# ypicchi-arm/vectorscan

Measured on AMD Instinct MI355X. Metric: GB/s scanned (hsbench block mode), FDR 5k literals, higher is better.
Workload: dtype u8; 1 GPU; cfg4: FDR 5000 literals len 4-8 (2% nocase), one 4 GiB corpus as 4 blocks striped over 1 GPU(s), engine id 0; global_bytes=4294967296, parallelism=stripe1

## Files before the change

include/vectorscan_amd.h:

```cpp
#ifndef VECTORSCAN_AMD_H
#define VECTORSCAN_AMD_H

#include <stddef.h>
#include <stdint.h>

#if defined(__x86_64__) || defined(__i386__)
#include <emmintrin.h>
typedef __m128i vsa_m128_t;
#else
typedef struct { uint8_t b[16]; } __attribute__((aligned(16))) vsa_m128_t;
#endif

#ifdef __cplusplus
extern "C" {
#endif


struct HWLM;
struct FDR;
struct noodTable;
struct hs_scratch;
union AccelAux;

typedef int hwlm_error_t;
// ... 85 lines not shown
#define VSA_E_OVERFLOW (-5)

typedef struct vsa_ctx vsa_ctx_t;
typedef struct vsa_db vsa_db_t;

typedef struct {
    uint64_t key;
    uint32_t id;
    uint32_t pad;
} vsa_match_t;

int vsa_device_count(void);
int vsa_ctx_create(int device, vsa_ctx_t **ctx);
int vsa_ctx_destroy(vsa_ctx_t *ctx);
int vsa_ctx_create_shared(vsa_ctx_t *base, vsa_ctx_t **ctx);
void *vsa_ctx_stream(vsa_ctx_t *ctx);
int vsa_ctx_set_reserved_cus(vsa_ctx_t *ctx, int n);

int vsa_db_load(vsa_ctx_t *ctx, const void *hwlm, size_t size, vsa_db_t **db);
int vsa_db_free(vsa_db_t *db);
int vsa_db_engine(const vsa_db_t *db);

int vsa_malloc(vsa_ctx_t *ctx, size_t bytes, void **dptr);
int vsa_free(vsa_ctx_t *ctx, void *dptr);
int vsa_memcpy_h2d(vsa_ctx_t *ctx, void *dst, const void *src, size_t bytes);
int vsa_memcpy_d2h(vsa_ctx_t *ctx, void *dst, const void *src, size_t bytes);
int vsa_sync(vsa_ctx_t *ctx);

#define VSA_MAX_BLOCKS (1u << 20)

#define VSA_SCAN_UNSORTED 1u
#define VSA_SCAN_ASYNC 2u
int vsa_scan_blocks(vsa_ctx_t *ctx, const vsa_db_t *db, const uint8_t *d_data,
                    const uint64_t *offsets, const uint64_t *lens,
                    const uint64_t *starts, uint32_t nblocks, uint32_t flags,
                    uint64_t *n_matches);
int vsa_scan_blocks_ex(vsa_ctx_t *ctx, const vsa_db_t *db, const uint8_t *d_data,
                       const uint64_t *offsets, const uint64_t *lens,
                       const uint64_t *starts, const uint64_t *report_lo,
                       uint32_t nblocks, uint32_t flags, uint64_t *n_matches);
int vsa_scan_blocks_stream(vsa_ctx_t *ctx, const vsa_db_t *db, const uint8_t *d_data,
                           const uint64_t *offsets, const uint64_t *lens,
                           const uint64_t *starts, const uint64_t *hlens, uint32_t nblocks,
                           uint32_t flags, uint64_t *n_matches);
typedef struct vsa_plan vsa_plan_t;
int vsa_plan_describe(const uint8_t *d_data, const uint64_t *offsets, const uint64_t *lens,
                      const uint64_t *starts, const uint64_t *hlens, const uint64_t *report_lo,
                      uint32_t nblocks, uint32_t num_cus, uint32_t ns, uint32_t *words,
                      uint64_t cap, uint64_t *nsegs, uint32_t *grid,
                      const float *wg_weights);
int vsa_plan_blocks(const uint8_t *d_data, const uint64_t *offsets, const uint64_t *lens,
                    const uint64_t *starts, const uint64_t *hlens, const uint64_t *report_lo,
                    uint32_t nblocks, void *out);

int vsa_plan_dyn(const uint8_t *d_data, const uint64_t *offsets, const uint64_t *lens,
                 const uint64_t *starts, const uint64_t *hlens, const uint64_t *report_lo,
                 uint32_t nblocks, uint32_t num_cus, uint32_t ns, uint32_t *out);
int vsa_feedback_simulate(const double *rate, uint32_t grid, uint32_t launches, double jitter,
                          float *w_out);
int vsa_plan_create(vsa_ctx_t *ctx, const uint8_t *d_data, const uint64_t *offsets,
                    const uint64_t *lens, const uint64_t *starts, const uint64_t *hlens,
                    const uint64_t *report_lo, uint32_t nblocks, vsa_plan_t **plan);
int vsa_plan_free(vsa_plan_t *plan);
uint32_t vsa_plan_rebuilds(const vsa_plan_t *plan);
int vsa_scan_plan(vsa_ctx_t *ctx, const vsa_db_t *db, const vsa_plan_t *plan, uint32_t flags,
                  uint64_t *n_matches);
int vsa_scan_wait(vsa_ctx_t *ctx, uint64_t *n_matches);
int vsa_scan_pack(vsa_ctx_t *ctx, void *d_dst, uint64_t cap);
int vsa_scan_plan_pack(vsa_ctx_t *ctx, const vsa_db_t *db, const vsa_plan_t *plan, void *d_dst,
                       uint64_t cap);
int vsa_scan_results(vsa_ctx_t *ctx, const uint64_t **d_keys,
                     const uint32_t **d_ids);
int vsa_scan_copy(vsa_ctx_t *ctx, vsa_match_t *out, uint64_t cap,
                  uint64_t *n_copied);
int vsa_scan_copy_device(vsa_ctx_t *ctx, uint64_t *d_keys, uint32_t *d_ids, uint64_t cap,
                         uint64_t *n_copied);
uint64_t vsa_scan_candidates(vsa_ctx_t *ctx);
int vsa_scan_debug_counters(vsa_ctx_t *ctx, uint64_t out[16]);
double vsa_scan_kernel_ms(vsa_ctx_t *ctx);
int vsa_ctx_set_timing(vsa_ctx_t *ctx, uint32_t every);
uint64_t vsa_scan_launches(vsa_ctx_t *ctx);
int vsa_scan_last_fused(vsa_ctx_t *ctx);
int vsa_scan_last_dyn(vsa_ctx_t *ctx);
int vsa_ctx_set_dyn_shares(vsa_ctx_t *ctx, int on, uint64_t min_bytes);
int vsa_ctx_set_fused_finish(vsa_ctx_t *ctx, int on);
int vsa_read_ceiling(vsa_ctx_t *ctx, const uint8_t *d_data, uint64_t len, uint32_t runs,
                     double *best_ms, uint64_t *bytes);

int vsa_class_scan(vsa_ctx_t *ctx, const uint8_t cls[32], const uint8_t *cls2,
                   const uint8_t *d_data, uint64_t len, uint64_t *d_bitmap,
                   uint64_t *first, uint64_t *last, uint64_t *count,
                   uint32_t flags);
int vsa_class_scan_masks(vsa_ctx_t *ctx, int kind, const uint8_t a[16], const uint8_t b[16],
                         const uint8_t *d_data, uint64_t len, uint64_t *d_bitmap,
                         uint64_t *first, uint64_t *last, uint64_t *count);


typedef struct {
    const uint8_t *s;
    uint32_t len;
    uint32_t id;
    uint8_t nocase;
    uint8_t noruns;
    uint8_t msk_len;
    uint8_t pad;
    uint64_t groups;
    const uint8_t *msk;
    const uint8_t *cmp;
} vsa_literal_t;

typedef struct {
    int32_t engine_hint;
    uint8_t allow_noodle;
    uint8_t allow_teddy;
    uint8_t allow_fat_teddy;
    uint8_t allow_flood;
} vsa_build_opts_t;

void vsa_build_opts_default(vsa_build_opts_t *o);
int vsa_hwlm_build(const vsa_literal_t *lits, size_t n,
                   const vsa_build_opts_t *opts, void **blob, size_t *size);
void vsa_blob_free(void *blob);
int vsa_hwlm_set_accel(void *blob, const union AccelAux *accel0,
                       const union AccelAux *accel1, uint64_t accel1_groups);
int vsa_shufti_build_masks(const uint8_t cls[32], uint8_t lo[16], uint8_t hi[16]);
void vsa_truffle_build_masks(const uint8_t cls[32], uint8_t m1[16], uint8_t m2[16]);

int64_t vsa_shufti_find(const uint8_t lo[16], const uint8_t hi[16],
                        const uint8_t *buf, size_t len, int reverse);
int64_t vsa_truffle_find(const uint8_t m1[16], const uint8_t m2[16],
                         const uint8_t *buf, size_t len, int reverse);
int64_t vsa_shufti_double_find(const uint8_t lo1[16], const uint8_t hi1[16],
                               const uint8_t lo2[16], const uint8_t hi2[16],
                               const uint8_t *buf, size_t len);
void vsa_set_accel_vector_size(uint32_t vsize);

void vsa_set_wave_log(void *d_log);
int vsa_shufti_build_double_masks(const uint8_t onechar[32], const uint8_t *pairs,
                                  size_t npairs, uint8_t lo1[16], uint8_t hi1[16],
                                  uint8_t lo2[16], uint8_t hi2[16]);
int64_t vsa_verm_find(int mode, uint8_t c1, uint8_t c2, uint8_t m1, uint8_t m2,
                      int nocase, const uint8_t *buf, size_t len);

int vsa_derive_first_stage(const void *hwlm, size_t size, uint64_t *table, uint32_t cap,
                           uint32_t *key_bits, uint32_t *field_bits);
int vsa_derive_fdr4_table(const void *hwlm, size_t size, uint32_t bits, uint32_t *table,
                          uint32_t cap);

int vsa_derive_fdr4_pass(const void *hwlm, size_t size, int par, uint32_t *table, uint32_t cap,
                         double *text_rate);

int vsa_db_split(const vsa_db_t *db);

void vsa_set_scratch_layout(long fdr_conf_off, long fdr_conf_offset_off);
void vsa_get_scratch_layout(long *fdr_conf_off, long *fdr_conf_offset_off);

void vsa_set_scratch_core_info(long buf_off, long hbuf_off, long hlen_off);
void vsa_get_scratch_core_info(long *buf_off, long *hbuf_off, long *hlen_off);

int vsa_last_error(void);

const char *vsa_version(void);

#ifdef __cplusplus
}
#endif
// ... 3 lines not shown
```

vectorscan_amd/__init__.py:

```python
import ctypes
import os

import numpy as np

__all__ = [
    "HWLM_SUCCESS", "HWLM_TERMINATED", "HWLM_ERROR_UNKNOWN",
    "HWLM_ALL_GROUPS", "HWLM_CONTINUE_MATCHING", "HWLM_TERMINATE_MATCHING",
    "HwlmLiteral", "hwlm_build", "hwlm_exec", "fdr_exec", "nood_exec",
    "engine_blob", "shufti_exec", "rshufti_exec", "truffle_exec",
    "rtruffle_exec", "vermicelli_exec", "nvermicelli_exec",
    "rvermicelli_exec", "rnvermicelli_exec", "vermicelli_double_exec",
    "vermicelli_double_masked_exec", "shufti_build_masks",
    "truffle_build_masks", "Context", "Database", "lib", "LIB_PATH",
]

HWLM_SUCCESS = 0
HWLM_TERMINATED = 1
HWLM_ERROR_UNKNOWN = 2
HWLM_ALL_GROUPS = (1 << 64) - 1
HWLM_CONTINUE_MATCHING = HWLM_ALL_GROUPS
HWLM_TERMINATE_MATCHING = 0

ENGINE_NOOD = 16
HWLM_HEADER = 192
# ... 41 lines not shown
_sig("vsa_hwlm_set_accel", ctypes.c_int, ctypes.c_void_p, ctypes.c_void_p,
     ctypes.c_void_p, ctypes.c_uint64)
_sig("hwlmExec", ctypes.c_int, ctypes.c_void_p, ctypes.c_void_p, ctypes.c_size_t,
     ctypes.c_size_t, HWLMCallback, ctypes.c_void_p, ctypes.c_uint64)
_sig("fdrExec", ctypes.c_int, ctypes.c_void_p, ctypes.c_void_p, ctypes.c_size_t,
     ctypes.c_size_t, HWLMCallback, ctypes.c_void_p, ctypes.c_uint64)
_sig("noodExec", ctypes.c_int, ctypes.c_void_p, ctypes.c_void_p, ctypes.c_size_t,
     ctypes.c_size_t, HWLMCallback, ctypes.c_void_p)
_sig("hwlmExecStreaming", ctypes.c_int, ctypes.c_void_p, ctypes.c_size_t, ctypes.c_size_t,
     HWLMCallback, ctypes.c_void_p, ctypes.c_uint64)
_sig("fdrExecStreaming", ctypes.c_int, ctypes.c_void_p, ctypes.c_void_p, ctypes.c_size_t,
     ctypes.c_void_p, ctypes.c_size_t, ctypes.c_size_t, HWLMCallback, ctypes.c_void_p,
     ctypes.c_uint64)
_sig("noodExecStreaming", ctypes.c_int, ctypes.c_void_p, ctypes.c_void_p, ctypes.c_size_t,
     ctypes.c_void_p, ctypes.c_size_t, HWLMCallback, ctypes.c_void_p)
_sig("vsa_get_scratch_core_info", None, ctypes.POINTER(ctypes.c_long),
     ctypes.POINTER(ctypes.c_long), ctypes.POINTER(ctypes.c_long))
_sig("vsa_shufti_find", ctypes.c_int64, ctypes.c_void_p, ctypes.c_void_p,
     ctypes.c_void_p, ctypes.c_size_t, ctypes.c_int)
_sig("vsa_shufti_double_find", ctypes.c_int64, ctypes.c_void_p, ctypes.c_void_p,
     ctypes.c_void_p, ctypes.c_void_p, ctypes.c_void_p, ctypes.c_size_t)
_sig("vsa_set_accel_vector_size", None, ctypes.c_uint32)
_sig("vsa_shufti_build_double_masks", ctypes.c_int, ctypes.c_void_p, ctypes.c_void_p,
     ctypes.c_size_t, ctypes.c_void_p, ctypes.c_void_p, ctypes.c_void_p, ctypes.c_void_p)
_sig("vsa_truffle_find", ctypes.c_int64, ctypes.c_void_p, ctypes.c_void_p,
     ctypes.c_void_p, ctypes.c_size_t, ctypes.c_int)
_sig("vsa_verm_find", ctypes.c_int64, ctypes.c_int, ctypes.c_uint8, ctypes.c_uint8,
     ctypes.c_uint8, ctypes.c_uint8, ctypes.c_int, ctypes.c_void_p, ctypes.c_size_t)
_sig("vsa_shufti_build_masks", ctypes.c_int, ctypes.c_void_p, ctypes.c_void_p,
     ctypes.c_void_p)
_sig("vsa_truffle_build_masks", None, ctypes.c_void_p, ctypes.c_void_p,
     ctypes.c_void_p)
_sig("vsa_device_count", ctypes.c_int)
_sig("vsa_ctx_create", ctypes.c_int, ctypes.c_int, ctypes.POINTER(ctypes.c_void_p))
_sig("vsa_ctx_destroy", ctypes.c_int, ctypes.c_void_p)
_sig("vsa_ctx_create_shared", ctypes.c_int, ctypes.c_void_p, ctypes.POINTER(ctypes.c_void_p))
_sig("vsa_ctx_stream", ctypes.c_void_p, ctypes.c_void_p)
_sig("vsa_db_load", ctypes.c_int, ctypes.c_void_p, ctypes.c_void_p, ctypes.c_size_t,
     ctypes.POINTER(ctypes.c_void_p))
_sig("vsa_db_free", ctypes.c_int, ctypes.c_void_p)
_sig("vsa_db_engine", ctypes.c_int, ctypes.c_void_p)
_sig("vsa_malloc", ctypes.c_int, ctypes.c_void_p, ctypes.c_size_t,
     ctypes.POINTER(ctypes.c_void_p))
_sig("vsa_free", ctypes.c_int, ctypes.c_void_p, ctypes.c_void_p)
_sig("vsa_memcpy_h2d", ctypes.c_int, ctypes.c_void_p, ctypes.c_void_p,
     ctypes.c_void_p, ctypes.c_size_t)
_sig("vsa_memcpy_d2h", ctypes.c_int, ctypes.c_void_p, ctypes.c_void_p,
     ctypes.c_void_p, ctypes.c_size_t)
_sig("vsa_sync", ctypes.c_int, ctypes.c_void_p)
_sig("vsa_scan_blocks", ctypes.c_int, ctypes.c_void_p, ctypes.c_void_p,
     ctypes.c_void_p, _u64p, _u64p, ctypes.c_void_p, ctypes.c_uint32,
     ctypes.c_uint32, _u64p)
_sig("vsa_scan_blocks_ex", ctypes.c_int, ctypes.c_void_p, ctypes.c_void_p,
     ctypes.c_void_p, _u64p, _u64p, ctypes.c_void_p, ctypes.c_void_p, ctypes.c_uint32,
     ctypes.c_uint32, _u64p)
_sig("vsa_scan_blocks_stream", ctypes.c_int, ctypes.c_void_p, ctypes.c_void_p,
     ctypes.c_void_p, _u64p, _u64p, ctypes.c_void_p, _u64p, ctypes.c_uint32,
     ctypes.c_uint32, _u64p)
_sig("vsa_plan_create", ctypes.c_int, ctypes.c_void_p, ctypes.c_void_p, ctypes.c_void_p,
     ctypes.c_void_p, ctypes.c_void_p, ctypes.c_void_p, ctypes.c_void_p, ctypes.c_uint32,
     ctypes.POINTER(ctypes.c_void_p))
_sig("vsa_plan_free", ctypes.c_int, ctypes.c_void_p)
_sig("vsa_plan_rebuilds", ctypes.c_uint32, ctypes.c_void_p)
_sig("vsa_scan_plan", ctypes.c_int, ctypes.c_void_p, ctypes.c_void_p, ctypes.c_void_p,
     ctypes.c_uint32, _u64p)
_sig("vsa_scan_wait", ctypes.c_int, ctypes.c_void_p, _u64p)
_sig("vsa_scan_pack", ctypes.c_int, ctypes.c_void_p, ctypes.c_void_p, ctypes.c_uint64)
_sig("vsa_scan_plan_pack", ctypes.c_int, ctypes.c_void_p, ctypes.c_void_p, ctypes.c_void_p,
     ctypes.c_void_p, ctypes.c_uint64)
_sig("vsa_scan_results", ctypes.c_int, ctypes.c_void_p,
     ctypes.POINTER(ctypes.c_void_p), ctypes.POINTER(ctypes.c_void_p))
_sig("vsa_scan_copy", ctypes.c_int, ctypes.c_void_p, ctypes.c_void_p,
     ctypes.c_uint64, _u64p)
_sig("vsa_scan_copy_device", ctypes.c_int, ctypes.c_void_p, ctypes.c_void_p, ctypes.c_void_p,
     ctypes.c_uint64, _u64p)
_sig("vsa_scan_candidates", ctypes.c_uint64, ctypes.c_void_p)
_sig("vsa_scan_debug_counters", ctypes.c_int, ctypes.c_void_p, ctypes.c_void_p)
_sig("vsa_derive_first_stage", ctypes.c_int, ctypes.c_void_p, ctypes.c_size_t, ctypes.c_void_p,
     ctypes.c_uint32, ctypes.POINTER(ctypes.c_uint32), ctypes.POINTER(ctypes.c_uint32))
_sig("vsa_scan_kernel_ms", ctypes.c_double, ctypes.c_void_p)
_sig("vsa_scan_launches", ctypes.c_uint64, ctypes.c_void_p)
_sig("vsa_scan_last_fused", ctypes.c_int, ctypes.c_void_p)
_sig("vsa_scan_last_dyn", ctypes.c_int, ctypes.c_void_p)
_sig("vsa_ctx_set_dyn_shares", ctypes.c_int, ctypes.c_void_p, ctypes.c_int, ctypes.c_uint64)
_sig("vsa_ctx_set_fused_finish", ctypes.c_int, ctypes.c_void_p, ctypes.c_int)
_sig("vsa_ctx_set_timing", ctypes.c_int, ctypes.c_void_p, ctypes.c_uint32)
_sig("vsa_ctx_set_reserved_cus", ctypes.c_int, ctypes.c_void_p, ctypes.c_int)
_sig("vsa_read_ceiling", ctypes.c_int, ctypes.c_void_p, ctypes.c_void_p, ctypes.c_uint64,
     ctypes.c_uint32, ctypes.POINTER(ctypes.c_double), _u64p)
_sig("vsa_class_scan", ctypes.c_int, ctypes.c_void_p, ctypes.c_void_p,
     ctypes.c_void_p, ctypes.c_void_p, ctypes.c_uint64, ctypes.c_void_p, _u64p,
     _u64p, _u64p, ctypes.c_uint32)
_sig("vsa_class_scan_masks", ctypes.c_int, ctypes.c_void_p, ctypes.c_int, ctypes.c_void_p,
     ctypes.c_void_p, ctypes.c_void_p, ctypes.c_uint64, ctypes.c_void_p, _u64p, _u64p, _u64p)
_sig("vsa_version", ctypes.c_char_p)
_sig("vsa_set_scratch_layout", None, ctypes.c_long, ctypes.c_long)
_sig("vsa_get_scratch_layout", None, ctypes.POINTER(ctypes.c_long), ctypes.POINTER(ctypes.c_long))
_sig("vsa_last_error", ctypes.c_int)


class HwlmLiteral:

    def __init__(self, s, nocase=False, id=0, noruns=False,
                 groups=HWLM_ALL_GROUPS, msk=b"", cmp=b""):
        if isinstance(s, str):
            s = s.encode("latin-1")
        self.s = bytes(s)
        self.nocase = bool(nocase)
        self.id = int(id)
        self.noruns = bool(noruns)
        self.groups = int(groups)
        self.msk = bytes(msk)
        self.cmp = bytes(cmp)

    def __repr__(self):
        return "HwlmLiteral(%r, nocase=%s, id=%d)" % (self.s, self.nocase, self.id)


class Blob:

    def __init__(self, ptr, size, owned=True):
        self.ptr = ptr
        self.size = size
        self.owned = owned

    def tobytes(self):
        return ctypes.string_at(self.ptr, self.size)

    @property
    def type(self):
        return ctypes.string_at(self.ptr, 1)[0]

    @property
    def is_noodle(self):
        return self.type == ENGINE_NOOD

    @property
    def engine_id(self):
        if self.is_noodle:
            return None
        return int(np.frombuffer(ctypes.string_at(self.ptr + HWLM_HEADER, 4), np.uint32)[0])

    def set_accel(self, accel0=None, accel1=None, accel1_groups=0):
        a0 = ctypes.create_string_buffer(bytes(accel0), 80) if accel0 else None
        a1 = ctypes.create_string_buffer(bytes(accel1), 80) if accel1 else None
        _check(lib.vsa_hwlm_set_accel(self.ptr, a0, a1, accel1_groups))

    def __del__(self):
        if getattr(self, "ptr", None) and getattr(self, "owned", True) and lib is not None:
            lib.vsa_blob_free(self.ptr)
        self.ptr = None


class BuildError(RuntimeError):
    pass


def _check(rc):
    if rc != 0:
        raise BuildError("vectorscan_amd call failed with %d" % rc)


def hwlm_build(lits, engine_hint=-1, allow_noodle=True, allow_teddy=True,
               allow_fat_teddy=True, allow_flood=True):
    arr = (_Literal * len(lits))()
    keep = []
# ... 404 lines not shown
        ln = np.ascontiguousarray(lens, np.uint64)
        hl = np.ascontiguousarray(hlens, np.uint64)
        st = None if starts is None else np.ascontiguousarray(starts, np.uint64)
        n = ctypes.c_uint64()
        flags = (0 if sort else 1) | (2 if asynchronous else 0)
        rc = lib.vsa_scan_blocks_stream(
            self.ptr, db.ptr, d_data, off.ctypes.data_as(_u64p), ln.ctypes.data_as(_u64p),
            None if st is None else st.ctypes.data, hl.ctypes.data_as(_u64p), len(off), flags,
            ctypes.byref(n))
        if rc != 0:
            raise RuntimeError("vsa_scan_blocks_stream failed (%d)" % rc)
        return n.value

    def plan(self, d_data, offsets, lens, starts=None, hlens=None, report_lo=None):
        arrs = [None if a is None else np.ascontiguousarray(a, np.uint64)
                for a in (offsets, lens, starts, hlens, report_lo)]
        h = ctypes.c_void_p()
        rc = lib.vsa_plan_create(self.ptr, d_data, *[None if a is None else a.ctypes.data
                                                      for a in arrs], len(arrs[0]),
                                 ctypes.byref(h))
        if rc != 0:
            raise RuntimeError("vsa_plan_create failed (%d)" % rc)
        return Plan(self, h.value)

    def scan_plan(self, db, plan, sort=True, asynchronous=False):
        n = ctypes.c_uint64()
        flags = (0 if sort else 1) | (2 if asynchronous else 0)
        rc = lib.vsa_scan_plan(self.ptr, db.ptr, plan.ptr, flags, ctypes.byref(n))
        if rc != 0:
            raise RuntimeError("vsa_scan_plan failed (%d)" % rc)
        return n.value

    def scan_wait(self):
        n = ctypes.c_uint64()
        _check(lib.vsa_scan_wait(self.ptr, ctypes.byref(n)))
        return n.value

    def scan_pack(self, d_dst, cap):
        _check(lib.vsa_scan_pack(self.ptr, d_dst, cap))

    def scan_plan_pack(self, db, plan, d_dst, cap):
        _check(lib.vsa_scan_plan_pack(self.ptr, db.ptr, plan.ptr, d_dst, cap))

    def results(self, n):
        out = np.zeros(n, dtype=[("key", np.uint64), ("id", np.uint32), ("pad", np.uint32)])
        got = ctypes.c_uint64()
        _check(lib.vsa_scan_copy(self.ptr, out.ctypes.data, n, ctypes.byref(got)))
        return out[: got.value]

    def results_to_device(self, d_keys, d_ids, cap):
        got = ctypes.c_uint64()
        _check(lib.vsa_scan_copy_device(self.ptr, d_keys, d_ids, cap, ctypes.byref(got)))
        return got.value

    def candidates(self):
        return lib.vsa_scan_candidates(self.ptr)

    def debug_counters(self):
        out = (ctypes.c_uint64 * 16)()
        _check(lib.vsa_scan_debug_counters(self.ptr, out))
        return list(out)

    def kernel_ms(self):
        return lib.vsa_scan_kernel_ms(self.ptr)

    def reserve_cus(self, n):
        _check(lib.vsa_ctx_set_reserved_cus(self.ptr, n))

    def launches(self):
        return lib.vsa_scan_launches(self.ptr)

    def timing(self, every=1):
        _check(lib.vsa_ctx_set_timing(self.ptr, every))

    def fused_finish(self, on=True):
        _check(lib.vsa_ctx_set_fused_finish(self.ptr, 1 if on else 0))

    def last_fused(self):
        return lib.vsa_scan_last_fused(self.ptr) == 1

    def last_dyn(self):
        return lib.vsa_scan_last_dyn(self.ptr) == 1

    def dyn_shares(self, on=True, min_mib=2048):
        _check(lib.vsa_ctx_set_dyn_shares(self.ptr, 1 if on else 0, int(min_mib) << 20))

    def read_ceiling(self, d_data, length, runs=5):
        ms = ctypes.c_double()
        n = ctypes.c_uint64()
        _check(lib.vsa_read_ceiling(self.ptr, d_data, length, runs, ctypes.byref(ms),
                                    ctypes.byref(n)))
        return n.value / (ms.value * 1e-3) / 1e9, ms.value, n.value

    def class_scan(self, cls, d_data, length, d_bitmap=None, cls2=None):
        cls = np.ascontiguousarray(cls, np.uint8)
        c2 = None if cls2 is None else np.ascontiguousarray(cls2, np.uint8)
        f, l, c = ctypes.c_uint64(), ctypes.c_uint64(), ctypes.c_uint64()
        _check(lib.vsa_class_scan(self.ptr, cls.ctypes.data,
                                  None if c2 is None else c2.ctypes.data, d_data,
                                  length, d_bitmap, ctypes.byref(f), ctypes.byref(l),
                                  ctypes.byref(c), 0))
        return f.value, l.value, c.value

    def class_scan_masks(self, kind, a, b, d_data, length, d_bitmap=None):
        ma = ctypes.create_string_buffer(bytes(a), 16)
        mb = ctypes.create_string_buffer(bytes(b), 16)
        f, l, c = ctypes.c_uint64(), ctypes.c_uint64(), ctypes.c_uint64()
        _check(lib.vsa_class_scan_masks(self.ptr, 0 if kind == "shufti" else 1, ma, mb, d_data,
                                        length, d_bitmap, ctypes.byref(f), ctypes.byref(l),
                                        ctypes.byref(c)))
        return f.value, l.value, c.value

    def close(self):
        if self.ptr:
            lib.vsa_ctx_destroy(self.ptr)
            self.ptr = None

    def __del__(self):
        try:
            self.close()
        except Exception:
            pass


class Plan:

    def __init__(self, ctx, ptr):
        self.ctx = ctx
        self.ptr = ptr

    def rebuilds(self):
        return lib.vsa_plan_rebuilds(self.ptr)

    def close(self):
        if self.ptr:
            lib.vsa_plan_free(self.ptr)
            self.ptr = None

    def __del__(self):
        try:
            self.close()
        except Exception:
            pass


class Database:

    def __init__(self, ctx, blob):
        self.ctx = ctx
        self.blob = blob
        self.ptr = ctypes.c_void_p()
        rc = lib.vsa_db_load(ctx.ptr, blob.ptr, blob.size, ctypes.byref(self.ptr))
        if rc != 0:
            raise RuntimeError("vsa_db_load failed (%d)" % rc)

    @property
    def engine(self):
        return lib.vsa_db_engine(self.ptr)

    @property
    def split(self):
        return lib.vsa_db_split(self.ptr) == 1

    def close(self):
        if self.ptr:
            lib.vsa_db_free(self.ptr)
# ... 6 lines not shown
```

vectorscan_amd/csrc/kernels.h:

```cpp
#ifndef VSA_KERNELS_H
#define VSA_KERNELS_H

#include <stdint.h>

struct VsaBlock {
    uint64_t base;
    uint64_t len;
    uint64_t start;
    uint64_t seg_first;
    int64_t zbase;
    int64_t org;
    int64_t rlo;
    uint64_t hlen;
    uint32_t hist;
    uint32_t flags;
};
#ifdef __cplusplus
static_assert(sizeof(VsaBlock) == 72, "VsaBlock layout (vsa_plan_blocks, tests/test_plan.py)");
#endif

#define VSA_BLK_STREAM 1u
#define VSA_BLK_RUN 2u
#define VSA_RUN_MAX 128u
#define VSA_RUN_MIN_LEN 1024u

#define VSA_KEY_END_SHIFT 24
#define VSA_KEY_BUCKET_SHIFT 20
#define VSA_KEY_LI_MASK 0xfffffu

#ifdef __HIPCC__
__host__ __device__
#endif
static inline uint32_t vsa_fdr4_key(uint32_t b2, uint32_t b1, uint32_t b0) {
    return (b1 & 0x7fu) | ((b2 & 1u) << 7) | ((b0 & 0x7fu) << 8);
}

enum VsaLitMode {
    VSA_MODE_TEDDY = 1,
    VSA_MODE_FAT = 2,
    VSA_MODE_NOOD = 3,
    VSA_MODE_FDR4 = 4,
};

#define VSA_SORT_BIN_BITS 14
#define VSA_SORT_BINS (1u << VSA_SORT_BIN_BITS)
#define VSA_LBINS 256u
#define VSA_SORT_BIN_MAX 64
#define VSA_CTR_BIN_OVERFLOW 12
#define VSA_FIN_MAX_GRID 1024u

struct VsaLitParams {
    const uint8_t *data;
    const VsaBlock *blocks;
    uint32_t nblocks;
    uint64_t nsegs;
    const uint32_t *seg_desc;
    const uint32_t *wg_seg;
    const uint32_t *wg_bins;
    uint32_t steal;
    const uint64_t *table;
    uint32_t table_entries;
    uint32_t dmask;
    uint32_t end_par;
    uint64_t state_lo, state_hi;
    const uint8_t *conf_base;
    uint32_t conf_off[16];
    const uint32_t *slotmap;
    uint32_t slot_words;
    uint32_t slot_off[16];
    uint8_t slot_bits[16];
    uint64_t nood_msk, nood_cmp;
    uint32_t nood_len, nood_id;
    uint64_t pf_mult;
    uint32_t qcap;
    uint32_t nconf;
    uint32_t dbg;
    uint64_t *out_keys;
    uint32_t *out_ids;
    uint64_t out_cap;
    uint32_t *bin_counts;
    uint32_t bin_shift;
    uint64_t *bin_keys;
    uint32_t *bin_ids;
    unsigned long long *wg_time;
    unsigned long long *wave_log;
    unsigned long long *counters;
    const uint32_t *fin_wg;
    uint64_t *fin_keys;
    uint32_t *fin_ids;
    unsigned long long *fin_agg;
    uint32_t fin_epoch;
    unsigned long long *fin_pub;
    unsigned long long fin_seq;
    uint64_t *fin_pk;
    uint64_t fin_pk_cap;
    const unsigned long long *dyn_prev;
    const uint32_t *dyn_wprev;
    uint32_t *dyn_wout;
    uint32_t dyn_kib;
    uint32_t dyn_margin;
};


struct VsaClassParams {
    const uint8_t *data;
    uint64_t len;
    uint32_t cls[8];
    uint32_t cls2[8];
    int pair;
    uint64_t *bitmap;
    unsigned long long *first;
    unsigned long long *last;
    unsigned long long *count;
    uint32_t slots;
};

struct VsaPairParams {
    const uint8_t *data;
    uint64_t len;
    uint8_t n1[256], n2[256];
    uint32_t vsize;
    uint32_t mis;
    unsigned long long *first;
};

// ... 2 lines not shown
```

vectorscan_amd/csrc/kernels.hip:

```cpp
#include <hip/hip_runtime.h>
#include <stdint.h>

#include "kernels.h"

#define WAVE 64
#define LIT_WAVES 16
#ifdef VSA_DIAG
#define VSA_DIAG_ON 1
#else
#define VSA_DIAG_ON 0
#endif
#define VSA_DBG(flags, bits) (VSA_DIAG_ON && ((flags) & (bits)))
#define LIT_THREADS (LIT_WAVES * WAVE)
#define QCAP 256

typedef uint32_t u32;
typedef uint64_t u64;
typedef uint8_t u8;

__device__ __forceinline__ u32 lane_id() { return __lane_id(); }

__device__ __forceinline__ u32 readlane_u32(u32 v, int src) {
    return (u32)__builtin_amdgcn_readlane((int)v, src);
}
__device__ __forceinline__ u32 readfirstlane_u32(u32 v) {
    return (u32)__builtin_amdgcn_readfirstlane((int)v);
}

__device__ __forceinline__ u32 shfl_u32(u32 v, int src) {
    return (u32)__shfl((int)v, src, WAVE);
}
__device__ __forceinline__ u32 shfl_up_u32(u32 v, unsigned d) {
    return (u32)__shfl_up((int)v, d, WAVE);
}
__device__ __forceinline__ u32 lane_up1(u32 v) {
    return (u32)__builtin_amdgcn_update_dpp(0, (int)v, 0x138, 0xf, 0xf, true);
}
__device__ __forceinline__ u32 lane_down1(u32 v) {
    return (u32)__builtin_amdgcn_update_dpp(0, (int)v, 0x130, 0xf, 0xf, true);
}
__device__ __forceinline__ u32 lane_up1_or_old(u32 old, u32 v) {
    return (u32)__builtin_amdgcn_update_dpp((int)old, (int)v, 0x138, 0xf, 0xf, false);
}
__device__ __forceinline__ u32 lane_ror1(u32 v) {
    return (u32)__builtin_amdgcn_update_dpp(0, (int)v, 0x13c, 0xf, 0xf, true);
}
template <int L>
__device__ __forceinline__ u32 writelane_u32(u32 v, u32 s) {
    asm("v_writelane_b32 %0, %1, %2" : "+v"(v) : "s"(readfirstlane_u32(s)), "n"(L));
    return v;
}
typedef const __attribute__((address_space(3))) u64 lds_u64_t;
typedef const __attribute__((address_space(3))) u8 lds_u8_t;
__device__ __forceinline__ u64 lds_ld64(u32 addr) { return *(lds_u64_t *)(uintptr_t)addr; }

#define TEDDY_TAB_LDS 0x10000u

__device__ __forceinline__ u32 or3(u32 a, u32 b, u32 c) {
    u32 r;
    asm("v_or3_b32 %0, %1, %2, %3" : "=v"(r) : "v"(a), "v"(b), "v"(c));
    return r;
}
__device__ __forceinline__ u32 shfl_xor_u32(u32 v, int m) {
    return (u32)__shfl_xor((int)v, m, WAVE);
}
__device__ __forceinline__ u32 shfl_down_u32(u32 v, unsigned d) {
    return (u32)__shfl_down((int)v, d, WAVE);
}
template <int M>
__device__ __forceinline__ u32 lane_xor(u32 v) {
    static_assert(M == 1 || M == 2 || M == 4 || M == 8 || M == 16 || M == 32, "lane_xor");
    if constexpr (M == 1) {
        return (u32)__builtin_amdgcn_update_dpp(0, (int)v, 0xB1, 0xf, 0xf, false);
    } else if constexpr (M == 2) {
        return (u32)__builtin_amdgcn_update_dpp(0, (int)v, 0x4E, 0xf, 0xf, false);
    } else if constexpr (M == 4) {
        const int h = __builtin_amdgcn_update_dpp(0, (int)v, 0x141, 0xf, 0xf, false);
        return (u32)__builtin_amdgcn_update_dpp(0, h, 0x1B, 0xf, 0xf, false);
    } else if constexpr (M == 8) {
        const int h = __builtin_amdgcn_update_dpp(0, (int)v, 0x140, 0xf, 0xf, false);
        return (u32)__builtin_amdgcn_update_dpp(0, h, 0x141, 0xf, 0xf, false);
    } else if constexpr (M == 16) {
        return (u32)__builtin_amdgcn_ds_swizzle((int)v, 0x401F);
    } else {
        return shfl_xor_u32(v, 32);
    }
}

struct Bins4 {
    u64 k[4];
    u32 id[4], jb[4];
    bool ok[4];
    u32 S, npass, r;
};
__device__ __forceinline__ void bins4_load(Bins4 &B, const uint64_t *skeys, const uint32_t *sids,
// ... 109 lines not shown
    }
    *total = shfl_u32(x, WAVE - 1);
    return x - v;
}

__device__ __forceinline__ u8 load_byte_masked(const u8 *A, int64_t aoff, int64_t lo, int64_t hi,
                                               bool want, const u8 *safe) {
    const bool ok = want && aoff >= lo && aoff < hi;
    typedef const __attribute__((address_space(1))) u8 gu8;
    const u8 v = *(gu8 *)(ok ? A + aoff : safe);
    return ok ? v : (u8)0;
}

__device__ __forceinline__ VsaBlock load_block(const VsaBlock *blocks, u32 i) {
    static_assert(sizeof(VsaBlock) == 9 * sizeof(u64), "VsaBlock: 9 words");
    typedef const __attribute__((address_space(4))) u64 cu64;
    cu64 *p = (cu64 *)(blocks + i);
    u64 w[9];
#pragma unroll
    for (int k = 0; k < 9; k++) w[k] = p[k];
    VsaBlock b;
    __builtin_memcpy(&b, w, sizeof(b));
    return b;
}


template <int MODE>
struct LitTraits;

template <>
struct LitTraits<VSA_MODE_TEDDY> {
    static constexpr int LB = 8;
    static constexpr int NL = 4;
    static constexpr int CW = 4;
    static constexpr int EW = 3;
    typedef u32 S_t;
};
template <>
struct LitTraits<VSA_MODE_NOOD> {
    static constexpr int LB = 8;
    static constexpr int NL = 1;
    static constexpr int CW = 1;
    static constexpr int EW = 2;
    typedef u32 S_t;
};
template <>
struct LitTraits<VSA_MODE_FAT> {
    static constexpr int LB = 16;
    static constexpr int NL = 4;
    static constexpr int CW = 8;
    static constexpr int EW = 4;
    typedef u64 S_t;
};
template <>
struct LitTraits<VSA_MODE_FDR4> {
    static constexpr int LB = 8;
    static constexpr int NL = 4;
    static constexpr int CW = 4;
    static constexpr int EW = 3;
    typedef u32 S_t;
};

struct PfRec {
    u64 andmsk;
    u32 slot_off;
    u32 shift;
};

struct ConfLds {
    u64 andmsk[16];
    u64 mult[16];
    u32 nbits[16];
    u32 off[16];
    PfRec pf[16];
    u32 lb_lo, lb_n;
    u32 lbins[VSA_LBINS];
    u32 nrec;
    u64 f_lo;
    u32 f_shift;
    u32 f_bad;
    u32 f_cand;
};

__device__ __forceinline__ u32 rec_bin(const VsaLitParams &P, const ConfLds &cl, u64 end) {
    if (P.fin_keys) {
        const u64 d = (end - cl.f_lo) >> cl.f_shift;
        return d < VSA_LBINS ? (u32)d : 0xffffffffu;
    }
    return (u32)(end >> P.bin_shift);
}
__device__ __forceinline__ size_t bin_row(const VsaLitParams &P, u32 bin) {
    return P.fin_keys ? (size_t)blockIdx.x * VSA_LBINS + bin : (size_t)bin;
}

__device__ __forceinline__ u32 bin_slot_take(const VsaLitParams &P, const ConfLds &cl, u32 bin) {
    const u32 k = bin - cl.lb_lo;
    if (k < cl.lb_n)
        return __hip_atomic_fetch_add(const_cast<u32 *>(&cl.lbins[k]), 1u, __ATOMIC_RELAXED,
                                      __HIP_MEMORY_SCOPE_WORKGROUP);
    if (P.fin_keys) {
        __hip_atomic_store(const_cast<u32 *>(&cl.f_bad), 1u, __ATOMIC_RELAXED,
                           __HIP_MEMORY_SCOPE_WORKGROUP);
        return VSA_SORT_BIN_MAX;
    }
    return __hip_atomic_fetch_add(&P.bin_counts[bin], 1u, __ATOMIC_RELAXED,
                                  __HIP_MEMORY_SCOPE_AGENT);
}

__device__ __forceinline__ void flag_crowd(const VsaLitParams &P) {
    __hip_atomic_store(&P.counters[VSA_CTR_BIN_OVERFLOW], 1ULL, __ATOMIC_RELAXED,
                       __HIP_MEMORY_SCOPE_AGENT);
}

struct QEnt {
    u64 meta;
    u64 key;
};

#define ENT_BLK_SHIFT 40
#define ENT_LAP_SHIFT 60
#define ENT_P0_MASK ((1ULL << ENT_BLK_SHIFT) - 1)
struct LitShared {
    const void *tab;
    u32 tab_lds;
    u32 tsel;
    uint4 *ring;
    const u32 *tail;
    u32 *head;
    u32 lg;
    u32 dbg;
    const u32 *slots;
    unsigned long long *diag;
};

__device__ __forceinline__ u32 lds_ld32(const u32 *p) {
    return __hip_atomic_load(p, __ATOMIC_RELAXED, __HIP_MEMORY_SCOPE_WORKGROUP);
}
__device__ __forceinline__ void lds_st32(u32 *p, u32 v) {
    __hip_atomic_store(p, v, __ATOMIC_RELAXED, __HIP_MEMORY_SCOPE_WORKGROUP);
}

__device__ __forceinline__ u32 conf_hash(u64 key, u64 andmsk, u64 mult, u32 nbits) {
    return (u32)(((key & andmsk) * mult) >> (64 - nbits));
}

template <int CONF_U>
__device__ __forceinline__ void confirm_multi(const VsaLitParams &P, const ConfLds &cl,
                                              const QEnt (&q)[CONF_U], const bool (&valid)[CONF_U],
                                              u32 mis) {
    u32 fc[CONF_U], li[CONF_U];
    u32 st[CONF_U], b[CONF_U];
    u64 base[CONF_U], blen[CONF_U];
    int64_t hlen[CONF_U], e[CONF_U];
#pragma unroll
    for (int i = 0; i < CONF_U; i++) {
        b[i] = (u32)(q[i].meta & 15);
        const u32 blk = (u32)((q[i].meta >> 4) & 0xfffff);
        fc[i] = cl.off[b[i]];
        st[i] = 0;
        base[i] = 0;
        blen[i] = ~0ULL;
        hlen[i] = 0;
        if (valid[i]) {
            const u32 c = conf_hash(q[i].key, cl.andmsk[b[i]], cl.mult[b[i]], cl.nbits[b[i]]);
            st[i] = *((const u32 *)(P.conf_base + fc[i] + 32) + c);
            base[i] = P.blocks[blk].base;
            blen[i] = P.blocks[blk].len;
            hlen[i] = (int64_t)P.blocks[blk].hlen;
        }
    }
    bool live[CONF_U];
#pragma unroll
    for (int i = 0; i < CONF_U; i++) {
        live[i] = st[i] != 0;
        li[i] = fc[i] + st[i];
        e[i] = (int64_t)((q[i].meta >> 24) - mis - base[i]);
        if (e[i] >= (int64_t)blen[i]) {
            const VsaBlock &nb = P.blocks[((q[i].meta >> 4) & 0xfffff) + 1];
            base[i] += blen[i];
            e[i] -= (int64_t)blen[i];
            hlen[i] = (int64_t)nb.hlen;
        }
    }
    for (;;) {
        bool any = false;
#pragma unroll
        for (int i = 0; i < CONF_U; i++) any |= live[i];
        if (!__any(any)) break;
        uint4 w0[CONF_U], w1[CONF_U];
#pragma unroll
        for (int i = 0; i < CONF_U; i++) {
            if (live[i]) {
                w0[i] = *(const uint4 *)(P.conf_base + li[i]);
                w1[i] = *(const uint4 *)(P.conf_base + li[i] + 16);
            }
        }
        bool mt[CONF_U];
        u64 pm[CONF_U];
        u32 tot = 0;
#pragma unroll
        for (int i = 0; i < CONF_U; i++) {
            mt[i] = false;
            if (live[i]) {
                const u64 v = ((u64)w0[i].y << 32) | w0[i].x;
                const u64 msk = ((u64)w0[i].w << 32) | w0[i].z;
                const u32 size = w1[i].w & 0xff;
                mt[i] = (q[i].key & msk) == v && e[i] + 1 + hlen[i] >= (int64_t)size;
            }
            pm[i] = __ballot(mt[i]);
            tot += (u32)__popcll(pm[i]);
        }
        if (tot) {
            const bool bins = P.bin_keys != nullptr;
            unsigned long long s0 = 0;
            if (lane_id() == 0) {
                if (bins)
                    __hip_atomic_fetch_add(const_cast<u32 *>(&cl.nrec), tot, __ATOMIC_RELAXED,
                                           __HIP_MEMORY_SCOPE_WORKGROUP);
                else
                    s0 = atomicAdd(&P.counters[0], (unsigned long long)tot);
            }
            const u64 sb = ((u64)readlane_u32((u32)(s0 >> 32), 0) << 32) | readlane_u32((u32)s0, 0);
            u32 bslot[CONF_U], bbin[CONF_U];
#pragma unroll
            for (int i = 0; i < CONF_U; i++)
                if (bins && mt[i]) {
                    bbin[i] = rec_bin(P, cl, base[i] + (u64)e[i]);
                    bslot[i] = bin_slot_take(P, cl, bbin[i]);
                }
#pragma unroll
            for (int i = 0; i < CONF_U; i++) {
                if (!mt[i]) continue;
                const u64 end = base[i] + (u64)e[i];
                const u64 lidx = (u64)((li[i] - fc[i]) >> 3) & VSA_KEY_LI_MASK;
                u32 before = 0;
#pragma unroll
                for (int k = 0; k < i; k++) before += (u32)__popcll(pm[k]);
                const u64 q = bins ? (u64)bin_row(P, bbin[i]) * VSA_SORT_BIN_MAX + bslot[i]
                                   : sb + before + __builtin_amdgcn_mbcnt_hi(
                                         (u32)(pm[i] >> 32), __builtin_amdgcn_mbcnt_lo((u32)pm[i], 0));
                if (bins ? bslot[i] < VSA_SORT_BIN_MAX : q < P.out_cap) {
                    (bins ? P.bin_keys : P.out_keys)[q] = (end << VSA_KEY_END_SHIFT) |
                                                          ((u64)b[i] << VSA_KEY_BUCKET_SHIFT) | lidx;
                    (bins ? P.bin_ids : P.out_ids)[q] = w1[i].z;
                } else if (bins) {
                    flag_crowd(P);
                }
            }
        }
#pragma unroll
        for (int i = 0; i < CONF_U; i++) {
            if (!live[i]) continue;
            li[i] += 32;
            live[i] = ((w1[i].w >> 16) & 0xff) != 0;
        }
    }
}

template <int MODE>
__device__ __forceinline__ u64 lit_lookup(const void *tab, u32 key, u32 lane) {
    if constexpr (MODE == VSA_MODE_FDR4) {
        (void)lane;
        return ((const u32 *)tab)[key];
    } else if constexpr (MODE == VSA_MODE_TEDDY) {
        return ((const u32 *)tab)[(key << 6) | (lane & 31)];
    } else {
        return ((const u64 *)tab)[(key << 5) | (lane & 31)];
    }
}

struct IterState {
    u64 carry;
    u64 pbytes;
    u32 p3, p4;
    u32 ncand;
    u32 tail_cache;
    u32 head;
    u32 xs[4];
    u32 xn;
};

struct SegCtx {
    u32 blk;
    int64_t blo, bhi;
    int64_t vlo;
    int64_t start, len, zbase;
    int64_t rlo;
    int64_t qlo;
    int64_t run_nxt;
    bool stream;
};

template <int EW, typename ST>
__device__ __forceinline__ void ring_push(const LitShared &L, ST &st, bool push,
                                          const u32 (&w)[4 * EW]) {
    const u64 pm = __ballot(push);
    if (pm == 0) return;
    const u32 n = (u32)__popcll(pm);
    const u32 r = __builtin_amdgcn_mbcnt_hi((u32)(pm >> 32),
                                             __builtin_amdgcn_mbcnt_lo((u32)pm, 0));
    const u32 cap = 1u << L.lg;
    for (u32 b0 = 0; b0 < n; b0 += cap) {
        const u32 m = n - b0 < cap ? n - b0 : cap;
        const u32 pos = st.head;
        if (pos + m - st.tail_cache > cap) {
            for (;;) {
                st.tail_cache = readfirstlane_u32(lds_ld32(L.tail));
                if (pos + m - st.tail_cache <= cap) break;
                __builtin_amdgcn_s_sleep(2);
            }
        }
        if (push && r >= b0 && r < b0 + m) {
            const u32 slot = pos + r - b0;
            uint4 *q = L.ring + (size_t)(slot & (cap - 1)) * EW;
#pragma unroll
            for (int k = 0; k < EW; k++)
                if (k < 2 || !VSA_DBG(L.dbg, 256))
                    q[k] = make_uint4(w[4 * k], w[4 * k + 1], w[4 * k + 2], w[4 * k + 3]);
        }
        st.head = pos + m;
        asm volatile("" ::: "memory");
// ... 174 lines not shown
__device__ __forceinline__ u32 nib_to_bytes(u32 t) {
    return (((t & 0xfu) * 0x00204081u) & 0x01010101u) * 0xffu;
}
__device__ __forceinline__ u32 window4(const u32 (&s)[4], int o) {
    const int a = o >> 2;
    const u32 b = (u32)o & 3u;
    auto W = [&](int i) -> u32 {
        u32 v = 0;
#pragma unroll
        for (int k = 0; k < 4; k++) v = i == k ? s[k] : v;
        return v;
    };
    return __builtin_amdgcn_alignbyte(W(a + 1), W(a), b);
}

template <typename ST>
__device__ __forceinline__ void xp_flush(const VsaLitParams &P, const ConfLds &cl,
                                         const LitShared &L, ST &st) {
    const u32 n = st.xn;
    if (n == 0) return;
    const bool act = lane_id() < n;
    const u64 key = ((u64)st.xs[3] << 32) | st.xs[2];
    const u32 bb = st.xs[0] & 7u;
    const PfRec pf = cl.pf[bb];
    const bool chk = act && pf.slot_off != 0xffffffffu;
    const u32 h = (u32)(((key & pf.andmsk) * P.pf_mult) >> pf.shift);
    const u32 sw = chk ? lds_ld32(&L.slots[pf.slot_off + (h >> 5)]) : ~0u;
    const bool push = act && ((sw >> (h & 31)) & 1u);
    const u32 w[4] = {st.xs[0], st.xs[1], st.xs[2], st.xs[3]};
    ring_push<1>(L, st, push, w);
    st.xn = 0;
}

__device__ __forceinline__ void xp_push(const VsaLitParams &P, const ConfLds &cl,
                                        const LitShared &L, IterState &st, u32 (&c)[4],
                                        u64 meta, u32 pv2, u32 pv3, const u32 (&d)[4]) {
    const u32 D[6] = {pv2, pv3, d[0], d[1], d[2], d[3]};
    const u64 p0 = meta & ENT_P0_MASK;
    const u64 blk4 = (meta >> ENT_BLK_SHIFT) << 4;
    const u32 lane = lane_id();
    u64 lo = ((u64)c[1] << 32) | c[0];
    u64 hi = ((u64)c[3] << 32) | c[2];
    for (;;) {
        const bool have = (lo | hi) != 0;
        const u64 B = __ballot(have);
        if (B == 0) break;
        const u32 cnt = (u32)__popcll(B);
        if (st.xn + cnt > WAVE) xp_flush(P, cl, L, st);
        const bool inlo = lo != 0;
        const u64 cur = inlo ? lo : hi;
        const u32 b = (inlo ? 0u : 64u) + (u32)__builtin_ctzll(cur | (1ull << 63));
        const u64 nxt = cur & (cur - 1);
        lo = inlo ? nxt : lo;
        hi = inlo ? hi : nxt;
        const u32 jj = b >> 3, bb = b & 7;
        const u32 o = jj + 1, a = o >> 2, sh = o & 3u;
        u32 x0 = D[0], x1 = D[1], x2 = D[2];
#pragma unroll
        for (int k = 1; k < 5; k++) {
            const bool sel = a == (u32)k;
            x0 = sel ? D[k] : x0;
            x1 = sel ? D[k + 1] : x1;
            x2 = sel ? D[k + 2 < 6 ? k + 2 : 5] : x2;
        }
        const u32 key_lo = __builtin_amdgcn_alignbyte(x1, x0, sh);
        const u32 key_hi = __builtin_amdgcn_alignbyte(x2, x1, sh);
        const u64 qm = ((p0 + jj) << 24) | blk4 | bb;
        const u32 rk = __builtin_amdgcn_mbcnt_hi((u32)(B >> 32), __builtin_amdgcn_mbcnt_lo((u32)B, 0));
        const u32 dst = have ? st.xn + rk : (st.xn + cnt + (lane - rk)) & (WAVE - 1);
        const int da = (int)(dst << 2);
        const u32 r0 = (u32)__builtin_amdgcn_ds_permute(da, (int)(u32)qm);
        const u32 r1 = (u32)__builtin_amdgcn_ds_permute(da, (int)(u32)(qm >> 32));
        const u32 r2 = (u32)__builtin_amdgcn_ds_permute(da, (int)key_lo);
        const u32 r3 = (u32)__builtin_amdgcn_ds_permute(da, (int)key_hi);
        const bool mine = lane - st.xn < cnt;
        st.xs[0] = mine ? r0 : st.xs[0];
        st.xs[1] = mine ? r1 : st.xs[1];
        st.xs[2] = mine ? r2 : st.xs[2];
        st.xs[3] = mine ? r3 : st.xs[3];
        st.xn += cnt;
    }
}

template <int MODE, bool EDGE, bool XP, bool SPLIT>
__device__ __forceinline__ IterState lit_iter(const VsaLitParams &P, const ConfLds &cl,
                                              const LitShared &L, const SegCtx &S,
                                              u32 mis, int64_t ib, uint4 chunk,
                                              IterState in, u32 bucket_mask) {
    typedef LitTraits<MODE> T;
    typedef typename T::S_t S_t;
    const u32 lane = lane_id();
    const int64_t p0 = ib + 16 * (int64_t)lane;
    const int64_t q0 = p0 - S.blo;

    u32 d[4] = {chunk.x, chunk.y, chunk.z, chunk.w};
    u32 look_m = 0xffffu;
    if (EDGE) {
        const int r_len = rel32(S.len, q0);
        const u32 bm = range_mask(rel32(S.vlo - S.blo, q0), r_len);
#pragma unroll
        for (int w = 0; w < 4; w++) d[w] &= nib_to_bytes(bm >> (4 * w));
        look_m = range_mask(rel32(MODE == VSA_MODE_FDR4 ? S.zbase : S.qlo, q0), r_len);
    }

    constexpr bool F4 = MODE == VSA_MODE_FDR4;
    constexpr bool PSTATE = F4 && !EDGE;
    u32 pv3;
    IterState out;
    if constexpr (PSTATE) {
        pv3 = lane_up1_or_old(in.p3, d[3]);
        out.p3 = lane_ror1(d[3]);
    } else {
        pv3 = writelane_u32<0>(lane_up1(d[3]), (u32)(in.pbytes >> 32));
    }
    u32 c[T::CW];
    out.ncand = in.ncand;
    out.tail_cache = in.tail_cache;
    out.head = in.head;
#pragma unroll
    for (int k = 0; k < 4; k++) out.xs[k] = in.xs[k];
    out.xn = in.xn;
    if constexpr (PSTATE) {
        out.pbytes = (in.pbytes & 0xffffffff00000000ULL) | readlane_u32(d[2], WAVE - 1);
        out.carry = in.carry;
    } else {
        out.pbytes = ((u64)readlane_u32(d[3], WAVE - 1) << 32) | readlane_u32(d[2], WAVE - 1);
    }
    if constexpr (F4) {
        u32 U[5];
        fdr4_conf<EDGE>(L, {d[0], d[1], d[2], d[3]}, pv3, look_m, U);
        auto split_mask = [&]() {
            if constexpr (SPLIT) {
                const u32 fl = P.end_par == 1 ? 0u : 0x01010101u;
#pragma unroll
                for (int w = 0; w < 4; w++) {
                    const u32 t = (d[w] ^ fl) & 0x01010101u;
                    U[w] |= (t << 8) - t;
                }
            }
        };
        if constexpr (EDGE) {
            const u32 s_in = writelane_u32<0>(lane_up1(U[4]), (u32)in.carry);
            out.carry = readlane_u32(U[4], WAVE - 1);
            U[0] |= s_in;
            split_mask();
        } else {
            U[0] |= lane_up1_or_old(in.p4, U[4]);
            out.p4 = lane_ror1(U[4]);
            split_mask();
            const u32 nbm = ~bucket_mask;
            if (!wave_any(((U[0] & U[1] & U[2] & U[3]) | nbm) != 0xffffffffu)) return out;
        }
#pragma unroll
        for (int w = 0; w < 4; w++) c[w] = U[w];
    } else {
    S_t x[16];
#pragma unroll
    for (int j = 0; j < 16; j++) {
        const u32 sel = 0x0c020000u | ((4u + (j & 3)) << 8);
        const u32 a = __builtin_amdgcn_perm(d[j >> 2], L.tsel, sel);
        if constexpr (MODE == VSA_MODE_TEDDY) x[j] = lds_ld32a(a);
        else x[j] = lds_ld64(a);
        if (EDGE) {
            if (!((look_m >> j) & 1u)) x[j] = 0;
        }
    }
    u64 s_out;
    conf_accumulate<MODE>(x, c, s_out);
    const u32 s_in_lo = writelane_u32<0>(lane_up1((u32)s_out), (u32)in.carry);
    const u32 s_in_hi = sizeof(S_t) == 8
                            ? writelane_u32<0>(lane_up1((u32)(s_out >> 32)), (u32)(in.carry >> 32))
                            : 0u;
    const u64 s_in = ((u64)s_in_hi << 32) | s_in_lo;
    out.carry = ((u64)readlane_u32((u32)(s_out >> 32), WAVE - 1) << 32) |
                readlane_u32((u32)s_out, WAVE - 1);
    c[0] |= (u32)s_in;
    if constexpr (sizeof(S_t) == 8) c[1] |= (u32)(s_in >> 32);
    }
    if (EDGE) {
        if constexpr (MODE == VSA_MODE_FDR4) if (!S.stream) {
            const int64_t r0 = q0 - S.start;
            if (r0 > -16 && r0 < 16) {
                const u32 sv[4] = {(u32)P.state_lo, (u32)(P.state_lo >> 32), (u32)P.state_hi,
                                   (u32)(P.state_hi >> 32)};
#pragma unroll
                for (int w = 0; w < 4; w++) c[w] |= window4(sv, (int)r0 + 4 * w);
            }
        }
        const u32 out_m = ~range_mask(rel32(S.rlo, q0), rel32(S.len, q0)) & 0xffffu;
        if constexpr (T::LB == 8) {
#pragma unroll
            for (int w = 0; w < 4; w++) c[w] |= nib_to_bytes(out_m >> (4 * w));
        } else {
#pragma unroll
            for (int w = 0; w < 8; w++) {
                const u32 t = out_m >> (2 * w);
                c[w] |= ((t & 1u) ? 0xffffu : 0u) | ((t & 2u) ? 0xffff0000u : 0u);
            }
        }
    }

    u32 all = c[0];
#pragma unroll
    for (int i = 1; i < T::CW; i++) all &= c[i];
    if (!wave_any((all | ~bucket_mask) != 0xffffffffu)) return out;
#ifdef VSA_DIAG
    const bool tdiag = (P.dbg & 32768) != 0;
#else
    constexpr bool tdiag = false;
#endif
    const u64 t_c0 = tdiag ? __builtin_amdgcn_s_memtime() : 0;
    u32 any = 0;
#pragma unroll
    for (int i = 0; i < T::CW; i++) {
        c[i] = ~c[i] & bucket_mask;
        any |= c[i];
    }
    if (VSA_DBG(P.dbg, 32)) {
        u32 pc = 0;
#pragma unroll
        for (int i = 0; i < T::CW; i++) pc += __popc(c[i]);
#pragma unroll
        for (int dd = 32; dd >= 1; dd >>= 1) pc += shfl_xor_u32(pc, dd);
        out.ncand += readfirstlane_u32(pc);
    }
    if (VSA_DBG(P.dbg, 8)) return out;

    u32 pv2 = lane_up1(d[2]);
    if (lane == 0) pv2 = (u32)in.pbytes;
    const u32 lblk = S.blk + (p0 >= S.run_nxt ? 1u : 0u);
    const u64 meta = (u64)p0 | ((u64)lblk << ENT_BLK_SHIFT);
    if constexpr (XP) {
        xp_push(P, cl, L, out, c, meta, pv2, pv3, d);
        return out;
    }
    u32 w[4 * T::EW];
#pragma unroll
    for (int i = 0; i < 4 * T::EW; i++) w[i] = 0;
    w[0] = (u32)meta;
    w[1] = (u32)(meta >> 32);
#pragma unroll
    for (int i = 0; i < T::CW; i++) w[2 + i] = c[i];
    w[2 + T::CW] = pv2;
    w[3 + T::CW] = pv3;
#pragma unroll
    for (int i = 0; i < 4; i++) w[4 + T::CW + i] = d[i];
    const u64 t_c1 = tdiag ? __builtin_amdgcn_s_memtime() : 0;
    ring_push<T::EW>(L, out, any != 0, w);
    if (tdiag && lane == 0) {
        const u64 t_c2 = __builtin_amdgcn_s_memtime();
        atomicAdd(&L.diag[0], (unsigned long long)(t_c1 - t_c0));
        atomicAdd(&L.diag[1], (unsigned long long)(t_c2 - t_c1));
        atomicAdd(&L.diag[2], 1ull);
    }
    return out;
}

template <bool EDGE>
__device__ __forceinline__ IterState nood_iter(const VsaLitParams &P, const LitShared &L,
                                               const SegCtx &S, int64_t ib, uint4 chunk,
                                               IterState in) {
    const u32 lane = lane_id();
    const int64_t p0 = ib + 16 * (int64_t)lane;
    const int64_t q0 = p0 - S.blo;
    u32 d[4] = {chunk.x, chunk.y, chunk.z, chunk.w};
    if (EDGE) {
        const u32 bm = range_mask(rel32(S.vlo - S.blo, q0), rel32(S.len, q0));
#pragma unroll
        for (int w = 0; w < 4; w++) d[w] &= nib_to_bytes(bm >> (4 * w));
    }
    u32 pv2 = lane_up1(d[2]), pv3 = lane_up1(d[3]);
    if (lane == 0) {
        pv2 = (u32)in.pbytes;
        pv3 = (u32)(in.pbytes >> 32);
    }
    IterState out = in;
    out.pbytes = ((u64)readlane_u32(d[3], WAVE - 1) << 32) | readlane_u32(d[2], WAVE - 1);
    if (!EDGE) {
        auto rep8 = [](u64 v, int byte) { return ((u32)(v >> (8 * byte)) & 0xffu) * 0x01010101u; };
        const u32 M2 = rep8(P.nood_msk, 7), C2 = rep8(P.nood_cmp, 7);
        const u32 M1 = rep8(P.nood_msk, 6), C1 = rep8(P.nood_cmp, 6);
        const u32 M0 = rep8(P.nood_msk, 5), C0 = rep8(P.nood_cmp, 5);
        u32 z = 0;
#pragma unroll
        for (int k = 0; k < 4; k++) {
            const u32 lo = k ? d[k - 1] : pv3;
            const u32 p1 = __builtin_amdgcn_alignbyte(d[k], lo, 3);
            const u32 p2 = __builtin_amdgcn_alignbyte(d[k], lo, 2);
            const u32 t = or3((d[k] & M2) ^ C2, (p1 & M1) ^ C1, (p2 & M0) ^ C0);
            z |= (t - 0x01010101u) & ~t;
        }
        if (!wave_any((z & 0x80808080u) != 0)) return out;
    }
    const u32 w[6] = {pv2, pv3, d[0], d[1], d[2], d[3]};
    const u32 mlo = (u32)P.nood_msk, mhi = (u32)(P.nood_msk >> 32);
    const u32 clo = (u32)P.nood_cmp, chi = (u32)(P.nood_cmp >> 32);
    u32 hits = 0;
#pragma unroll
    for (int j = 0; j < 16; j++) {
        const int bo = j + 1;
        u32 lo, hi;
        if (bo & 3) {
            lo = __builtin_amdgcn_alignbyte(w[(bo >> 2) + 1], w[bo >> 2], bo & 3);
            hi = __builtin_amdgcn_alignbyte(w[(bo >> 2) + 2], w[(bo >> 2) + 1], bo & 3);
        } else {
            lo = w[bo >> 2];
            hi = w[(bo >> 2) + 1];
        }
        if (((lo & mlo) == clo) & ((hi & mhi) == chi)) hits |= 1u << j;
    }
    if (EDGE) {
        const int64_t elo = S.start + (int64_t)P.nood_len - 1 + S.qlo;
        hits &= range_mask(rel32(elo > S.rlo ? elo : S.rlo, q0), rel32(S.len, q0));
    }
    if (!wave_any(hits != 0)) return out;
    const u64 meta = (u64)p0 | ((u64)S.blk << ENT_BLK_SHIFT);
    const u32 ent[8] = {(u32)meta, (u32)(meta >> 32), 0, 0, hits, 0, 0, 0};
    ring_push<2>(L, out, hits != 0, ent);
    return out;
}

template <int MODE, bool EDGE, bool XP, bool SPLIT>
__device__ __forceinline__ IterState scan_iter(const VsaLitParams &P, const ConfLds &cl,
                                               const LitShared &L, const SegCtx &S,
                                               u32 mis, int64_t ib, uint4 chunk,
                                               IterState in, u32 bucket_mask) {
    if constexpr (MODE == VSA_MODE_NOOD) {
        return nood_iter<EDGE>(P, L, S, ib, chunk, in);
    } else {
        return lit_iter<MODE, EDGE, XP, SPLIT>(P, cl, L, S, mis, ib, chunk, in,
                                                   bucket_mask);
    }
}

__device__ __forceinline__ uint4 load_chunk(const u8 *A, int64_t p0, int64_t bhi) {
    uint4 v = make_uint4(0, 0, 0, 0);
    typedef u32 v4u __attribute__((ext_vector_type(4)));
    if (p0 < bhi) {
        v4u t = __builtin_nontemporal_load((const v4u *)(A + p0));
        v = make_uint4(t.x, t.y, t.z, t.w);
    }
    return v;
}

__device__ __forceinline__ uint4 load_chunk_nc(const u8 *A, int64_t p0) {
    typedef u32 v4u __attribute__((ext_vector_type(4)));
    v4u t = __builtin_nontemporal_load((const v4u *)(A + p0));
    return make_uint4(t.x, t.y, t.z, t.w);
}

__device__ __forceinline__ const u8 *uniform_ptr(const u8 *p) {
    const u64 a = (u64)p;
    return (const u8 *)(((u64)readfirstlane_u32((u32)(a >> 32)) << 32) |
                        readfirstlane_u32((u32)a));
}
__device__ __forceinline__ uint4 load_wave_kib(const u8 *base, u32 off) {
    typedef u32 v4u __attribute__((ext_vector_type(4)));
    typedef const __attribute__((address_space(1))) v4u gv4u;
    gv4u *p = (gv4u *)(base + (off + 16 * lane_id()));
    v4u t = __builtin_nontemporal_load(p);
    return make_uint4(t.x, t.y, t.z, t.w);
}

#define LIT_DEPTH 4
#define VMCNT0 0x0f70

#define MAX_CONF_WAVES 4
#ifndef CONF_IDLE_SLEEP
#define CONF_IDLE_SLEEP 8
#endif
#define EXP_U 1
#define PQ_ENTRIES(CU) ((CU) == 4 ? 512 : 256)
template <int MODE, int CONF_U, bool XP>
__device__ __forceinline__ void confirm_wave(const VsaLitParams &P, const ConfLds &cl,
                                             const uint4 *rings, u32 lg, u32 *tails,
                                             const u32 *heads, const u32 *q_done, u32 mis,
                                             const u32 *slots, QEnt *pq, u32 cw, u32 nc,
                                             u64 *pcl, u64 (&dg)[3]) {
    typedef LitTraits<MODE> T;
    constexpr int EW = XP ? 1 : T::EW;
    constexpr int CW = T::CW;
    constexpr u32 PQ_CAP = PQ_ENTRIES(CONF_U);
    static_assert(PQ_CAP >= CONF_U * 64 + EXP_U * 64 - 1, "confirm queue too small");
    const u32 lane = lane_id();
    const u32 cap = 1u << lg;
    const u32 nscan = LIT_WAVES - nc;
    const u32 nr = (nscan - cw + nc - 1) / nc;
    const u32 sl0 = nr <= 4 ? 16u : nr <= 8 ? 8u : 4u;
    const u32 sl = sl0 < cap ? sl0 : cap;
    const u32 ri = lane / sl;
    const u32 rr = cw + nc * ri, rk = lane - ri * sl;
    const bool ring_lane = ri < nr;
    u32 tail = 0;
    u32 filled = 0;
    u32 consumed = 0;
    u32 pq_head = 0, pq_tail = 0;
    const bool prof = VSA_DBG(P.dbg, 64);
    u64 tmark = prof ? __builtin_amdgcn_s_memtime() : 0;
    auto pcount = [&](int i, u64 v) {
        if (prof && lane == 0) pcl[i] += v;
    };
    auto phase = [&](int i) {
        if (prof) {
            const u64 now = __builtin_amdgcn_s_memtime();
            pcount(i, now - tmark);
            tmark = now;
        }
    };
#ifdef VSA_DIAG
    const bool dlog = (P.dbg & 8192) != 0;
#else
    constexpr bool dlog = false;
#endif
    bool seen_done = false;
    auto confirm_batch = [&](u32 k) {
        if (dlog) {
            dg[1] = __builtin_amdgcn_s_memrealtime();
            if (seen_done) dg[2]++;
        }
        phase(1);
        asm volatile("" ::: "memory");
        QEnt q[CONF_U];
        bool valid[CONF_U];
#pragma unroll
        for (int i = 0; i < CONF_U; i++) {
            const u32 j = lane + (u32)WAVE * i;
            valid[i] = j < k;
            q[i] = valid[i] ? pq[(pq_tail + j) & (PQ_CAP - 1)] : QEnt{0, 0};
        }
        confirm_multi<CONF_U>(P, cl, q, valid, mis);
        asm volatile("" ::: "memory");
        pq_tail += k;
        consumed += k;
        pcount(7, 1);
        phase(2);
    };
    for (;;) {
        const bool all_done = lds_ld32(q_done) == nscan;
        asm volatile("" ::: "memory");
        if (dlog && all_done && !seen_done) {
            seen_done = true;
            dg[0] = __builtin_amdgcn_s_memrealtime();
        }
        const u32 avail = ring_lane ? lds_ld32(&heads[rr]) - tail : 0u;
        const bool valid = rk < avail;
        u32 e[4 * EW];
#pragma unroll
        for (int i = 0; i < 4 * EW; i++) e[i] = 0;
        filled = (u32)__popcll(__ballot(valid));
        if (filled) {
            if (valid) {
                const uint4 *q = rings + ((size_t)rr * cap + ((tail + rk) & (cap - 1))) * EW;
#pragma unroll
                for (int k = 0; k < EW; k++) {
                    const uint4 v = q[k];
                    e[4 * k] = v.x;
                    e[4 * k + 1] = v.y;
                    e[4 * k + 2] = v.z;
                    e[4 * k + 3] = v.w;
                }
            }
            asm volatile("" ::: "memory");
            const u32 run = avail < sl ? avail : sl;
            tail += run;
            if (rk == 0 && ring_lane && run) lds_st32(&tails[rr], tail);
        }
        pcount(4, 1);
        pcount(5, filled);
        phase(0);
        if (filled == 0) {
            if (pq_head != pq_tail) {
                confirm_batch(pq_head - pq_tail);
                continue;
            }
            if (all_done) break;
            __builtin_amdgcn_s_setprio(0);
            __builtin_amdgcn_s_sleep(CONF_IDLE_SLEEP);
            phase(3);
            continue;
        }
        if (VSA_DBG(P.dbg, 128)) continue;
        if constexpr (XP) {
            const u64 pm = __ballot(valid);
            if (valid) {
                const u32 r = __builtin_amdgcn_mbcnt_hi((u32)(pm >> 32),
                                                        __builtin_amdgcn_mbcnt_lo((u32)pm, 0));
                QEnt *q = &pq[(pq_head + r) & (PQ_CAP - 1)];
                q->meta = ((u64)e[1] << 32) | e[0];
                q->key = ((u64)e[3] << 32) | e[2];
            }
            pq_head += filled;
            if (pq_head - pq_tail >= (u32)WAVE * CONF_U) {
                if (filled >= 16 && !VSA_DBG(P.dbg, 1024)) __builtin_amdgcn_s_setprio(2);
                else __builtin_amdgcn_s_setprio(0);
                confirm_batch(WAVE * CONF_U);
            }
            continue;
        }
        if constexpr (MODE != VSA_MODE_NOOD)
        {
            if (filled >= 16 && !VSA_DBG(P.dbg, 1024)) __builtin_amdgcn_s_setprio(2);
            else __builtin_amdgcn_s_setprio(0);
        }
        const u64 meta0 = ((u64)e[1] << 32) | e[0];
        const u64 p0 = meta0 & ENT_P0_MASK;
        const u32 blk = (u32)(meta0 >> ENT_BLK_SHIFT);
        if constexpr (MODE == VSA_MODE_NOOD) {
            u32 hits = e[4];
            if (hits && P.bin_keys) {
                __hip_atomic_fetch_add(const_cast<u32 *>(&cl.nrec), (u32)__popc(hits),
                                       __ATOMIC_RELAXED, __HIP_MEMORY_SCOPE_WORKGROUP);
                consumed += (u32)__popc(hits);
                for (; hits; hits &= hits - 1) {
                    const u32 j = __ffs(hits) - 1;
                    const u64 end = p0 + j - mis;
                    const u32 bin = rec_bin(P, cl, end);
                    const u32 s = bin_slot_take(P, cl, bin);
                    if (s < VSA_SORT_BIN_MAX) {
                        const size_t q = bin_row(P, bin) * VSA_SORT_BIN_MAX + s;
                        P.bin_keys[q] = end << VSA_KEY_END_SHIFT;
                        P.bin_ids[q] = P.nood_id;
                    } else {
                        flag_crowd(P);
                    }
                }
            } else if (hits) {
                const u32 n = (u32)__popc(hits);
                unsigned long long slot = atomicAdd(&P.counters[0], (unsigned long long)n);
                consumed += n;
                for (; hits; hits &= hits - 1, slot++) {
                    const u32 j = __ffs(hits) - 1;
                    if (slot < P.out_cap) {
                        P.out_keys[slot] = (p0 + j - mis) << VSA_KEY_END_SHIFT;
                        P.out_ids[slot] = P.nood_id;
                    }
                }
            }
            continue;
        } else {
            u32 c[CW];
#pragma unroll
            for (int i = 0; i < CW; i++) c[i] = e[2 + i];
            const u64 W0 = ((u64)e[3 + CW] << 32) | e[2 + CW];
            const u64 W1 = ((u64)e[5 + CW] << 32) | e[4 + CW];
            const u64 W2 = ((u64)e[7 + CW] << 32) | e[6 + CW];
            for (;;) {
                bool have[EXP_U];
                u32 jj[EXP_U], bb[EXP_U];
#pragma unroll
                for (int u = 0; u < EXP_U; u++) {
                    u32 word = 0, bits = c[0];
#pragma unroll
                    for (int k = 1; k < CW; k++) {
                        const bool take = bits == 0;
                        bits = take ? c[k] : bits;
                        word = take ? (u32)k : word;
                    }
                    have[u] = bits != 0;
                    const u32 bit = __ffs(bits) - 1;
#pragma unroll
                    for (int k = 0; k < CW; k++)
                        if (have[u] && word == (u32)k) c[k] &= c[k] - 1;
                    if constexpr (T::LB == 8) {
                        jj[u] = 4 * word + (bit >> 3);
                        bb[u] = bit & 7;
                    } else {
                        jj[u] = 2 * word + (bit >> 4);
                        bb[u] = bit & 15;
                    }
                }
                if (!__any(have[0])) break;
                pcount(6, 1);
                u64 key[EXP_U];
                PfRec pf[EXP_U];
#pragma unroll
                for (int u = 0; u < EXP_U; u++) {
                    const u32 o = jj[u] + 1;
                    u64 k8;
                    if (o < 8) k8 = (W0 >> (8 * o)) | (W1 << (64 - 8 * o));
                    else if (o == 8) k8 = W1;
                    else if (o < 16) k8 = (W1 >> (8 * (o - 8))) | (W2 << (64 - 8 * (o - 8)));
                    else k8 = W2;
                    key[u] = k8;
                    pf[u] = cl.pf[bb[u] & 15];
                }
                u32 sw[EXP_U], sh[EXP_U];
                bool chk[EXP_U];
#pragma unroll
                for (int u = 0; u < EXP_U; u++) {
                    chk[u] = have[u] && pf[u].slot_off != 0xffffffffu;
                    const u32 h = (u32)(((key[u] & pf[u].andmsk) * P.pf_mult) >> pf[u].shift);
                    sh[u] = h & 31;
                    sw[u] = chk[u] ? lds_ld32(&slots[pf[u].slot_off + (h >> 5)]) : ~0u;
                }
                bool push[EXP_U];
#pragma unroll
                for (int u = 0; u < EXP_U; u++) {
                    push[u] = have[u] && ((sw[u] >> sh[u]) & 1u);
                    if (VSA_DBG(P.dbg, 16)) push[u] = false;
                }
#pragma unroll
                for (int u = 0; u < EXP_U; u++) {
                    const u64 pm = __ballot(push[u]);
                    if (push[u]) {
                        const u32 r = __builtin_amdgcn_mbcnt_hi(
                            (u32)(pm >> 32), __builtin_amdgcn_mbcnt_lo((u32)pm, 0));
                        QEnt *q = &pq[(pq_head + r) & (PQ_CAP - 1)];
                        q->meta = ((p0 + jj[u]) << 24) | ((u64)blk << 4) | bb[u];
                        q->key = key[u];
                    }
                    pq_head += (u32)__popcll(pm);
                }
                if (pq_head - pq_tail >= (u32)WAVE * CONF_U) confirm_batch(WAVE * CONF_U);
            }
            phase(1);
        }
    }
    if (P.counters && lane == 0 && consumed && !VSA_DBG(P.dbg, 32)) {
        atomicAdd(&P.counters[2], (unsigned long long)consumed);
        if (P.fin_keys)
            __hip_atomic_fetch_add(const_cast<u32 *>(&cl.f_cand), consumed, __ATOMIC_RELAXED,
                                   __HIP_MEMORY_SCOPE_WORKGROUP);
    }
    if (prof && lane == 0) {
        phase(1);
        for (int i = 0; i < 8; i++) atomicAdd(&P.counters[4 + i], (unsigned long long)pcl[i]);
    }
}

template <int UNR, typename TV, typename F>
__device__ __forceinline__ void stage_lds(TV *dst, u32 n, u32 tid, F &&src) {
    u32 base = 0;
    for (; base + UNR * LIT_THREADS <= n; base += UNR * LIT_THREADS) {
        TV v[UNR];
#pragma unroll
        for (int k = 0; k < UNR; k++) v[k] = src(base + (u32)k * LIT_THREADS + tid);
#pragma unroll
        for (int k = 0; k < UNR; k++) dst[base + (u32)k * LIT_THREADS + tid] = v[k];
    }
    for (u32 i = base + tid; i < n; i += LIT_THREADS) dst[i] = src(i);
}

__device__ __forceinline__ void fused_finish(const VsaLitParams &P, const ConfLds &cl, u32 *sc);

struct DynB {
    u32 s_lo, s_hi;
    u32 lk, hk;
};

__device__ __forceinline__ u32 wave_sum_u32(u32 v) {
#pragma unroll
    for (int m = 32; m >= 1; m >>= 1) v += shfl_xor_u32(v, m);
    return readfirstlane_u32(v);
}

__device__ __forceinline__ u32 dyn_window_base(u32 n, u32 near) {
    u32 base = near > 32 ? near - 32 : 0;
    if (base + 64 > n) base = n > 64 ? n - 64 : 0;
    return base;
}

__device__ __forceinline__ u32 dyn_count(const VsaLitParams &P, u32 lane, u32 base, u32 v, u32 L,
                                         bool strict) {
    const u32 n = (u32)P.nsegs;
    const u32 *pos = P.seg_desc + 3;
    auto pred = [&](u32 s, u32 end) -> bool {
        if (s >= end) return false;
        const u32 x = pos[4 * (size_t)s];
        return strict ? x < L : x <= L;
    };
    {
        const bool in = base + lane < n && (strict ? v < L : v <= L);
        const u32 c = (u32)__popcll(__ballot(in));
        if ((c > 0 || base == 0) && (c < 64 || base + 64 >= n)) return base + c;
    }
    u32 lo = 0, hi = n;
    while (hi - lo > 64) {
        const u32 step = (hi - lo + 63) / 64;
        const u32 c = (u32)__popcll(__ballot(pred(lo + lane * step, hi)));
        if (c == 0) return lo;
        const u32 nhi = min(hi, lo + c * step);
        lo = lo + (c - 1) * step + 1;
        hi = nhi;
    }
    return lo + (u32)__popcll(__ballot(pred(lo + lane, hi)));
}

struct DynPre {
    unsigned long long en[4], ex[4];
    u32 wp;
    u32 base_lo, base_hi, v_lo, v_hi;
};

__device__ __forceinline__ void dyn_load(const VsaLitParams &P, u32 lane, DynPre &d) {
    const u32 G = gridDim.x, b = blockIdx.x;
    const u32 n = (u32)P.nsegs;
    const unsigned long long T = P.dyn_kib;
    const u32 *pos = P.seg_desc + 3;
    d.base_lo = dyn_window_base(n, (u32)((unsigned long long)n * (T * b / G) / T));
    d.base_hi = dyn_window_base(n, (u32)((unsigned long long)n * (T * (b + 1) / G) / T));
    d.v_lo = d.base_lo + lane < n ? pos[4 * (size_t)(d.base_lo + lane)] : 0xffffffffu;
    d.v_hi = d.base_hi + lane < n ? pos[4 * (size_t)(d.base_hi + lane)] : 0xffffffffu;
    constexpr unsigned long long M60 = (1ull << 60) - 1;
    d.wp = 65536;
    if (!P.dyn_prev) return;
    if (lane < 8 && P.dyn_wprev) d.wp = P.dyn_wprev[lane];
#pragma unroll
    for (int j = 0; j < 4; j++) {
        const u32 k = lane + 64 * j;
        d.en[j] = ~0ull;
        d.ex[j] = M60;
        if (k < G) {
            d.ex[j] = P.dyn_prev[k];
            d.en[j] = P.dyn_prev[G + k];
        }
    }
}

__device__ __forceinline__ void dyn_bounds(const VsaLitParams &P, u32 lane, const DynPre &dp,
                                           DynB &o) {
    const u32 G = gridDim.x, b = blockIdx.x;
    constexpr u32 ONE = 65536;
    constexpr unsigned long long M60 = (1ull << 60) - 1;
    u32 wq[8];
#pragma unroll
// ... 24 lines not shown
            const u32 x = (u32)(ex[j] >> 60) & 7u;
            const unsigned long long e = ex[j] & M60;
            bad = bad || (k < G && e <= t0);
            const unsigned long long dt = e > t0 ? e - t0 : 0ull;
            const u32 d = dt < 0xffffffull ? (u32)dt : 0xffffffu;
            xk[j] = x;
#pragma unroll
            for (int xx = 0; xx < 8; xx++)
                if (k < G && x == (u32)xx) {
                    s[xx] += d;
                    c[xx] += 1;
                }
        }
        if (!__ballot(bad)) {
            float tx[8], tm = 0.f, np = 0.f;
#pragma unroll
            for (int x = 0; x < 8; x++) {
                s[x] = wave_sum_u32(s[x]);
                c[x] = wave_sum_u32(c[x]);
                tx[x] = c[x] ? (float)s[x] / (float)c[x] : 0.f;
                if (c[x]) {
                    tm += tx[x];
                    np += 1.f;
                }
            }
            tm /= np;
            float tw[8], tsum = 0.f;
#pragma unroll
            for (int x = 0; x < 8; x++) {
                const float w0 = (float)readlane_u32(wp, x) * (1.f / 65536.f);
                tw[x] = c[x] ? w0 * tm / fmaxf(tx[x], 1.f) : 0.f;
                tsum += tw[x];
            }
            const float mean = tsum / np;
#pragma unroll
            for (int x = 0; x < 8; x++)
                if (c[x]) wq[x] = (u32)(fminf(1.1f, fmaxf(0.9f, tw[x] / mean)) * 65536.f + 0.5f);
        } else {
#pragma unroll
            for (int j = 0; j < 4; j++) xk[j] = 0;
        }
    }
    if (b == 0 && lane < 8 && P.dyn_wout) {
        u32 w = wq[0];
#pragma unroll
        for (int x = 1; x < 8; x++) w = lane == (u32)x ? wq[x] : w;
        P.dyn_wout[lane] = w;
    }
    u32 pre = 0, mine = 0, tot = 0;
#pragma unroll
    for (int j = 0; j < 4; j++) {
        const u32 k = lane + 64 * j;
        u32 w = wq[0];
#pragma unroll
        for (int x = 1; x < 8; x++) w = xk[j] == (u32)x ? wq[x] : w;
        if (k < G) {
            tot += w;
            if (k < b) pre += w;
            if (k == b) mine = w;
        }
    }
    pre = wave_sum_u32(pre);
    mine = wave_sum_u32(mine);
    tot = wave_sum_u32(tot);
    const unsigned long long T = P.dyn_kib, M = P.dyn_margin;
    auto bound = [&](u32 i, u32 S) -> u32 {
        if (i == 0) return 0u;
        if (i >= G) return (u32)T;
        const unsigned long long nom = T * i / G;
        unsigned long long L = T * S / tot;
        const unsigned long long lo = nom > M ? nom - M : 0ull, hi = min(nom + M, T);
        L = L < lo ? lo : L > hi ? hi : L;
        return (u32)L;
    };
    o.lk = bound(b, pre);
    o.hk = bound(b + 1, pre + mine);
    o.s_lo = o.s_hi = 0;
    if (o.lk < o.hk) {
        o.s_lo = dyn_count(P, lane, dp.base_lo, dp.v_lo, o.lk, false) - 1;
        o.s_hi = dyn_count(P, lane, dp.base_hi, dp.v_hi, o.hk, true);
    }
}

template <int MODE, bool XP, bool SPLIT>
__global__ void __launch_bounds__(LIT_THREADS)
vsa_lit_scan(VsaLitParams P) {
    typedef LitTraits<MODE> T;
    constexpr int REW = XP ? 1 : T::EW;
    typedef typename T::S_t S_t;
    extern __shared__ __align__(16) u8 smem[];
    __shared__ ConfLds cl;
    __shared__ u32 q_tails[16], q_heads[16], q_done, wg_ctr, conf_fin;
    __shared__ u32 dyn_s[4];
    __shared__ unsigned long long rng[16];
    __shared__ u64 prof_lds[8 * MAX_CONF_WAVES];
    __shared__ unsigned long long diag_lds[3];
    const u32 tid = threadIdx.x;
    const u32 lane = lane_id();
    const u32 wave = readfirstlane_u32(tid / WAVE);
    const unsigned long long t_entry = __builtin_amdgcn_s_memrealtime();
    DynPre dpre;
    if (P.dyn_kib && wave == 0) dyn_load(P, lane, dpre);

    const u32 mis = (u32)((uintptr_t)P.data & 15);
    const u8 *A = P.data - mis;

    u32 tab_bytes = 0;
    const void *tab;
    if constexpr (MODE == VSA_MODE_FDR4) {
        tab_bytes = P.table_entries * 4;
        const uint4 *src = (const uint4 *)P.table;
        stage_lds<8>((uint4 *)smem, tab_bytes / 16, tid, [&](u32 i) { return src[i]; });
        tab = smem;
    } else if constexpr (MODE == VSA_MODE_NOOD) {
        tab = nullptr;
    } else {
        u8 *tb = smem + (TEDDY_TAB_LDS - (u32)(uintptr_t)(lds_u8_t *)smem);
        if constexpr (MODE == VSA_MODE_TEDDY) {
            u32 *t32 = (u32 *)tb;
            for (u32 b0 = 0; b0 < 256 * 32; b0 += 8 * LIT_THREADS) {
                u32 v[8];
#pragma unroll
                for (int k = 0; k < 8; k++) v[k] = (u32)P.table[(b0 + k * LIT_THREADS + tid) >> 5];
#pragma unroll
                for (int k = 0; k < 8; k++) {
                    const u32 i = b0 + k * LIT_THREADS + tid;
                    t32[((i >> 5) << 6) | (i & 31)] = v[k];
                }
            }
        } else {
            stage_lds<8>((u64 *)tb, 256 * 32, tid, [&](u32 i) { return P.table[i >> 5]; });
        }
        tab = tb;
    }
    const u32 NC = P.nconf;
    const u32 NS = LIT_WAVES - NC;
    uint4 *rings = (uint4 *)(smem + ((tab_bytes + 15) & ~15u));
    u32 *slots = (u32 *)(rings + (size_t)NS * P.qcap * REW);
    QEnt *pqx = (QEnt *)(slots + ((P.slot_words + 3) & ~3u));
    stage_lds<4>(slots, P.slot_words, tid, [&](u32 i) { return P.slotmap[i]; });
    if (tid < 16) {
        const u32 off = P.conf_off[tid];
        cl.off[tid] = off;
        PfRec pf;
        pf.slot_off = P.slot_off[tid];
        if (off) {
            const u8 *fc = P.conf_base + off;
            cl.andmsk[tid] = pf.andmsk = *(const u64 *)fc;
            cl.mult[tid] = *(const u64 *)(fc + 8);
            cl.nbits[tid] = *(const u32 *)(fc + 16);
            pf.shift = 64 - (P.slot_bits[tid] ? P.slot_bits[tid] : cl.nbits[tid]);
            if (cl.mult[tid] != P.pf_mult) pf.slot_off = 0xffffffffu;
        } else {
            cl.andmsk[tid] = pf.andmsk = 0;
            cl.mult[tid] = 0;
            cl.nbits[tid] = 1;
            pf.shift = 63;
            pf.slot_off = 0xffffffffu;
        }
        cl.pf[tid] = pf;
    }
    {
        u32 lo = 0, n = 0;
        if (P.fin_keys) {
            const uint32_t *f = P.fin_wg + 4 * (size_t)blockIdx.x;
            n = f[3];
            if (tid == 0) {
                cl.f_lo = ((u64)f[1] << 32) | f[0];
                cl.f_shift = f[2];
                cl.f_bad = 0;
                cl.f_cand = 0;
            }
            for (u32 i = tid; i < n; i += LIT_THREADS) cl.lbins[i] = 0;
        } else if (P.bin_keys && P.wg_bins) {
            lo = P.wg_bins[2 * blockIdx.x];
            n = P.wg_bins[2 * blockIdx.x + 1] - lo;
            for (u32 i = tid; i < n; i += LIT_THREADS) cl.lbins[i] = P.bin_counts[lo + i];
        }
        if (tid == 0) {
            cl.lb_lo = lo;
            cl.lb_n = n;
            cl.nrec = 0;
            conf_fin = 0;
        }
    }
    if (tid < 16) {
        q_tails[tid] = 0;
        q_heads[tid] = 0;
        rng[tid] = 0;
    }
    if (tid == 0) {
        q_done = 0;
        wg_ctr = 0;
        if (P.wg_time)
            __hip_atomic_store(&P.wg_time[gridDim.x + blockIdx.x], t_entry, __ATOMIC_RELAXED,
                               __HIP_MEMORY_SCOPE_AGENT);
    }
    if (tid < 8 * MAX_CONF_WAVES) prof_lds[tid] = 0;
    if (tid < 3) diag_lds[tid] = 0;
    if (P.dyn_kib && wave == 0) {
        DynB d;
        dyn_bounds(P, lane, dpre, d);
        if (lane == 0) {
            dyn_s[0] = d.s_lo;
            dyn_s[1] = d.s_hi;
            dyn_s[2] = d.lk;
            dyn_s[3] = d.hk;
        }
    }
    __syncthreads();

    if (wave >= NS) {
        const u32 cw = wave - NS;
        u64 dg[3] = {0, 0, 0};
        if (NC == 1)
            confirm_wave<MODE, 4, XP>(P, cl, rings, 31 - __clz(P.qcap), q_tails, q_heads, &q_done,
                                  mis, slots, pqx, 0, 1, prof_lds, dg);
        else
            confirm_wave<MODE, 2, XP>(P, cl, rings, 31 - __clz(P.qcap), q_tails, q_heads, &q_done,
                                  mis, slots, pqx + (size_t)cw * PQ_ENTRIES(2), cw, NC,
                                  prof_lds + 8 * cw, dg);
        {
            u32 prev = 0;
            if (lane == 0)
                prev = __hip_atomic_fetch_add(&conf_fin, 1u, __ATOMIC_ACQ_REL,
                                              __HIP_MEMORY_SCOPE_WORKGROUP);
            if (readfirstlane_u32(prev) + 1 == NC) {
                const u32 lo = cl.lb_lo, n = P.fin_keys ? 0u : cl.lb_n;
                for (u32 i = lane; i < n; i += WAVE) P.bin_counts[lo + i] = cl.lbins[i];
                if (lane == 0 && cl.nrec)
                    atomicAdd(&P.counters[0], (unsigned long long)cl.nrec);
            }
        }
        if ((P.dbg & 8192) && P.wave_log && lane < 8) {
            const unsigned long long t_end = __builtin_amdgcn_s_memrealtime();
            P.wave_log[((size_t)blockIdx.x * LIT_WAVES + wave) * 8 + lane] =
                lane == 0 ? t_entry : lane == 1 ? t_end : lane == 2 ? 1ull
                : lane == 3 ? dg[0] : lane == 4 ? dg[1] : lane == 5 ? dg[2] : 0ull;
        }
        goto finish;
    }
    {

    u32 bucket_mask = 0;
    if (!(P.dbg & 2)) {
        u32 present = 0;
        for (int b = 0; b < 16; b++) {
            if (P.conf_off[b]) present |= 1u << b;
        }
        if (T::LB == 8) {
            u32 m8 = present & 0xff;
            bucket_mask = m8 | (m8 << 8) | (m8 << 16) | (m8 << 24);
        } else {
            bucket_mask = (present & 0xffff) | (present << 16);
        }
    }
    LitShared L;
    L.tab = tab;
    L.tab_lds = (u32)(uintptr_t)(lds_u8_t *)smem;
    L.tsel = TEDDY_TAB_LDS | ((lane & 31) << (MODE == VSA_MODE_TEDDY ? 2 : 3));
    L.ring = rings + (size_t)wave * P.qcap * REW;
    L.slots = slots;
    L.tail = &q_tails[wave];
    L.head = &q_heads[wave];
    L.lg = 31 - __clz(P.qcap);
    L.dbg = P.dbg;
    L.diag = diag_lds;

    const unsigned long long t_start = __builtin_amdgcn_s_memrealtime();
    u32 n_seg = 0, n_iter = 0;
    if ((P.dbg & 2048) && lane == 0)
        atomicMax(&P.counters[8], ~t_start);
    u32 ncand_total = 0;
    u32 ring_tail_cache = 0, ring_head = 0;
    u32 xp_s[4] = {0, 0, 0, 0}, xp_n = 0;

    auto take = [&]() -> u32 {
        u32 t = 0;
        if (lane == 0)
            t = __hip_atomic_fetch_add(&wg_ctr, 1u, __ATOMIC_RELAXED, __HIP_MEMORY_SCOPE_WORKGROUP);
        return t;
    };
    auto resolve = [&](u32 t0) -> u32 {
        const u32 t = readlane_u32(t0, 0);
        const u32 wg_lo = readfirstlane_u32(P.dyn_kib ? dyn_s[0] : P.wg_seg[blockIdx.x]);
        const u32 wg_hi = readfirstlane_u32(P.dyn_kib ? dyn_s[1] : P.wg_seg[blockIdx.x + 1]);
        return wg_lo + t < wg_hi ? wg_lo + t : (u32)P.nsegs;
    };
    const bool steal_on = P.steal != 0;
    auto steal = [&](u32 &sg, u32 &gs, u32 &ge) -> bool {
        for (int tries = 0; tries < 64; tries++) {
            unsigned long long w = 0;
            if (lane < NS) w = rng[lane];
            const u32 c = (u32)w & 0xfffffu, e = (u32)(w >> 20) & 0xfffffu;
            const u32 wt = lane < 4 ? 4u : lane < 8 ? 5u : lane < 12 ? 6u : 9u;
            u32 best = e > c ? (e - c) * wt : 0u;
            const u32 mine = best;
#pragma unroll
            for (int dd = 32; dd >= 1; dd >>= 1) {
                const u32 o = shfl_xor_u32(best, dd);
                best = o > best ? o : best;
            }
            best = readfirstlane_u32(best);
            if (best < 4u * P.steal) return false;
            const u64 mk = __ballot(mine == best);
            const u32 v = (u32)__ffsll((long long)mk) - 1;
            const unsigned long long wv =
                ((unsigned long long)readlane_u32((u32)(w >> 32), (int)v) << 32) |
                readlane_u32((u32)w, (int)v);
            const u32 vc = (u32)wv & 0xfffffu, ve = (u32)(wv >> 20) & 0xfffffu;
            const u32 wv_ = v < 4 ? 4u : v < 8 ? 5u : v < 12 ? 6u : 9u;
            const u32 wt_ = wave < 4 ? 4u : wave < 8 ? 5u : wave < 12 ? 6u : 9u;
            u32 mid = ve - ((ve - vc) * wv_ + (wv_ + wt_) / 2) / (wv_ + wt_);
            mid = mid < ve ? mid : ve - 1;
            const unsigned long long nw = (wv & ~(0xfffffULL << 20)) | ((unsigned long long)mid << 20);
            unsigned long long old = wv;
            if (lane == 0)
                __hip_atomic_compare_exchange_strong(&rng[v], &old, nw, __ATOMIC_RELAXED,
                                                     __ATOMIC_RELAXED, __HIP_MEMORY_SCOPE_WORKGROUP);
            old = ((unsigned long long)readlane_u32((u32)(old >> 32), 0) << 32) |
                  readlane_u32((u32)old, 0);
            if (old == wv) {
                sg = (u32)(wv >> 40);
                gs = mid;
                ge = ve;
                return true;
            }
        }
        return false;
    };
    u32 seg = resolve(take());
    u32 st_gs = 0, st_ge = 0;
    bool from_list = true;
    for (;;) {
        bool stolen = false;
        if (seg >= P.nsegs) {
            from_list = false;
            if (steal_on && steal(seg, st_gs, st_ge)) stolen = true;
            else break;
        }
        u32 t_next = 0;
        bool have_next = false;
        bool lastb = true;
        auto prefetch_ticket = [&]() {
            if (!have_next && lastb) {
                t_next = take();
                have_next = true;
            }
        };
        typedef const __attribute__((address_space(4))) u32 cu32;
        const u32 segu = readfirstlane_u32(seg);
        const u32 sbv = ((cu32 *)P.seg_desc)[4 * (size_t)segu];
        u32 d_off = ((cu32 *)P.seg_desc)[4 * (size_t)segu + 1];
        u32 d_len = ((cu32 *)P.seg_desc)[4 * (size_t)segu + 2];
        if (P.dyn_kib) {
            const u32 d_pos = ((cu32 *)P.seg_desc)[4 * (size_t)segu + 3];
            const u32 lk = readfirstlane_u32(dyn_s[2]), hk = readfirstlane_u32(dyn_s[3]);
            const u32 a = d_pos > lk ? d_pos : lk;
            const u32 e = d_pos + d_len < hk ? d_pos + d_len : hk;
            d_off += a - d_pos;
            d_len = e > a ? e - a : 0u;
        }
        const u32 gcount = sbv >> 24;
        const u32 first = sbv & 0xffffffu;
        bool run = false;
        if constexpr (MODE != VSA_MODE_NOOD)
            run = gcount > 1 &&
                  (((cu32 *)P.blocks)[(size_t)first * (sizeof(VsaBlock) / 4) +
                                      offsetof(VsaBlock, flags) / 4] & VSA_BLK_RUN);
        u32 rend0 = 0xffffffffu, rend1 = 0xffffffffu;
        const u32 nblk = run ? 1u : (gcount ? gcount : 1u);
        for (u32 gi = 0; gi < nblk; gi++) {
        lastb = gi + 1 == nblk;
        const u32 blk = first + gi;
        const VsaBlock B = load_block(P.blocks, blk);
        SegCtx S;
        S.blk = blk;
        S.blo = (int64_t)B.base + mis;
        S.bhi = S.blo + (int64_t)B.len;
        S.run_nxt = INT64_MAX;
        u32 rb = 0;
        if (run) {
            if (lane < gcount) {
                const VsaBlock &bl = P.blocks[first + lane];
                rend0 = (u32)(bl.base + bl.len - B.base);
            }
            if (lane + 64 < gcount) {
                const VsaBlock &bl = P.blocks[first + 64 + lane];
                rend1 = (u32)(bl.base + bl.len - B.base);
            }
            S.bhi = S.blo + (int64_t)(gcount > 64 ? readlane_u32(rend1, gcount - 65)
                                                  : readlane_u32(rend0, gcount - 1));
            S.run_nxt = S.blo + (int64_t)readlane_u32(rend0, 0);
        }
        int32_t rn32 = run ? (int32_t)readlane_u32(rend0, 0) : INT32_MAX;
        auto run_adv = [&](int64_t ib) {
            if ((int32_t)(ib - S.blo) + 1024 >= rn32) {
                rb++;
                S.blk++;
                const bool last = rb + 1 >= gcount;
                const u32 nx = rb < 64 ? readlane_u32(rend0, rb) : readlane_u32(rend1, rb - 64);
                S.run_nxt = last ? INT64_MAX : S.blo + (int64_t)nx;
                rn32 = last ? INT32_MAX : (int32_t)nx;
            }
        };
        S.vlo = S.blo - (int64_t)B.hist;
        S.stream = (B.flags & VSA_BLK_STREAM) != 0;
        S.qlo = 0;
        if (S.stream) {
            const int64_t back = (MODE == VSA_MODE_NOOD) ? (int64_t)P.nood_len - 1
                                                         : (int64_t)(T::NL - 1);
            if (MODE != VSA_MODE_NOOD || B.start == 0)
                S.qlo = -min((int64_t)B.hlen, back);
        }
        S.start = (int64_t)B.start;
        S.len = S.bhi - S.blo;
        S.zbase = B.zbase;
        S.rlo = B.rlo > S.start ? B.rlo : S.start;
        const int64_t s_lo = (gcount || run) ? B.org : B.org + ((int64_t)d_off << 10);
        const int64_t s_hi =
            (!gcount && s_lo + ((int64_t)d_len << 10) < S.bhi) ? s_lo + ((int64_t)d_len << 10) : S.bhi;
        const u32 niters = (u32)((s_hi - s_lo + 1023) >> 10);
        const int64_t zlo = MODE == VSA_MODE_FDR4 ? B.zbase : S.qlo;

        const int64_t fast_lo = S.blo + S.rlo + 16;
        u32 f0 = 0, f1 = niters;
        if (s_lo < fast_lo) f0 = (u32)min((int64_t)niters, (fast_lo - s_lo + 1023) >> 10);
        {
            int64_t lim = S.bhi - s_lo - 1024;
            int64_t nf = lim <= 0 ? 0 : (lim + 1023) >> 10;
            if (nf < (int64_t)f1) f1 = (u32)nf;
        }
        if (f1 < f0) f1 = f0;
        const u32 nf = f1 - f0;
        const int64_t fb = s_lo + 1024 * (int64_t)f0;
        uint4 ring[LIT_DEPTH];
        const u32 ng = nf / LIT_DEPTH;
        const u32 gs = stolen ? st_gs : 0u;
        const u32 it0 = gs * LIT_DEPTH;
        const int64_t pro_lo = stolen ? fb + 1024 * (int64_t)it0 : s_lo;
        const bool pro1 = lane < (u32)(T::NL - 1);
        const int64_t pp = pro_lo - (T::NL - 1) + (int64_t)lane;
        const bool pro1_in = pro1 && pp - S.blo >= zlo && pp - S.blo < S.len;
        const u8 *safe = (const u8 *)P.blocks;
        const u8 pb0 = load_byte_masked(A, pp, S.vlo, S.bhi, pro1_in, safe);
        const bool F4P = MODE == VSA_MODE_FDR4;
        const u8 pm2 = F4P ? load_byte_masked(A, pp - 2, S.vlo, S.bhi, pro1_in, safe) : (u8)0;
        const u8 pm1 = F4P ? load_byte_masked(A, pp - 1, S.vlo, S.bhi, pro1_in, safe) : (u8)0;
        const u32 pbb = load_byte_masked(A, pro_lo - 8 + (int64_t)lane, S.vlo, S.bhi, lane < 8, safe);
        const bool early = (f0 == 0 || stolen) && nf > 0;
        const u8 *sb = uniform_ptr(A + fb);
        if (early) {
#pragma unroll
            for (int k = 0; k < LIT_DEPTH; k++)
                ring[k] = load_wave_kib(sb, it0 + (u32)k < nf ? 1024u * (it0 + k) : 1024u * it0);
        }
        if (!early) {
            ring[0] = make_uint4(0, 0, 0, 0);
            ring[1] = make_uint4(0, 0, 0, 0);
        }
        if (f0 > 0 && !stolen) {
            ring[0] = load_chunk(A, s_lo + 16 * (int64_t)lane, S.bhi);
        }
        const bool tail_pre = nf == 0 && f1 < niters && f1 > 0;
        if (tail_pre) {
            const int64_t ibt = s_lo + 1024 * (int64_t)f1;
            ring[1] = load_chunk(A, ibt + 16 * (int64_t)lane, S.bhi);
        }
        IterState is;
        is.ncand = ncand_total;
        is.tail_cache = ring_tail_cache;
        is.head = ring_head;
#pragma unroll
        for (int k = 0; k < 4; k++) is.xs[k] = xp_s[k];
        is.xn = xp_n;
        {
            S_t x = 0;
            if (pro1_in) {
                u32 key;
                if constexpr (MODE == VSA_MODE_FDR4) key = vsa_fdr4_key(pm2, pm1, pb0);
                else key = pb0;
                x = (S_t)lit_lookup<MODE>(tab, key, lane);
                x >>= T::LB * (pro_lo - pp);
            }
            u64 xv = (u64)x;
#pragma unroll
            for (int dd = 1; dd < 8; dd <<= 1) {
                const u32 lo = shfl_down_u32((u32)xv, dd);
                const u32 hi = shfl_down_u32((u32)(xv >> 32), dd);
                xv |= ((u64)hi << 32) | lo;
            }
            is.carry = ((u64)shfl_u32((u32)(xv >> 32), 0) << 32) | shfl_u32((u32)xv, 0);
            u64 pb = (u64)pbb << (8 * (lane & 7));
#pragma unroll
            for (int dd = 1; dd < 8; dd <<= 1) {
                const u32 lo = shfl_down_u32((u32)pb, dd);
                const u32 hi = shfl_down_u32((u32)(pb >> 32), dd);
                pb |= ((u64)hi << 32) | lo;
            }
            is.pbytes = ((u64)shfl_u32((u32)(pb >> 32), 0) << 32) | shfl_u32((u32)pb, 0);
        }
        for (u32 it = 0; it < (stolen ? 0u : f0); it++) {
            const int64_t ib = s_lo + 1024 * (int64_t)it;
            uint4 cur = ring[0];
            if (it > 0) cur = load_chunk(A, ib + 16 * (int64_t)lane, S.bhi);
            is = scan_iter<MODE, true, XP, SPLIT>(P, cl, L, S, mis, ib, cur, is, bucket_mask);
            run_adv(ib);
        }
        bool tail_mine = true;
        u32 swept = 0;
        if (nf > 0) {
            if constexpr (MODE == VSA_MODE_FDR4) {
                is.p3 = (u32)(is.pbytes >> 32);
                is.p4 = (u32)is.carry;
            }
            __builtin_amdgcn_s_waitcnt(VMCNT0);
            if (!early) {
#pragma unroll
                for (int k = 0; k < LIT_DEPTH; k++)
                    ring[k] = load_wave_kib(sb, (u32)k < nf ? 1024u * k : 0u);
            }
            u32 g_end = stolen ? st_ge : ng;
            const bool stealable = steal_on && gcount == 0 && !run && g_end > gs + 1;
            if (stealable && lane == 0)
                rng[wave] = ((unsigned long long)seg << 40) | ((unsigned long long)g_end << 20) | (gs + 1);
            for (u32 g = gs; g < g_end; g++) {
                unsigned long long clm = 0;
                if (stealable && lane == 0)
                    clm = __hip_atomic_fetch_add(&rng[wave], 1ULL, __ATOMIC_RELAXED,
                                                 __HIP_MEMORY_SCOPE_WORKGROUP);
                if (g + 1 == g_end) prefetch_ticket();
#pragma unroll
                for (int k = 0; k < LIT_DEPTH; k++) {
                    const u32 it = g * LIT_DEPTH + k;
                    const int64_t ib = fb + 1024 * (int64_t)it;
                    is = scan_iter<MODE, false, XP, SPLIT>(P, cl, L, S, mis, ib, ring[k], is, bucket_mask);
                    run_adv(ib);
                    const u32 itn = (it + LIT_DEPTH < nf) ? it + LIT_DEPTH : it;
                    ring[k] = load_wave_kib(sb, 1024u * itn);
                }
                if (stealable) {
                    const u32 oe = (readlane_u32((u32)clm, 0) >> 20) |
                                   ((readlane_u32((u32)(clm >> 32), 0) & 0xffu) << 12);
                    if (g + 1 >= oe) {
                        g_end = g + 1;
                        prefetch_ticket();
                    }
                }
            }
            tail_mine = g_end == ng;
            const u32 rem = tail_mine ? nf - ng * LIT_DEPTH : 0u;
            swept = (g_end - gs) * LIT_DEPTH + rem;
#pragma unroll
            for (int k = 0; k < LIT_DEPTH - 1; k++) {
                if ((u32)k < rem) {
                    const u32 it = ng * LIT_DEPTH + k;
                    const int64_t ib = fb + 1024 * (int64_t)it;
                    is = scan_iter<MODE, false, XP, SPLIT>(P, cl, L, S, mis, ib, ring[k], is, bucket_mask);
                    run_adv(ib);
                }
            }
            if constexpr (MODE == VSA_MODE_FDR4) {
                is.pbytes = ((u64)readlane_u32(is.p3, 0) << 32) | (u32)is.pbytes;
                is.carry = readlane_u32(is.p4, 0);
            }
        }
        prefetch_ticket();
        for (u32 it = f1; tail_mine && it < niters; it++) {
            const int64_t ib = s_lo + 1024 * (int64_t)it;
            uint4 cur = ring[1];
            if (it > f1 || !tail_pre) cur = load_chunk(A, ib + 16 * (int64_t)lane, S.bhi);
            is = scan_iter<MODE, true, XP, SPLIT>(P, cl, L, S, mis, ib, cur, is, bucket_mask);
            run_adv(ib);
        }
        n_iter += (stolen ? 0u : f0) + swept + (tail_mine ? niters - f1 : 0u);
        ncand_total = is.ncand;
        ring_tail_cache = is.tail_cache;
        ring_head = is.head;
#pragma unroll
        for (int k = 0; k < 4; k++) xp_s[k] = is.xs[k];
        xp_n = is.xn;
        }
        n_seg++;
        seg = (stolen || !from_list) ? (u32)P.nsegs : resolve(t_next);
    }
    if constexpr (XP) {
        IterState fs;
        fs.tail_cache = ring_tail_cache;
        fs.head = ring_head;
#pragma unroll
        for (int k = 0; k < 4; k++) fs.xs[k] = xp_s[k];
        fs.xn = xp_n;
        xp_flush(P, cl, L, fs);
    }
    if ((P.dbg & 4096) && P.wave_log && lane < 8) {
        u32 xcc, hwid;
        asm volatile("s_getreg_b32 %0, hwreg(HW_REG_XCC_ID)" : "=s"(xcc));
        asm volatile("s_getreg_b32 %0, hwreg(HW_REG_HW_ID)" : "=s"(hwid));
        const unsigned long long t_end = __builtin_amdgcn_s_memrealtime();
        const unsigned long long v[8] = {t_start, t_end, n_seg, n_iter, blockIdx.x, wave,
                                         xcc, (P.dbg & 8192) ? t_entry : hwid};
        unsigned long long x = 0;
#pragma unroll
        for (int k = 0; k < 8; k++) x = (u32)k == lane ? v[k] : x;
        P.wave_log[((size_t)blockIdx.x * LIT_WAVES + wave) * 8 + lane] = x;
    }
    if ((P.dbg & 2048) && lane == 0) {
        const unsigned long long t = __builtin_amdgcn_s_memrealtime();
        atomicMax(&P.counters[9], ~t);
        atomicMax(&P.counters[10], t);
    }
    if (lane == 0) {
        const u32 prev = __hip_atomic_fetch_add(&q_done, 1u, __ATOMIC_RELAXED,
                                                __HIP_MEMORY_SCOPE_WORKGROUP);
        if (VSA_DIAG_ON && (P.dbg & 32768) && prev + 1 == NS) {
            for (int k = 0; k < 3; k++) atomicAdd(&P.counters[13 + k], diag_lds[k]);
        }
        if ((P.dbg & 2048) && prev + 1 == NS)
            atomicMax(&P.counters[11], ~(unsigned long long)__builtin_amdgcn_s_memrealtime());
        if (P.wg_time && prev + 1 == NS) {
            u32 xcc;
            asm volatile("s_getreg_b32 %0, hwreg(HW_REG_XCC_ID)" : "=s"(xcc));
            __hip_atomic_store(&P.wg_time[blockIdx.x],
                               ((unsigned long long)(xcc & 15u) << 60) |
                                   (__builtin_amdgcn_s_memrealtime() & ((1ULL << 60) - 1)),
                               __ATOMIC_RELAXED, __HIP_MEMORY_SCOPE_AGENT);
        }
    }
    if (P.counters && lane_id() == 0 && ncand_total) {
        atomicAdd(&P.counters[2], (unsigned long long)ncand_total);
        if (P.fin_keys)
            __hip_atomic_fetch_add(&cl.f_cand, ncand_total, __ATOMIC_RELAXED,
                                   __HIP_MEMORY_SCOPE_WORKGROUP);
    }
    }
finish:
    if constexpr (MODE != VSA_MODE_FAT)
        if (P.fin_keys) fused_finish(P, cl, (u32 *)smem);
}

template __global__ void vsa_lit_scan<VSA_MODE_FDR4, false, false>(VsaLitParams);
template __global__ void vsa_lit_scan<VSA_MODE_FDR4, true, false>(VsaLitParams);
template __global__ void vsa_lit_scan<VSA_MODE_FDR4, false, true>(VsaLitParams);
template __global__ void vsa_lit_scan<VSA_MODE_FDR4, true, true>(VsaLitParams);
template __global__ void vsa_lit_scan<VSA_MODE_TEDDY, false, false>(VsaLitParams);
template __global__ void vsa_lit_scan<VSA_MODE_FAT, false, false>(VsaLitParams);
template __global__ void vsa_lit_scan<VSA_MODE_NOOD, false, false>(VsaLitParams);



__device__ __forceinline__ void publish_body(unsigned long long *ctr, unsigned long long *h,
                                             unsigned long long seq, uint32_t nzero,
                                             const uint64_t *keys, const uint32_t *ids,
                                             uint32_t kmax) {
    const u32 t = threadIdx.x;
    unsigned long long v = 0;
    if (t < 16) v = ctr[t];
    if (kmax) {
        const uint64_t n = ctr[0];
        const uint32_t m = n < kmax ? (uint32_t)n : kmax;
        uint32_t *hid = (uint32_t *)(h + 17 + kmax);
        for (uint32_t i = t; i < m; i += 256) {
            h[17 + i] = keys[i];
            hid[i] = ids[i];
        }
    }
    __syncthreads();
    if (t < 16) {
        h[1 + t] = v;
        ctr[nzero + t] = v;
    }
    for (u32 i = t; i < nzero; i += 256) ctr[i] = 0;
    asm volatile("s_waitcnt vmcnt(0)" ::: "memory");
    __syncthreads();
    if (t == 0) {
        __threadfence_system();
        __hip_atomic_store(&h[0], seq, __ATOMIC_RELEASE, __HIP_MEMORY_SCOPE_SYSTEM);
    }
}

template <bool COH = false>
__device__ __forceinline__ void publish_wave(unsigned long long *ctr, unsigned long long *h,
                                             unsigned long long seq, uint32_t nzero,
                                             const unsigned long long *fb = nullptr,
                                             unsigned long long *hfb = nullptr, u32 nfb = 0,
                                             uint64_t *pk = nullptr, uint64_t out_cap = 0) {
    auto ld = [](const unsigned long long *p) -> unsigned long long {
        if constexpr (COH)
            return __hip_atomic_load(p, __ATOMIC_RELAXED, __HIP_MEMORY_SCOPE_AGENT);
        else
            return *p;
    };
    const u32 l = lane_id();
    const unsigned long long v = l < 16 ? ld(&ctr[l]) : 0ULL;
    if (pk && l == 0) {
        const unsigned long long ovf = ld(&ctr[VSA_CTR_BIN_OVERFLOW]);
        pk[0] = v | ((v > out_cap || ovf) ? (1ULL << 62) : 0ULL);
    }
    for (u32 i = l; i < nfb; i += WAVE) hfb[i] = ld(&fb[i]);
    asm volatile("s_waitcnt vmcnt(0)" ::: "memory");
    if (l < 16) {
        h[1 + l] = v;
        ctr[nzero + l] = v;
    }
    for (u32 i = l; i < nzero; i += WAVE) ctr[i] = 0;
    asm volatile("s_waitcnt vmcnt(0)" ::: "memory");
    if (l == 0) {
        __threadfence_system();
        __hip_atomic_store(&h[0], seq, __ATOMIC_RELEASE, __HIP_MEMORY_SCOPE_SYSTEM);
    }
}

__device__ __forceinline__ void publish_fused(const VsaLitParams &P, unsigned long long n,
                                              unsigned long long cand, bool crowded) {
    const u32 l = lane_id();
    unsigned long long v = 0;
    if (l == 0) v = n;
    else if (l == 2) v = cand;
    else if (l == VSA_CTR_BIN_OVERFLOW) v = crowded ? 1ULL : 0ULL;
    else if (P.dbg && l < 16)
        v = __hip_atomic_load(&P.counters[l], __ATOMIC_RELAXED, __HIP_MEMORY_SCOPE_AGENT);
    if (P.fin_pk && l == 0)
        P.fin_pk[0] = n | ((n > P.out_cap || crowded) ? (1ULL << 62) : 0ULL);
    asm volatile("s_waitcnt vmcnt(0)" ::: "memory");
    if (l < 16) {
        P.fin_pub[1 + l] = v;
        P.counters[144 + l] = v;
    }
    for (u32 i = l; i < 144; i += WAVE) P.counters[i] = 0;
    asm volatile("s_waitcnt vmcnt(0)" ::: "memory");
    if (l == 0)
        __hip_atomic_store(&P.fin_pub[0], P.fin_seq, __ATOMIC_RELEASE, __HIP_MEMORY_SCOPE_SYSTEM);
}

__device__ __forceinline__ void fused_finish(const VsaLitParams &P, const ConfLds &cl, u32 *sc) {
    __syncthreads();
    const u32 tid = threadIdx.x, wave = tid / WAVE, lane = lane_id();
    const u32 w = blockIdx.x, nb = cl.lb_n;
    u32 *loff = sc;
    u32 *misc = sc + VSA_LBINS;
    static_assert(VSA_LBINS == 4 * WAVE, "one wave scans the local bins, 4 per lane");
    if (wave == 0) {
        u32 c[4], t4 = 0;
        bool crowd = false;
#pragma unroll
        for (int k = 0; k < 4; k++) {
            const u32 i = 4 * lane + k;
            const u32 v = i < nb ? cl.lbins[i] : 0u;
            crowd |= v > VSA_SORT_BIN_MAX;
            c[k] = v < VSA_SORT_BIN_MAX ? v : VSA_SORT_BIN_MAX;
            t4 += c[k];
        }
        u32 tot;
        u32 e = wave_excl_scan(t4, &tot);
#pragma unroll
        for (int k = 0; k < 4; k++) {
            loff[4 * lane + k] = e;
            e += c[k];
        }
        const bool cr = wave_any(crowd) || cl.f_bad != 0;
        if (lane == 0) {
            const unsigned long long ep = (unsigned long long)P.fin_epoch << 32;
            __hip_atomic_store(&P.fin_agg[2 * w], ep | (cr ? (1ULL << 31) : 0ULL) | tot,
                               __ATOMIC_RELAXED, __HIP_MEMORY_SCOPE_AGENT);
            __hip_atomic_store(&P.fin_agg[2 * w + 1], ep | cl.f_cand, __ATOMIC_RELAXED,
                               __HIP_MEMORY_SCOPE_AGENT);
        }
        misc[1] = tot;
        misc[2] = cr;
    }
    const u32 lb = 16 * wave;
    const u32 nbw = nb > lb ? (nb - lb < 16 ? nb - lb : 16u) : 0u;
    u32 mmax = 0;
    for (u32 j = 0; j < nbw; j++) mmax = cl.lbins[lb + j] > mmax ? cl.lbins[lb + j] : mmax;
    const bool live = mmax != 0 && mmax <= VSA_SORT_BIN_MAX;
    u32 S = 2;
    while (S < mmax && S < WAVE) S <<= 1;
    const u32 per = WAVE / S;
    const u32 np = (nbw + per - 1) / per;
    const bool early = live && np <= 4;
    const size_t row0 = (size_t)w * VSA_LBINS + lb;
    Bins4 B0;
    if (early) {
        bins16_load(B0, P.bin_keys, P.bin_ids, row0, &cl.lbins[lb], nbw, S, 0, lane);
        bins4_sort(B0, lane);
    }
    auto put = [&](const Bins4 &B, u32 pass0, u32 base) {
        const u32 j_l = lane / S;
#pragma unroll
        for (u32 p = 0; p < 4; p++) {
            if (p >= B.npass) break;
            const u32 j = (pass0 + p) * per + j_l;
            if (j >= nbw || B.r >= cl.lbins[lb + j]) continue;
            const u64 o = (u64)base + loff[lb + j] + B.r;
            if (o < P.out_cap) {
                P.fin_keys[o] = B.k[p];
                P.fin_ids[o] = B.id[p];
            }
            if (P.fin_pk && o < P.fin_pk_cap) {
                P.fin_pk[1 + o] = B.k[p];
                ((uint32_t *)(P.fin_pk + 1 + P.fin_pk_cap))[o] = B.id[p];
            }
        }
    };
    if (wave == 0) {
        u32 base = 0, polls = 0, crowd_lo = 0;
        unsigned long long cand = 0;
        for (u32 v0 = 0; v0 < w; v0 += WAVE) {
            const u32 v = v0 + lane;
            if (v < w) {
                unsigned long long a = 0, b = 0;
                for (; polls < (1u << 20); polls++) {
                    a = __hip_atomic_load(&P.fin_agg[2 * v], __ATOMIC_RELAXED,
                                          __HIP_MEMORY_SCOPE_AGENT);
                    b = __hip_atomic_load(&P.fin_agg[2 * v + 1], __ATOMIC_RELAXED,
                                          __HIP_MEMORY_SCOPE_AGENT);
                    if ((u32)(a >> 32) == P.fin_epoch && (u32)(b >> 32) == P.fin_epoch) break;
                    __builtin_amdgcn_s_sleep(2);
                }
                base += (u32)a & 0x7fffffffu;
                crowd_lo |= (u32)(a >> 31) & 1u;
                cand += (u32)b;
            }
        }
        const bool timeout = wave_any(polls >= (1u << 20));
        if (timeout && lane == 0) flag_crowd(P);
#pragma unroll
        for (int dd = 32; dd >= 1; dd >>= 1) {
            base += shfl_xor_u32(base, dd);
            crowd_lo |= shfl_xor_u32(crowd_lo, dd);
            cand += ((unsigned long long)shfl_xor_u32((u32)(cand >> 32), dd) << 32) |
                    shfl_xor_u32((u32)cand, dd);
        }
        if (lane == 0) {
            misc[0] = base;
            misc[3] = crowd_lo | (timeout ? 1u : 0u);
            misc[4] = (u32)cand;
            misc[5] = (u32)(cand >> 32);
        }
    }
    __syncthreads();
    const u32 base = misc[0];
    if (early) {
        put(B0, 0, base);
    } else if (live) {
        for (u32 pass0 = 0; pass0 < np; pass0 += 4) {
            Bins4 B;
            bins16_load(B, P.bin_keys, P.bin_ids, row0, &cl.lbins[lb], nbw, S, pass0, lane);
            bins4_sort(B, lane);
            put(B, pass0, base);
        }
    }
    if (w + 1 == gridDim.x && wave == 0) {
        const unsigned long long n = (unsigned long long)base + misc[1];
        const bool crowded = misc[2] != 0 || misc[3] != 0;
        const unsigned long long cand =
            (((unsigned long long)misc[5] << 32) | misc[4]) + cl.f_cand;
        publish_fused(P, n, cand, crowded);
    }
}

__global__ void __launch_bounds__(256) vsa_publish(unsigned long long *ctr,
                                                   unsigned long long *h,
                                                   unsigned long long seq, uint32_t nzero,
                                                   const uint64_t *keys, const uint32_t *ids,
                                                   uint32_t kmax) {
    publish_body(ctr, h, seq, nzero, keys, ids, kmax);
}

#define FIN_BINS 64
__global__ void __launch_bounds__(1024) vsa_bin_finish(const uint32_t *counts, uint32_t *counts_next,
                                                     const uint64_t *skeys, const uint32_t *sids,
                                                     uint64_t *okeys,
                                                     uint32_t *oids,
                                                     uint64_t out_cap, unsigned long long *ctr,
                                                     unsigned long long *h,
                                                     unsigned long long seq,
                                                     const unsigned long long *fb,
                                                     unsigned long long *hfb, uint32_t nfb,
                                                     uint64_t *pk, uint64_t pk_cap) {
    __shared__ u32 red[16], cnt[FIN_BINS], off[FIN_BINS];
    static_assert(VSA_SORT_BINS / 4 <= 4 * 1024, "the prefix is 4 uint4 loads per thread");
    const u32 t = threadIdx.x, wv = t / WAVE, lane = lane_id();
    const u32 b0 = blockIdx.x * FIN_BINS;
    const u32 lb = wv * 4;
    const uint4 mc = *(const uint4 *)(counts + b0 + lb);
    const u32 c64 = counts[b0 + (t & (FIN_BINS - 1))];
    uint4 pv[4];
#pragma unroll
    for (u32 q = 0; q < 4; q++) {
        const u32 i = t + q * 1024;
        pv[q] = ((const uint4 *)counts)[i < b0 / 4 ? i : 0u];
    }
    u32 s = 0;
#pragma unroll
    for (u32 q = 0; q < 4; q++)
        if (t + q * 1024 < b0 / 4) s += pv[q].x + pv[q].y + pv[q].z + pv[q].w;
    const u32 m[4] = {mc.x, mc.y, mc.z, mc.w};
    u32 mmax = 0;
#pragma unroll
    for (int j = 0; j < 4; j++) mmax = m[j] > mmax ? m[j] : mmax;
    const bool sorting = mmax != 0 && mmax <= VSA_SORT_BIN_MAX;
    Bins4 B;
    bins4_load(B, skeys, sids, (size_t)(b0 + lb), m, sorting, lane);
#pragma unroll
    for (int dd = 32; dd >= 1; dd >>= 1) s += shfl_xor_u32(s, dd);
    if (lane == 0) red[wv] = s;
    if (t < FIN_BINS) {
        cnt[t] = c64;
        counts_next[b0 + t] = 0;
    }
    __syncthreads();
    if (wv == 0) {
        u32 base = 0;
#pragma unroll
        for (int kk = 0; kk < 16; kk++) base += red[kk];
        u32 tot;
        const u32 e = wave_excl_scan(cnt[lane], &tot);
        off[lane] = base + e;
    }
    __syncthreads();
    if (blockIdx.x == 0 && wv == 0) publish_wave(ctr, h, seq, 144u, fb, hfb, nfb, pk, out_cap);
    if (!sorting) return;
    bins4_sort(B, lane);
    const u32 o4[4] = {off[lb], off[lb + 1], off[lb + 2], off[lb + 3]};
    bins4_write(B, o4, okeys, oids, out_cap, pk, pk_cap);
}

__global__ void __launch_bounds__(256) vsa_pack(const unsigned long long *saved, uint64_t out_cap,
                                                const uint64_t *keys, const uint32_t *ids,
                                                uint64_t cap, uint64_t *dst) {
    const uint64_t n = saved[0];
    const bool bad = n > out_cap || saved[VSA_CTR_BIN_OVERFLOW] != 0;
    const uint64_t m = bad ? 0 : (n < cap ? n : cap);
    if (blockIdx.x == 0 && threadIdx.x == 0) dst[0] = n | (bad ? (1ULL << 62) : 0ULL);
    uint32_t *did = (uint32_t *)(dst + 1 + cap);
    for (uint64_t i = (uint64_t)blockIdx.x * 256 + threadIdx.x; i < m;
         i += (uint64_t)gridDim.x * 256) {
        dst[1 + i] = keys[i];
        did[i] = ids[i];
    }
}


// ... 185 lines not shown
            bits |= (r0 | (r1 << 2)) << (4 * k);
        }
        if (valid_bytes < 16) bits &= (1u << valid_bytes) - 1u;
        const u64 p0 = lo + 1024 * (u64)it + 16 * lane;
        if (P.bitmap) ((uint16_t *)P.bitmap)[p0 >> 4] = (uint16_t)bits;
        if (bits) {
            const u64 f = p0 + (u64)(__ffs(bits) - 1);
            const u64 l = p0 + (u64)(31 - __clz(bits)) + 1;
            first = f < first ? f : first;
            last = l > last ? l : last;
            cnt += __popc(bits);
        }
    };
    while (g < ngr) {
        u32 gnn = 0;
        if (lane == 0)
            gnn = __hip_atomic_fetch_add(&gctr, 1u, __ATOMIC_RELAXED, __HIP_MEMORY_SCOPE_WORKGROUP);
#pragma unroll
        for (int k = 0; k < CLS_DEPTH; k++) {
            const u32 it = g * CLS_DEPTH + k;
            const uint4 v = ring[k];
            const u32 itn = gn < ngr ? gn * CLS_DEPTH + k : it;
            if (nfull) ring[k] = load_wave_kib(sb, chunk_off(itn, it < nfull ? it : 0));
            if (it < nfull) {
                classify(it, v, 16);
            } else if (it < nit) {
                const u64 p0 = lo + 1024 * (u64)it + 16 * lane;
                u32 d[4] = {0, 0, 0, 0};
                u32 nv = 0;
                if (p0 < hi) {
                    nv = (u32)min((u64)16, hi - p0);
                    for (u32 b = 0; b < nv; b++) d[b >> 2] |= (u32)P.data[p0 + b] << (8 * (b & 3));
                }
                if (p0 < hi) classify(it, make_uint4(d[0], d[1], d[2], d[3]), nv);
            }
        }
        g = gn;
        gn = readfirstlane_u32(gnn);
    }
#pragma unroll
    for (int d = 32; d >= 1; d >>= 1) {
        u32 flo = shfl_down_u32((u32)first, d), fhi = shfl_down_u32((u32)(first >> 32), d);
        u64 of = ((u64)fhi << 32) | flo;
        if (of < first) first = of;
        u32 llo = shfl_down_u32((u32)last, d), lhi = shfl_down_u32((u32)(last >> 32), d);
        u64 ol = ((u64)lhi << 32) | llo;
        if (ol > last) last = ol;
        u32 clo = shfl_down_u32((u32)cnt, d), chi = shfl_down_u32((u32)(cnt >> 32), d);
        cnt += ((u64)chi << 32) | clo;
    }
    if (lane == 0) {
        const u32 sl = 16 * ((blockIdx.x * 16 + wave) % P.slots);
        if (first != ~0ULL) atomicMin(P.first + sl, first);
        if (last) atomicMax(P.last + sl, last);
        if (cnt) atomicAdd(P.count + sl, cnt);
    }
}

__global__ void __launch_bounds__(1024) vsa_read_probe(const uint8_t *A, u64 n, u32 *sink) {
    typedef u32 v4u __attribute__((ext_vector_type(4)));
    const u32 lane = threadIdx.x & 63;
    const u64 W = (u64)gridDim.x * 16;
    const u64 w = (u64)blockIdx.x * 16 + (threadIdx.x >> 6);
    constexpr u64 SEG = 64 << 10;
    constexpr u32 ITERS = SEG >> 10, DEPTH = 4;
    u32 acc = 0;
    for (u64 sg = w; sg * SEG < n; sg += W) {
        const uint8_t *base = A + sg * SEG + 16 * lane;
        v4u ring[DEPTH];
#pragma unroll
        for (u32 k = 0; k < DEPTH; k++) ring[k] = __builtin_nontemporal_load((const v4u *)(base + 1024 * k));
        for (u32 g = 0; g < ITERS / DEPTH; g++) {
#pragma unroll
            for (u32 k = 0; k < DEPTH; k++) {
                const v4u v = ring[k];
                acc ^= v.x + v.y * 3 + v.z * 5 + v.w * 7;
                const u32 it = g * DEPTH + k + DEPTH;
                ring[k] = __builtin_nontemporal_load((const v4u *)(base + 1024 * (it < ITERS ? it : 0)));
            }
        }
    }
    if (acc == 0x9e3779b9u) sink[threadIdx.x & 15] = acc;
}
```

vectorscan_amd/csrc/runtime.hip:

```cpp
#include <hipcub/hipcub.hpp>

#include "runtime_internal.h"

static uint32_t nconf_for_rate(double rate) {
    return rate > 0.05 ? 3u : rate > 5e-3 ? 2u : 1u;
}

static bool xp_for_rate(double rate) { return rate > 4e-4; }

namespace vsa_rt {


int ensure_out(vsa_ctx *c, uint64_t need) {
    Workspace &w = c->ws;
    if (need <= w.out_cap && w.d_tmp) return VSA_OK;
    uint64_t cap = std::max<uint64_t>(need + need / 4, 1u << 16);
    for (int i = 0; i < 2; i++) {
        if (w.d_keys[i]) (void)hipFree(w.d_keys[i]);
        if (w.d_ids[i]) (void)hipFree(w.d_ids[i]);
        w.d_keys[i] = nullptr;
        w.d_ids[i] = nullptr;
        VSA_CHECK(hipMalloc(&w.d_keys[i], cap * 8));
        VSA_CHECK(hipMalloc(&w.d_ids[i], cap * 4));
    }
    if (w.d_tmp) (void)hipFree(w.d_tmp);
    w.d_tmp = nullptr;
    size_t bytes = 0;
    hipcub::DoubleBuffer<uint64_t> kb(w.d_keys[0], w.d_keys[1]);
    hipcub::DoubleBuffer<uint32_t> vb(w.d_ids[0], w.d_ids[1]);
    VSA_CHECK(hipcub::DeviceRadixSort::SortPairs(nullptr, bytes, kb, vb, (int)std::min<uint64_t>(cap, 0x7fffffff), 0, 64, c->stream));
    VSA_CHECK(hipMalloc(&w.d_tmp, bytes));
    w.tmp_bytes = bytes;
    w.out_cap = cap;
    return VSA_OK;
}

int ensure_in(vsa_ctx *c, size_t need) {
    Workspace &w = c->ws;
    if (need <= w.in_cap) return VSA_OK;
    if (w.d_in) (void)hipFree(w.d_in);
    w.d_in = nullptr;
    size_t cap = std::max<size_t>(need + 64, 1u << 20);
    VSA_CHECK(hipMalloc(&w.d_in, cap));
    w.in_cap = cap;
    return VSA_OK;
}



int ensure_hin(vsa_ctx *c, size_t need) {
    Workspace &w = c->ws;
    if (need <= w.h_in_cap) return VSA_OK;
    if (w.h_in) (void)hipHostFree(w.h_in);
    w.h_in = nullptr;
    w.h_in_cap = 0;
    const size_t cap = std::max<size_t>(need, 64 << 10);
    VSA_CHECK(hipHostMalloc((void **)&w.h_in, cap, hipHostMallocDefault));
    w.h_in_cap = cap;
    return VSA_OK;
}

int ensure_tables(vsa_ctx *c, uint32_t nb, uint64_t nsegs, bool keep_blocks) {
    Workspace &w = c->ws;
    const size_t seg_off = ((size_t)nb * sizeof(VsaBlock) + TAB_ALIGN - 1) & ~(TAB_ALIGN - 1);
    const size_t need = seg_off + nsegs * sizeof(uint32_t);
    if (need > w.tab_cap) {
        VsaBlock *old = w.h_blocks;
        if (w.d_blocks) (void)hipFree(w.d_blocks);
        w.d_blocks = w.h_blocks = nullptr;
        w.tab_cap = 0;
        const size_t cap = std::max<size_t>(need + need / 4, 64 << 10);
        VSA_CHECK(hipMalloc(&w.d_blocks, cap));
        VSA_CHECK(hipHostMalloc((void **)&w.h_blocks, cap, hipHostMallocDefault));
        if (keep_blocks && old) memcpy(w.h_blocks, old, (size_t)nb * sizeof(VsaBlock));
        if (old) (void)hipHostFree(old);
        w.tab_cap = cap;
    }
    w.d_segblk = (uint32_t *)((uint8_t *)w.d_blocks + seg_off);
    w.h_segblk = (uint32_t *)((uint8_t *)w.h_blocks + seg_off);
    return VSA_OK;
}


int env_int(const char *name, int dflt) {
    const char *e = getenv(name);
    return e ? atoi(e) : dflt;
}

uint32_t steal_min() {
    static const uint32_t v = (uint32_t)std::max(0, env_int("VSA_STEAL", 4));
    return v;
}

int bits_for(uint64_t v) {
    int b = 0;
    while (v) {
        b++;
        v >>= 1;
    }
    return b;
}

template <int MODE, bool XP = false, bool SPLIT = false>
int launch_lit(vsa_ctx *c, const VsaLitParams &P, size_t lds) {
    auto fn = vsa_lit_scan<MODE, XP, SPLIT>;
    static std::atomic<int> lds_set[64];
    std::atomic<int> &ls = lds_set[c->device & 63];
    if (ls.load(std::memory_order_relaxed) < (int)lds) {
        VSA_CHECK(hipFuncSetAttribute((const void *)fn,
                                      hipFuncAttributeMaxDynamicSharedMemorySize, (int)lds));
        int cur = ls.load(std::memory_order_relaxed);
        while (cur < (int)lds && !ls.compare_exchange_weak(cur, (int)lds)) {
        }
    }
    const uint32_t grid = std::max<uint32_t>(1, c->launch.grid);
    static const bool print_launch = getenv("VSA_PRINT_LAUNCH") != nullptr;
    if (print_launch)
        fprintf(stderr,
                "vsa launch: mode %d xp %d grid %u nsegs %llu nblocks %u lds %zu qcap %u nconf %u "
                "end_par %u data %p blocks %p seg_desc %p out_cap %llu bins %p\n",
                MODE, (int)XP, grid, (unsigned long long)P.nsegs, P.nblocks, lds, P.qcap, P.nconf,
                P.end_par, (const void *)P.data, (const void *)P.blocks,
                (const void *)P.seg_desc, (unsigned long long)P.out_cap, (void *)P.bin_counts);
    hipEvent_t e0 = c->launch.ev_start;
    hipEvent_t e1 = P.end_par == 1 ? nullptr : c->launch.ev_stop;
    c->launch.ev_start = nullptr;
    if (e1) c->launch.ev_stop = nullptr;
    drop_stale_error();
    hipExtLaunchKernelGGL(fn, dim3(grid), dim3(LIT_THREADS), (uint32_t)lds, c->stream, e0, e1, 0u,
                          P);
    VSA_CHECK(hipGetLastError());
    return VSA_OK;
}

size_t plan_lds(size_t tab, uint32_t slot_words, size_t ent, uint32_t *qcap,
                size_t budget = LDS_BUDGET, uint32_t nconf = 1) {
    const size_t waves = LIT_WAVES - nconf;
    const size_t extra = nconf == 1 ? 512 * 16 : (size_t)nconf * 256 * 16;
    const size_t slots = ((size_t)slot_words * 4 + 15) & ~(size_t)15;
    tab = (tab + 15) & ~(size_t)15;
    size_t rest = budget > tab + slots + extra ? budget - tab - slots - extra : 0;
    uint32_t q = 4;
    while (q < 64 && waves * (size_t)(2 * q) * ent <= rest) q *= 2;
    *qcap = q;
    return tab + waves * (size_t)q * ent + slots + extra;
}

uint32_t launch_nconf(const vsa_db *db, size_t tab, size_t ent, size_t budget) {
    uint32_t nc = db->nconf.load(std::memory_order_relaxed);
    if (const char *e = getenv("VSA_NCONF")) nc = (uint32_t)std::min(4, std::max(1, atoi(e)));
    uint32_t q;
    while (nc > 1 && plan_lds(tab, db->slot_words, ent, &q, budget, nc) > budget) nc--;
    return nc;
}

bool use_xp(const vsa_db *db) {
    if (const char *e = getenv("VSA_XP")) return atoi(e) != 0;
    return db->xp.load(std::memory_order_relaxed);
}

bool use_bins(const vsa_ctx *c) {
    return !(c->launch.flags & VSA_SCAN_UNSORTED) && c->bin_skip == 0;
}

uint32_t bin_shift_for(int end_bits) {
    return end_bits > (int)VSA_SORT_BIN_BITS ? (uint32_t)end_bits - VSA_SORT_BIN_BITS : 0u;
}

uint64_t *bstage_keys(Workspace &w) { return (uint64_t *)w.d_bstage; }
uint32_t *bstage_ids(Workspace &w) {
    return (uint32_t *)(w.d_bstage + (size_t)VSA_SORT_BINS * VSA_SORT_BIN_MAX * sizeof(uint64_t));
}
uint32_t *bin_counts_of(vsa_ctx *c, uint32_t par) { return c->ws.d_bins + par * VSA_SORT_BINS; }

int queue_bin_sort(vsa_ctx *c) {
    Workspace &w = c->ws;
    const uint32_t par = c->bin_par;
    const bool fbd = c->fb.armed >= 0 && c->fb.dev;
    drop_stale_error();
    hipLaunchKernelGGL(vsa_bin_finish, dim3(VSA_SORT_BINS / 64), dim3(1024), 0, c->stream,
                       bin_counts_of(c, par), bin_counts_of(c, par ^ 1u), bstage_keys(w),
                       bstage_ids(w), w.d_keys[1], w.d_ids[1], (uint64_t)w.out_cap,
                       c->ws.d_counters, c->ws.d_pub, (unsigned long long)++c->pub_seq,
                       fbd ? c->fb.d_rec : nullptr, fbd ? c->fb.d : nullptr,
                       fbd ? 2 * c->fb.grid : 0u, (uint64_t *)c->launch.pack_dst,
                       c->launch.pack_cap);
    c->launch.pack_dst = nullptr;
    VSA_CHECK(hipGetLastError());
    c->bins_clean[par ^ 1u] = true;
    c->bin_par = par ^ 1u;
    return VSA_OK;
}

bool xcd_feedback_on() {
    static const bool v = env_int("VSA_XCD_FEEDBACK", 1) != 0;
    return v;
}

int fb_gain_us() {
    static const int v = env_int("VSA_FB_GAIN_US", 4);
    return v;
}

bool dyn_shares_on() {
    static const bool v = env_int("VSA_DYN_SHARES", 0) != 0;
    return v;
}

uint64_t dyn_min_bytes() {
    static const uint64_t v = (uint64_t)std::max(0, env_int("VSA_DYN_MIN_MIB", 2048)) << 20;
    return v;
}

static bool fb_trace() {
    static const bool v = env_int("VSA_FB_TRACE", 0) != 0;
// ... 176 lines not shown
        c->ctr_clean = true;
        return VSA_OK;
    }
    if (c->launch.fused) {
        c->launch.pack_dst = nullptr;
        c->launch.dev_sort = true;
        c->launch.published = true;
        c->ctr_clean = true;
        return VSA_OK;
    }
    c->launch.dev_sort = c->launch.bins;
    if (!c->launch.dev_sort) return VSA_OK;
    int r2 = queue_bin_sort(c);
    if (r2 != VSA_OK) return r2;
    c->launch.published = true;
    c->ctr_clean = true;
    return VSA_OK;
}

int launch_scan_kernel(vsa_ctx *c, const vsa_db *db, const uint8_t *d_data, uint32_t nb,
                       uint64_t nsegs) {
    Workspace &w = c->ws;
    VsaLitParams P;
    memset(&P, 0, sizeof(P));
    P.data = d_data;
    P.blocks = c->launch.d_blocks;
    P.seg_desc = c->launch.d_segblk;
    P.wg_seg = c->launch.d_segblk + 4 * nsegs;
    P.wg_bins = c->launch.d_segblk + 4 * nsegs + c->launch.grid + 1;
    P.nblocks = nb;
    P.steal = steal_min();
    P.nsegs = nsegs;
    P.out_keys = w.d_keys[0];
    P.out_ids = w.d_ids[0];
    P.out_cap = w.out_cap;
    P.bin_counts = c->launch.bins ? bin_counts_of(c, c->bin_par) : nullptr;
    P.bin_shift = bin_shift_for(c->launch.end_bits);
    P.bin_keys = c->launch.bins ? bstage_keys(w) : nullptr;
    P.bin_ids = c->launch.bins ? bstage_ids(w) : nullptr;
    P.counters = w.d_counters;
    P.wg_time = c->fb.armed >= 0 ? (c->fb.dev ? c->fb.d_rec : c->fb.d) : nullptr;
    if (c->launch.dyn) {
        DynState &D = *c->dyn;
        constexpr size_t REC = 512, WTS = 8;
        if (!D.d) {
            VSA_CHECK(hipMalloc(&D.d, (2 * REC + WTS) * sizeof(unsigned long long)));
            VSA_CHECK(hipMemsetAsync(D.d, 0, (2 * REC + WTS) * sizeof(unsigned long long),
                                     c->stream));
        }
        const uint64_t e = ++D.epoch;
        c->launch.dyn_epoch = e;
        const bool prev = D.grid == c->launch.grid && D.kind == db->mode;
        uint32_t *wts = (uint32_t *)(D.d + 2 * REC);
        P.wg_time = D.d + (e & 1) * REC;
        P.dyn_prev = prev ? D.d + ((e - 1) & 1) * REC : nullptr;
        P.dyn_wprev = prev ? wts + ((e - 1) & 1) * WTS : nullptr;
        P.dyn_wout = wts + (e & 1) * WTS;
        P.dyn_kib = c->launch.dyn_kib;
        P.dyn_margin = c->launch.dyn_margin;
        P.wg_bins = c->launch.d_segblk + 4 * nsegs + 7 * (size_t)c->launch.grid + 1;
        D.grid = c->launch.grid;
        D.kind = db->mode;
    }
    P.wave_log = g_wave_log;
    if (c->launch.fused) {
        const uint32_t G = c->launch.grid;
        P.bin_keys = (uint64_t *)w.d_fstage;
        P.bin_ids = (uint32_t *)(w.d_fstage + (size_t)w.fstage_grid * VSA_LBINS *
                                                  VSA_SORT_BIN_MAX * sizeof(uint64_t));
        P.bin_counts = nullptr;
        P.fin_wg = c->launch.d_segblk + 4 * nsegs + G + 1 + 2 * (size_t)G;
        P.fin_keys = w.d_keys[1];
        P.fin_ids = w.d_ids[1];
        P.fin_agg = w.d_fagg;
        P.fin_seq = ++c->pub_seq;
        P.fin_epoch = (uint32_t)(P.fin_seq % 0xfffffffeULL) + 1u;
        P.fin_pub = w.d_pub;
        P.fin_pk = (uint64_t *)c->launch.pack_dst;
        P.fin_pk_cap = c->launch.pack_cap;
    }
    {
        const char *e = getenv("VSA_DEBUG_FLAGS");
        P.dbg = e ? (uint32_t)atoi(e) : 0u;
    }
    if (db->type == HWLM_ENGINE_NOOD) {
        const uint32_t ml = db->nood.msk_len;
        P.nood_msk = db->nood.msk << (8 * (8 - ml));
        P.nood_cmp = db->nood.cmp << (8 * (8 - ml));
        P.nood_len = ml;
        P.nood_id = db->nood.id;
        for (int b = 0; b < 16; b++) P.slot_off[b] = 0xffffffffu;
        P.nconf = 1;
        size_t lds = plan_lds(0, 0, 32, &P.qcap);
        return launch_lit<VSA_MODE_NOOD>(c, P, lds);
    }
    const uint8_t *d_eng = db->d_blob + VSA_ROUNDUP_CL(sizeof(HWLM));
    P.table = db->d_table;
    P.table_entries = db->table_entries;
    P.dmask = db->dmask;
    P.state_lo = db->state_lo;
    P.state_hi = db->state_hi;
    const uint32_t conf_offset_in_eng = ((const uint32_t *)(db->hblob + VSA_ROUNDUP_CL(sizeof(HWLM))))[4];
    P.conf_base = d_eng + conf_offset_in_eng;
    memcpy(P.conf_off, db->conf_off, sizeof(P.conf_off));
    P.slotmap = db->d_slots;
    P.slot_words = db->slot_words;
    memcpy(P.slot_off, db->slot_off, sizeof(P.slot_off));
    memcpy(P.slot_bits, db->slot_bits, sizeof(P.slot_bits));
    P.pf_mult = db->pf_mult;
    if (db->mode == VSA_MODE_FDR4) {
        const size_t tb = (size_t)db->table_entries * 4;
        const bool xp = use_xp(db);
        const size_t ent = xp ? 16 : 48;
        P.nconf = launch_nconf(db, tb, ent, LDS_BUDGET);
        size_t lds = plan_lds(tb, db->slot_words, ent, &P.qcap, LDS_BUDGET, P.nconf);
        if (lds > LDS_BUDGET) return VSA_E_INVALID;
        if (!db->split)
            return xp ? launch_lit<VSA_MODE_FDR4, true>(c, P, lds)
                      : launch_lit<VSA_MODE_FDR4>(c, P, lds);
        auto go = [&](const VsaLitParams &Q) {
            return xp ? launch_lit<VSA_MODE_FDR4, true, true>(c, Q, lds)
                      : launch_lit<VSA_MODE_FDR4, false, true>(c, Q, lds);
        };
        P.end_par = 1;
        if (int r = go(P)) return r;
        P.end_par = 2;
        P.table = (const uint64_t *)db->d_table2;
        return go(P);
    }
    const size_t below = 0x10000 - (160 * 1024 - LDS_BUDGET);
    const size_t teddy_dyn = 128 * 1024;
    if (db->mode == VSA_MODE_TEDDY) {
        P.nconf = launch_nconf(db, 0, 48, below);
        if (plan_lds(0, db->slot_words, 48, &P.qcap, below, P.nconf) > below) return VSA_E_INVALID;
        return launch_lit<VSA_MODE_TEDDY>(c, P, teddy_dyn);
    }
    P.nconf = launch_nconf(db, 0, 64, below);
    if (plan_lds(0, db->slot_words, 64, &P.qcap, below, P.nconf) > below) return VSA_E_INVALID;
    return launch_lit<VSA_MODE_FAT>(c, P, teddy_dyn);
}

hipError_t wait_stream(vsa_ctx *c) {
    hipError_t e = hipEventRecord(c->ev_done, c->stream);
    if (e != hipSuccess) return e;
    const auto t0 = std::chrono::steady_clock::now();
    for (uint32_t i = 0;; i++) {
        e = hipEventQuery(c->ev_done);
        if (e != hipErrorNotReady) return e;
        (void)hipGetLastError();
        if ((i & 15) == 15) {
            const auto dt = std::chrono::steady_clock::now() - t0;
            if (dt > std::chrono::milliseconds(50)) return hipStreamSynchronize(c->stream);
            if (dt > std::chrono::microseconds(100)) sched_yield();
        }
    }
}

hipError_t wait_published(vsa_ctx *c, uint64_t seq) {
    volatile unsigned long long *h = c->ws.h_pub;
    const auto t0 = std::chrono::steady_clock::now();
    for (uint32_t i = 0;; i++) {
        if (h[0] == seq) break;
        if ((i & 15) == 15) {
            const auto dt = std::chrono::steady_clock::now() - t0;
            if (dt > std::chrono::milliseconds(50)) {
                hipError_t e = hipStreamSynchronize(c->stream);
// ... 717 lines not shown
    }
    c->pending = false;
    uint64_t n = 0;
    int r = complete_scan(c, &n);
    if (n_matches) *n_matches = n;
    return r;
}

int vsa_scan_results(vsa_ctx_t *c, const uint64_t **k, const uint32_t **ids) {
    if (!c) return VSA_E_INVALID;
    if (int r = finish_pending(c)) return r;
    VSA_CHECK(hipStreamSynchronize(c->stream));
    if (k) *k = c->ws.d_keys[c->cur];
    if (ids) *ids = c->ws.d_ids[c->cur];
    return VSA_OK;
}

int vsa_scan_pack(vsa_ctx_t *c, void *d_dst, uint64_t cap) {
    if (!c || !d_dst) return VSA_E_INVALID;
    VSA_CHECK(hipSetDevice(c->device));
    const uint32_t grid = (uint32_t)std::max<uint64_t>(1, std::min<uint64_t>((cap + 255) / 256, 256));
    if (c->pending && c->launch.published && c->launch.dev_sort) {
        drop_stale_error();
        hipLaunchKernelGGL(vsa_pack, dim3(grid), dim3(256), 0, c->stream,
                           (const unsigned long long *)c->ws.d_counters + 144,
                           (uint64_t)c->ws.out_cap, (const uint64_t *)c->ws.d_keys[1],
                           (const uint32_t *)c->ws.d_ids[1], cap, (uint64_t *)d_dst);
        VSA_CHECK(hipGetLastError());
        return VSA_OK;
    }
    if (int r = finish_pending(c)) return r;
    unsigned long long *save = c->ws.d_counters + 144;
    unsigned long long hv[16] = {c->last_n, 0};
    VSA_CHECK(hipMemcpyAsync(save, hv, sizeof(hv), hipMemcpyHostToDevice, c->stream));
    drop_stale_error();
    hipLaunchKernelGGL(vsa_pack, dim3(grid), dim3(256), 0, c->stream,
                       (const unsigned long long *)save, (uint64_t)c->ws.out_cap,
                       (const uint64_t *)c->ws.d_keys[c->cur], (const uint32_t *)c->ws.d_ids[c->cur],
                       cap, (uint64_t *)d_dst);
    VSA_CHECK(hipGetLastError());
    VSA_CHECK(hipStreamSynchronize(c->stream));
    return VSA_OK;
}

int vsa_scan_copy(vsa_ctx_t *c, vsa_match_t *out, uint64_t cap, uint64_t *n_copied) {
    if (!c) return VSA_E_INVALID;
    uint64_t n = std::min(cap, c->last_n);
    if (n) {
        std::vector<uint64_t> k(n);
        std::vector<uint32_t> id(n);
        VSA_CHECK(hipMemcpyAsync(k.data(), c->ws.d_keys[c->cur], n * 8, hipMemcpyDeviceToHost,
                                 c->stream));
        VSA_CHECK(hipMemcpyAsync(id.data(), c->ws.d_ids[c->cur], n * 4, hipMemcpyDeviceToHost,
                                 c->stream));
        VSA_CHECK(hipStreamSynchronize(c->stream));
        for (uint64_t i = 0; i < n; i++) {
            out[i].key = k[i];
            out[i].id = id[i];
            out[i].pad = 0;
        }
    }
    if (n_copied) *n_copied = n;
    return VSA_OK;
}

int vsa_scan_copy_device(vsa_ctx_t *c, uint64_t *d_keys, uint32_t *d_ids, uint64_t cap,
                         uint64_t *n_copied) {
    if (!c) return VSA_E_INVALID;
    const uint64_t n = std::min(cap, c->last_n);
    if (n) {
        if (d_keys)
            VSA_CHECK(hipMemcpyAsync(d_keys, c->ws.d_keys[c->cur], n * 8,
                                     hipMemcpyDeviceToDevice, c->stream));
        if (d_ids)
            VSA_CHECK(hipMemcpyAsync(d_ids, c->ws.d_ids[c->cur], n * 4,
                                     hipMemcpyDeviceToDevice, c->stream));
    }
    if (n_copied) *n_copied = n;
    return VSA_OK;
}

uint64_t vsa_scan_candidates(vsa_ctx_t *c) { return c ? c->last_cand : 0; }

int vsa_scan_debug_counters(vsa_ctx_t *c, uint64_t out[16]) {
    if (!c || !out) return VSA_E_INVALID;
    if (int r = finish_pending(c)) return r;
    VSA_CHECK(hipStreamSynchronize(c->stream));
    memcpy(out, c->ws.h_counters, 16 * sizeof(uint64_t));
    return VSA_OK;
}

double vsa_scan_kernel_ms(vsa_ctx_t *c) {
    if (!c) return 0.0;
    if (c->kms_stale) {
        c->kms_stale = false;
        const auto t0 = std::chrono::steady_clock::now();
        hipError_t e;
        while ((e = hipEventQuery(c->ev1)) == hipErrorNotReady) {
            (void)hipGetLastError();
            if (std::chrono::steady_clock::now() - t0 > std::chrono::milliseconds(50)) {
                e = hipEventSynchronize(c->ev1);
                break;
            }
        }
        float ms = 0.f;
        if (e == hipSuccess && hipEventElapsedTime(&ms, c->ev0, c->ev1) == hipSuccess)
            c->last_kernel_ms = ms;
        (void)hipGetLastError();
    }
    return c->last_kernel_ms;
}

uint64_t vsa_scan_launches(vsa_ctx_t *c) { return c ? c->lit_launches : 0; }

int vsa_scan_last_fused(vsa_ctx_t *c) { return c && c->launch.fused ? 1 : 0; }

int vsa_scan_last_dyn(vsa_ctx_t *c) { return c && c->launch.dyn ? 1 : 0; }

int vsa_ctx_set_dyn_shares(vsa_ctx_t *c, int on, uint64_t min_bytes) {
    if (!c) return VSA_E_INVALID;
    c->dyn_shares = on != 0;
    c->dyn_min = min_bytes;
    return VSA_OK;
}

int vsa_ctx_set_timing(vsa_ctx_t *c, uint32_t every) {
    if (!c) return VSA_E_INVALID;
    c->timing_every = every;
    return VSA_OK;
}

int vsa_ctx_set_fused_finish(vsa_ctx_t *c, int on) {
    if (!c) return VSA_E_INVALID;
    c->fused_finish = on != 0;
    return VSA_OK;
}

int vsa_read_ceiling(vsa_ctx_t *c, const uint8_t *d_data, uint64_t len, uint32_t runs,
                     double *best_ms, uint64_t *bytes) {
    if (!c || !d_data || !best_ms || !runs) return VSA_E_INVALID;
    if ((uintptr_t)d_data & 15) return VSA_E_INVALID;
    const uint64_t n = len & ~((uint64_t)(64 << 10) - 1);
    if (!n) return VSA_E_INVALID;
    VSA_CHECK(hipSetDevice(c->device));
    uint32_t *sink = nullptr;
    VSA_CHECK(hipMalloc(&sink, 64));
    hipEvent_t e0, e1;
    hipError_t e = hipEventCreate(&e0);
    if (e == hipSuccess && (e = hipEventCreate(&e1)) != hipSuccess) (void)hipEventDestroy(e0);
    if (e != hipSuccess) {
        (void)hipFree(sink);
        VSA_CHECK(e);
    }
    float best = 1e30f;
    for (uint32_t r = 0; r <= runs && e == hipSuccess; r++) {
        e = hipEventRecord(e0, c->stream);
        if (e != hipSuccess) break;
        drop_stale_error();
        hipLaunchKernelGGL(vsa_read_probe, dim3(c->num_cus), dim3(1024), 0, c->stream, d_data, n,
                           sink);
        if ((e = hipGetLastError()) != hipSuccess) break;
        if ((e = hipEventRecord(e1, c->stream)) != hipSuccess) break;
        if ((e = hipEventSynchronize(e1)) != hipSuccess) break;
        float ms = 0.f;
        if ((e = hipEventElapsedTime(&ms, e0, e1)) != hipSuccess) break;
        if (r > 0 && ms < best) best = ms;
// ... 118 lines not shown
```

vectorscan_amd/csrc/runtime_internal.h:

```cpp
#ifndef VSA_RUNTIME_INTERNAL_H
#define VSA_RUNTIME_INTERNAL_H

#include <hip/hip_runtime.h>
#include <hip/hip_ext.h>

#include <algorithm>
#include <atomic>
#include <chrono>
#include <cmath>
#include <condition_variable>
#include <cstdio>
#include <cstdlib>
#include <cstring>
#include <deque>
#include <map>
#include <memory>
#include <mutex>
#include <thread>
#include <vector>
#include <sched.h>

#include "../../include/vectorscan_amd.h"
#include "hs_layout.h"
#include "kernels.h"
#include "vsa_internal.h"

template <int MODE, bool XP, bool SPLIT>
__global__ void vsa_lit_scan(VsaLitParams P);
__global__ void vsa_class_scan(VsaClassParams P);
__global__ void vsa_bin_finish(const uint32_t *counts, uint32_t *counts_next,
                               const uint64_t *skeys, const uint32_t *sids, uint64_t *okeys, uint32_t *oids, uint64_t out_cap,
                               unsigned long long *ctr,
                               unsigned long long *h, unsigned long long seq,
                               const unsigned long long *fb, unsigned long long *hfb,
                               uint32_t nfb, uint64_t *pk, uint64_t pk_cap);
__global__ void vsa_class_scan_lut(VsaClassParams P, uint64_t span);
__global__ void vsa_publish(unsigned long long *ctr, unsigned long long *h, unsigned long long seq,
                            uint32_t nzero, const uint64_t *keys, const uint32_t *ids,
                            uint32_t kmax);
__global__ void vsa_pack(const unsigned long long *saved, uint64_t out_cap, const uint64_t *keys,
                         const uint32_t *ids, uint64_t cap, uint64_t *dst);
__global__ void vsa_pair_scan(VsaPairParams P);
__global__ void vsa_read_probe(const uint8_t *A, uint64_t n, uint32_t *sink);

#define VSA_CHECK(x)                                                          \
    do {                                                                      \
        hipError_t e_ = (x);                                                  \
        if (e_ != hipSuccess) {                                               \
            if (!getenv("VSA_QUIET"))                                         \
                fprintf(stderr, "vsa: %s failed: %s (%s:%d)\n", #x,           \
                        hipGetErrorString(e_), __FILE__, __LINE__);           \
            return VSA_E_DEVICE;                                              \
        }                                                                     \
    } while (0)

namespace vsa_rt {


const int LIT_WAVES = 16;
const int LIT_THREADS = 1024;
const size_t LDS_BUDGET = 160 * 1024 - 4096;
const uint32_t SLOT_WORDS_MAX = 3072;

constexpr int CLASS_SLOTS = 64;
constexpr int PAIR_BASE = 160;
constexpr int CLASS_BASE = 256;
constexpr int N_COUNTERS = CLASS_BASE + 16 * CLASS_SLOTS;
constexpr uint32_t PUB_RECS = 1024;
constexpr size_t PUB_WORDS = 17 + PUB_RECS + PUB_RECS / 2;

struct Workspace {
    uint8_t *d_in = nullptr;
    size_t in_cap = 0;
    uint8_t *h_in = nullptr;
    size_t h_in_cap = 0;
    uint64_t *d_keys[2] = {nullptr, nullptr};
    uint32_t *d_ids[2] = {nullptr, nullptr};
    uint64_t out_cap = 0;
    void *d_tmp = nullptr;
    size_t tmp_bytes = 0;
    unsigned long long *d_counters = nullptr;
    uint32_t *d_bins = nullptr;
    uint8_t *d_bstage = nullptr;
    unsigned long long *h_counters = nullptr;
    unsigned long long *h_pub = nullptr, *d_pub = nullptr;
    VsaBlock *d_blocks = nullptr;
    VsaBlock *h_blocks = nullptr;
    size_t tab_cap = 0;
    uint32_t *d_segblk = nullptr;
    uint32_t *h_segblk = nullptr;
    uint8_t *d_fstage = nullptr;
    uint32_t fstage_grid = 0;
    unsigned long long *d_fagg = nullptr;
};


}

using namespace vsa_rt;

struct BatchPlan {
    std::vector<VsaBlock> blocks;
    std::vector<uint32_t> segblk;
    uint64_t nsegs = 0;
    uint32_t grid = 0;
    int end_bits = 0;
    uint64_t bytes = 0;
    bool fin_ok = false;
    uint32_t dyn_kib = 0, dyn_margin = 0;
    std::vector<int64_t> spans, live;
};

struct DynState {
    unsigned long long *d = nullptr;
    uint64_t epoch = 0;
    uint32_t grid = 0;
    int kind = -1;
    ~DynState() {
        if (d) (void)hipFree(d);
    }
};

struct vsa_plan;

struct vsa_ctx {
    int device = 0;
    int num_cus = 256;
    int reserved_cus = 0;
    int plan_cus() const { return std::max(1, num_cus - reserved_cus); }
    hipStream_t stream = nullptr;
    std::shared_ptr<void> stream_ref;
    std::shared_ptr<DynState> dyn;
    Workspace ws;
    int cur = 0;
    uint64_t last_n = 0;
    uint64_t last_cand = 0;
    bool pending = false;
    struct {
        const vsa_db *db = nullptr;
        const uint8_t *d_data = nullptr;
        uint32_t nb = 0;
        uint64_t segs = 0;
        uint32_t grid = 0;
        int end_bits = 0;
        uint32_t flags = 0;
        bool bins = false;
        bool dev_sort = false;
        bool published = false;
        bool fin_ok = false;
        bool timed = false;
        bool fused = false;
        uint32_t dyn_kib = 0, dyn_margin = 0;
        bool dyn = false;
        uint64_t dyn_epoch = 0;
        uint64_t bytes = 0;
        const VsaBlock *d_blocks = nullptr;
        const uint32_t *d_segblk = nullptr;
        hipEvent_t ev_start = nullptr, ev_stop = nullptr;
        void *pack_dst = nullptr;
        uint64_t pack_cap = 0;
    } launch;
    hipEvent_t ev0 = nullptr, ev1 = nullptr;
    hipEvent_t ev_done = nullptr;
    hipEvent_t ev_rec = nullptr;
    hipEvent_t ev_mark = nullptr;
    bool marked = false;
    hipStream_t copy_stream = nullptr;
    double last_kernel_ms = 0.0;
    bool kms_stale = false;
    bool fused_finish = false;
    uint32_t timing_every = 1;
    bool dyn_shares = true;
    uint64_t dyn_min = 0;
    uint32_t bin_skip = 0;
    uint32_t bin_backoff = 16;
    uint64_t lit_launches = 0;
    bool bins_clean[2] = {false, false};
    uint32_t bin_par = 0;
    const uint8_t *res_host = nullptr;
    size_t res_len = 0;
    BatchPlan plan;
    struct {
        bool valid = false;
        const uint8_t *d_data = nullptr;
        uint64_t waves = 0;
        uint32_t nb = 0;
        uint64_t fb_key = 0;
        std::vector<uint64_t> in[5];
    } memo;
    bool host_sort = false;
    bool ctr_clean = false;
    uint64_t pub_seq = 0;
    std::vector<vsa_plan *> plans;
    struct FbSet {
        float w[8] = {1, 1, 1, 1, 1, 1, 1, 1};
        float wa[8] = {1, 1, 1, 1, 1, 1, 1, 1};
        uint8_t xcc[1024];
        float wg[1024];
        uint32_t version = 0;
        uint32_t since = 0;
        bool known = false;
    };
    struct {
        FbSet set[2];
        unsigned long long *h = nullptr, *d = nullptr;
        int armed = -1;
        bool dev = false;
        unsigned long long *d_rec = nullptr;
        uint32_t grid = 0;
    } fb;
};

struct vsa_plan {
    vsa_ctx *ctx = nullptr;
    const uint8_t *d_data = nullptr;
    uint32_t nb = 0;
    uint64_t segs = 0;
    uint32_t grid = 0;
    int end_bits = 0;
    uint64_t bytes = 0;
    uint32_t rebuilds = 0;
    bool fin_ok = false;
    uint32_t dyn_kib = 0, dyn_margin = 0;
    VsaBlock *d_blocks = nullptr;
    uint32_t *d_segblk = nullptr;
    std::vector<uint64_t> in[5];
    size_t segblk_cap = 0;
    uint64_t fb_key = ~0ULL;
    void *h_stage = nullptr;
    std::vector<uint32_t> flags;
};

constexpr uint32_t SCAN_HOST_SORT_SMALL = 1u << 16;
constexpr uint64_t HOST_SORT_MAX = 1024;

struct vsa_db {
    vsa_ctx *ctx = nullptr;
// ... 105 lines not shown
```

Before: 5178 GB/s.

## Specialise literal scan kernel on dyn/fused/diag options as template parameters

Adds an OPT template parameter to vsa_lit_scan selecting dynamic-shares, fused-finish and diagnostic paths at compile time instead of runtime checks on P.fin_keys, P.dyn_kib and P.dbg. Unused LDS (profiling, dyn bounds) and timing reads are dropped from variants that don't need them, and the host dispatches to the matching instantiation, compiled in a second translation unit. The aim is lower register/LDS pressure and fewer branches in the hot scan loop. The cost is more kernel instantiations and longer builds, and debug flags now need a diag build.

Measured after the change: 5184 GB/s (median of 6 runs). Within noise of the previous version (+0.1%).

```diff
diff --git a/include/vectorscan_amd.h b/include/vectorscan_amd.h
--- a/include/vectorscan_amd.h
+++ b/include/vectorscan_amd.h
@@ -191,6 +191,7 @@
 uint64_t vsa_scan_launches(vsa_ctx_t *ctx);
 int vsa_scan_last_fused(vsa_ctx_t *ctx);
 int vsa_scan_last_dyn(vsa_ctx_t *ctx);
+uint32_t vsa_ctx_last_variant(vsa_ctx_t *ctx);
 int vsa_ctx_set_dyn_shares(vsa_ctx_t *ctx, int on, uint64_t min_bytes);
 int vsa_ctx_set_fused_finish(vsa_ctx_t *ctx, int on);
 int vsa_read_ceiling(vsa_ctx_t *ctx, const uint8_t *d_data, uint64_t len, uint32_t runs,
diff --git a/vectorscan_amd/__init__.py b/vectorscan_amd/__init__.py
--- a/vectorscan_amd/__init__.py
+++ b/vectorscan_amd/__init__.py
@@ -147,6 +147,9 @@
 _sig("vsa_scan_launches", ctypes.c_uint64, ctypes.c_void_p)
 _sig("vsa_scan_last_fused", ctypes.c_int, ctypes.c_void_p)
 _sig("vsa_scan_last_dyn", ctypes.c_int, ctypes.c_void_p)
+_sig("vsa_ctx_last_variant", ctypes.c_uint32, ctypes.c_void_p)
+VARIANT_XP, VARIANT_SPLIT, VARIANT_OPT_SHIFT = 0x10, 0x20, 8
+OPT_DYN, OPT_FUSED, OPT_DIAG = 1, 2, 4
 _sig("vsa_ctx_set_dyn_shares", ctypes.c_int, ctypes.c_void_p, ctypes.c_int, ctypes.c_uint64)
 _sig("vsa_ctx_set_fused_finish", ctypes.c_int, ctypes.c_void_p, ctypes.c_int)
 _sig("vsa_ctx_set_timing", ctypes.c_int, ctypes.c_void_p, ctypes.c_uint32)
@@ -717,6 +720,9 @@
     def last_dyn(self):
         return lib.vsa_scan_last_dyn(self.ptr) == 1
 
+    def last_variant(self):
+        return lib.vsa_ctx_last_variant(self.ptr)
+
     def dyn_shares(self, on=True, min_mib=2048):
         _check(lib.vsa_ctx_set_dyn_shares(self.ptr, 1 if on else 0, int(min_mib) << 20))
 
diff --git a/vectorscan_amd/csrc/kernels.h b/vectorscan_amd/csrc/kernels.h
--- a/vectorscan_amd/csrc/kernels.h
+++ b/vectorscan_amd/csrc/kernels.h
@@ -41,6 +41,15 @@
     VSA_MODE_NOOD = 3,
     VSA_MODE_FDR4 = 4,
 };
+
+enum VsaLitOpt : uint32_t {
+    OPT_DYN = 1,
+    OPT_FUSED = 2,
+    OPT_DIAG = 4,
+};
+#define VSA_VARIANT_XP 0x10u
+#define VSA_VARIANT_SPLIT 0x20u
+#define VSA_VARIANT_OPT_SHIFT 8
 
 #define VSA_SORT_BIN_BITS 14
 #define VSA_SORT_BINS (1u << VSA_SORT_BIN_BITS)
diff --git a/vectorscan_amd/csrc/kernels.hip b/vectorscan_amd/csrc/kernels.hip
--- a/vectorscan_amd/csrc/kernels.hip
+++ b/vectorscan_amd/csrc/kernels.hip
@@ -1,5 +1,6 @@
 #include <hip/hip_runtime.h>
 #include <stdint.h>
+#include <type_traits>
 
 #include "kernels.h"
 
@@ -11,6 +12,7 @@
 #define VSA_DIAG_ON 0
 #endif
 #define VSA_DBG(flags, bits) (VSA_DIAG_ON && ((flags) & (bits)))
+#define VSA_DBGO(OPT, flags, bits) ((((OPT) & OPT_DIAG) != 0) && ((flags) & (bits)))
 #define LIT_THREADS (LIT_WAVES * WAVE)
 #define QCAP 256
 
@@ -286,29 +288,33 @@
     u32 f_cand;
 };
 
+template <u32 OPT>
 __device__ __forceinline__ u32 rec_bin(const VsaLitParams &P, const ConfLds &cl, u64 end) {
-    if (P.fin_keys) {
+    if constexpr ((OPT & OPT_FUSED) != 0) {
         const u64 d = (end - cl.f_lo) >> cl.f_shift;
         return d < VSA_LBINS ? (u32)d : 0xffffffffu;
     }
     return (u32)(end >> P.bin_shift);
 }
-__device__ __forceinline__ size_t bin_row(const VsaLitParams &P, u32 bin) {
-    return P.fin_keys ? (size_t)blockIdx.x * VSA_LBINS + bin : (size_t)bin;
-}
-
+template <u32 OPT>
+__device__ __forceinline__ size_t bin_row(u32 bin) {
+    return (OPT & OPT_FUSED) ? (size_t)blockIdx.x * VSA_LBINS + bin : (size_t)bin;
+}
+
+template <u32 OPT>
 __device__ __forceinline__ u32 bin_slot_take(const VsaLitParams &P, const ConfLds &cl, u32 bin) {
     const u32 k = bin - cl.lb_lo;
     if (k < cl.lb_n)
         return __hip_atomic_fetch_add(const_cast<u32 *>(&cl.lbins[k]), 1u, __ATOMIC_RELAXED,
                                       __HIP_MEMORY_SCOPE_WORKGROUP);
-    if (P.fin_keys) {
+    if constexpr ((OPT & OPT_FUSED) != 0) {
         __hip_atomic_store(const_cast<u32 *>(&cl.f_bad), 1u, __ATOMIC_RELAXED,
                            __HIP_MEMORY_SCOPE_WORKGROUP);
         return VSA_SORT_BIN_MAX;
-    }
-    return __hip_atomic_fetch_add(&P.bin_counts[bin], 1u, __ATOMIC_RELAXED,
-                                  __HIP_MEMORY_SCOPE_AGENT);
+    } else {
+        return __hip_atomic_fetch_add(&P.bin_counts[bin], 1u, __ATOMIC_RELAXED,
+                                      __HIP_MEMORY_SCOPE_AGENT);
+    }
 }
 
 __device__ __forceinline__ void flag_crowd(const VsaLitParams &P) {
@@ -333,8 +339,8 @@
     u32 *head;
     u32 lg;
     u32 dbg;
+    unsigned long long *diag;
     const u32 *slots;
-    unsigned long long *diag;
 };
 
 __device__ __forceinline__ u32 lds_ld32(const u32 *p) {
@@ -348,7 +354,7 @@
     return (u32)(((key & andmsk) * mult) >> (64 - nbits));
 }
 
-template <int CONF_U>
+template <int CONF_U, u32 OPT>
 __device__ __forceinline__ void confirm_multi(const VsaLitParams &P, const ConfLds &cl,
                                               const QEnt (&q)[CONF_U], const bool (&valid)[CONF_U],
                                               u32 mis) {
@@ -429,8 +435,8 @@
 #pragma unroll
             for (int i = 0; i < CONF_U; i++)
                 if (bins && mt[i]) {
-                    bbin[i] = rec_bin(P, cl, base[i] + (u64)e[i]);
-                    bslot[i] = bin_slot_take(P, cl, bbin[i]);
+                    bbin[i] = rec_bin<OPT>(P, cl, base[i] + (u64)e[i]);
+                    bslot[i] = bin_slot_take<OPT>(P, cl, bbin[i]);
                 }
 #pragma unroll
             for (int i = 0; i < CONF_U; i++) {
@@ -440,7 +446,7 @@
                 u32 before = 0;
 #pragma unroll
                 for (int k = 0; k < i; k++) before += (u32)__popcll(pm[k]);
-                const u64 q = bins ? (u64)bin_row(P, bbin[i]) * VSA_SORT_BIN_MAX + bslot[i]
+                const u64 q = bins ? (u64)bin_row<OPT>(bbin[i]) * VSA_SORT_BIN_MAX + bslot[i]
                                    : sb + before + __builtin_amdgcn_mbcnt_hi(
                                          (u32)(pm[i] >> 32), __builtin_amdgcn_mbcnt_lo((u32)pm[i], 0));
                 if (bins ? bslot[i] < VSA_SORT_BIN_MAX : q < P.out_cap) {
@@ -781,7 +787,7 @@
     }
 }
 
-template <int MODE, bool EDGE, bool XP, bool SPLIT>
+template <int MODE, bool EDGE, bool XP, bool SPLIT, u32 OPT>
 __device__ __forceinline__ IterState lit_iter(const VsaLitParams &P, const ConfLds &cl,
                                               const LitShared &L, const SegCtx &S,
                                               u32 mis, int64_t ib, uint4 chunk,
@@ -903,11 +909,7 @@
 #pragma unroll
     for (int i = 1; i < T::CW; i++) all &= c[i];
     if (!wave_any((all | ~bucket_mask) != 0xffffffffu)) return out;
-#ifdef VSA_DIAG
-    const bool tdiag = (P.dbg & 32768) != 0;
-#else
-    constexpr bool tdiag = false;
-#endif
+    const bool tdiag = VSA_DBGO(OPT, P.dbg, 32768);
     const u64 t_c0 = tdiag ? __builtin_amdgcn_s_memtime() : 0;
     u32 any = 0;
 #pragma unroll
@@ -915,7 +917,7 @@
         c[i] = ~c[i] & bucket_mask;
         any |= c[i];
     }
-    if (VSA_DBG(P.dbg, 32)) {
+    if (VSA_DBGO(OPT, P.dbg, 32)) {
         u32 pc = 0;
 #pragma unroll
         for (int i = 0; i < T::CW; i++) pc += __popc(c[i]);
@@ -923,7 +925,7 @@
         for (int dd = 32; dd >= 1; dd >>= 1) pc += shfl_xor_u32(pc, dd);
         out.ncand += readfirstlane_u32(pc);
     }
-    if (VSA_DBG(P.dbg, 8)) return out;
+    if (VSA_DBGO(OPT, P.dbg, 8)) return out;
 
     u32 pv2 = lane_up1(d[2]);
     if (lane == 0) pv2 = (u32)in.pbytes;
@@ -1019,7 +1021,7 @@
     return out;
 }
 
-template <int MODE, bool EDGE, bool XP, bool SPLIT>
+template <int MODE, bool EDGE, bool XP, bool SPLIT, u32 OPT>
 __device__ __forceinline__ IterState scan_iter(const VsaLitParams &P, const ConfLds &cl,
                                                const LitShared &L, const SegCtx &S,
                                                u32 mis, int64_t ib, uint4 chunk,
@@ -1027,7 +1029,7 @@
     if constexpr (MODE == VSA_MODE_NOOD) {
         return nood_iter<EDGE>(P, L, S, ib, chunk, in);
     } else {
-        return lit_iter<MODE, EDGE, XP, SPLIT>(P, cl, L, S, mis, ib, chunk, in,
+        return lit_iter<MODE, EDGE, XP, SPLIT, OPT>(P, cl, L, S, mis, ib, chunk, in,
                                                    bucket_mask);
     }
 }
@@ -1070,7 +1072,7 @@
 #endif
 #define EXP_U 1
 #define PQ_ENTRIES(CU) ((CU) == 4 ? 512 : 256)
-template <int MODE, int CONF_U, bool XP>
+template <int MODE, int CONF_U, bool XP, u32 OPT>
 __device__ __forceinline__ void confirm_wave(const VsaLitParams &P, const ConfLds &cl,
                                              const uint4 *rings, u32 lg, u32 *tails,
                                              const u32 *heads, const u32 *q_done, u32 mis,
@@ -1094,7 +1096,7 @@
     u32 filled = 0;
     u32 consumed = 0;
     u32 pq_head = 0, pq_tail = 0;
-    const bool prof = VSA_DBG(P.dbg, 64);
+    const bool prof = VSA_DBGO(OPT, P.dbg, 64);
     u64 tmark = prof ? __builtin_amdgcn_s_memtime() : 0;
     auto pcount = [&](int i, u64 v) {
         if (prof && lane == 0) pcl[i] += v;
@@ -1106,11 +1108,7 @@
             tmark = now;
         }
     };
-#ifdef VSA_DIAG
-    const bool dlog = (P.dbg & 8192) != 0;
-#else
-    constexpr bool dlog = false;
-#endif
+    const bool dlog = VSA_DBGO(OPT, P.dbg, 8192);
     bool seen_done = false;
     auto confirm_batch = [&](u32 k) {
         if (dlog) {
@@ -1127,7 +1125,7 @@
             valid[i] = j < k;
             q[i] = valid[i] ? pq[(pq_tail + j) & (PQ_CAP - 1)] : QEnt{0, 0};
         }
-        confirm_multi<CONF_U>(P, cl, q, valid, mis);
+        confirm_multi<CONF_U, OPT>(P, cl, q, valid, mis);
         asm volatile("" ::: "memory");
         pq_tail += k;
         consumed += k;
@@ -1178,7 +1176,7 @@
             phase(3);
             continue;
         }
-        if (VSA_DBG(P.dbg, 128)) continue;
+        if (VSA_DBGO(OPT, P.dbg, 128)) continue;
         if constexpr (XP) {
             const u64 pm = __ballot(valid);
             if (valid) {
@@ -1190,7 +1188,7 @@
             }
             pq_head += filled;
             if (pq_head - pq_tail >= (u32)WAVE * CONF_U) {
-                if (filled >= 16 && !VSA_DBG(P.dbg, 1024)) __builtin_amdgcn_s_setprio(2);
+                if (filled >= 16 && !(VSA_DBGO(OPT, P.dbg, 1024))) __builtin_amdgcn_s_setprio(2);
                 else __builtin_amdgcn_s_setprio(0);
                 confirm_batch(WAVE * CONF_U);
             }
@@ -1198,7 +1196,7 @@
         }
         if constexpr (MODE != VSA_MODE_NOOD)
         {
-            if (filled >= 16 && !VSA_DBG(P.dbg, 1024)) __builtin_amdgcn_s_setprio(2);
+            if (filled >= 16 && !(VSA_DBGO(OPT, P.dbg, 1024))) __builtin_amdgcn_s_setprio(2);
             else __builtin_amdgcn_s_setprio(0);
         }
         const u64 meta0 = ((u64)e[1] << 32) | e[0];
@@ -1213,10 +1211,10 @@
                 for (; hits; hits &= hits - 1) {
                     const u32 j = __ffs(hits) - 1;
                     const u64 end = p0 + j - mis;
-                    const u32 bin = rec_bin(P, cl, end);
-                    const u32 s = bin_slot_take(P, cl, bin);
+                    const u32 bin = rec_bin<OPT>(P, cl, end);
+                    const u32 s = bin_slot_take<OPT>(P, cl, bin);
                     if (s < VSA_SORT_BIN_MAX) {
-                        const size_t q = bin_row(P, bin) * VSA_SORT_BIN_MAX + s;
+                        const size_t q = bin_row<OPT>(bin) * VSA_SORT_BIN_MAX + s;
                         P.bin_keys[q] = end << VSA_KEY_END_SHIFT;
                         P.bin_ids[q] = P.nood_id;
                     } else {
@@ -1296,7 +1294,7 @@
 #pragma unroll
                 for (int u = 0; u < EXP_U; u++) {
                     push[u] = have[u] && ((sw[u] >> sh[u]) & 1u);
-                    if (VSA_DBG(P.dbg, 16)) push[u] = false;
+                    if (VSA_DBGO(OPT, P.dbg, 16)) push[u] = false;
                 }
 #pragma unroll
                 for (int u = 0; u < EXP_U; u++) {
@@ -1315,9 +1313,9 @@
             phase(1);
         }
     }
-    if (P.counters && lane == 0 && consumed && !VSA_DBG(P.dbg, 32)) {
+    if (P.counters && lane == 0 && consumed && !(VSA_DBGO(OPT, P.dbg, 32))) {
         atomicAdd(&P.counters[2], (unsigned long long)consumed);
-        if (P.fin_keys)
+        if constexpr ((OPT & OPT_FUSED) != 0)
             __hip_atomic_fetch_add(const_cast<u32 *>(&cl.f_cand), consumed, __ATOMIC_RELAXED,
                                    __HIP_MEMORY_SCOPE_WORKGROUP);
     }
@@ -1340,6 +1338,7 @@
     for (u32 i = base + tid; i < n; i += LIT_THREADS) dst[i] = src(i);
 }
 
+template <u32 OPT>
 __device__ __forceinline__ void fused_finish(const VsaLitParams &P, const ConfLds &cl, u32 *sc);
 
 struct DynB {
@@ -1530,25 +1529,51 @@
     }
 }
 
-template <int MODE, bool XP, bool SPLIT>
+template <bool ON>
+struct DynLds {
+    u32 s[4];
+};
+template <>
+struct DynLds<false> {};
+template <bool ON>
+struct DiagLds {
+    u64 prof[8 * MAX_CONF_WAVES];
+    unsigned long long cyc[3];
+};
+template <>
+struct DiagLds<false> {};
+
+template <int MODE, bool XP, bool SPLIT, uint32_t OPT>
 __global__ void __launch_bounds__(LIT_THREADS)
 vsa_lit_scan(VsaLitParams P) {
+    constexpr bool DYN = (OPT & OPT_DYN) != 0;
+    constexpr bool FUSED = (OPT & OPT_FUSED) != 0;
+    constexpr bool DIAG = (OPT & OPT_DIAG) != 0;
+    static_assert(!DIAG || VSA_DIAG_ON, "OPT_DIAG exists in -DVSA_DIAG builds only");
+    static_assert(!(FUSED && MODE == VSA_MODE_FAT), "Fat Teddy never fuses (VGPRs)");
     typedef LitTraits<MODE> T;
     constexpr int REW = XP ? 1 : T::EW;
     typedef typename T::S_t S_t;
     extern __shared__ __align__(16) u8 smem[];
     __shared__ ConfLds cl;
     __shared__ u32 q_tails[16], q_heads[16], q_done, wg_ctr, conf_fin;
-    __shared__ u32 dyn_s[4];
+    __shared__ DynLds<DYN> dyn_s;
     __shared__ unsigned long long rng[16];
-    __shared__ u64 prof_lds[8 * MAX_CONF_WAVES];
-    __shared__ unsigned long long diag_lds[3];
+    __shared__ DiagLds<DIAG> diag_s;
+    u64 *prof_lds = nullptr;
+    unsigned long long *diag_lds = nullptr;
+    if constexpr (DIAG) {
+        prof_lds = diag_s.prof;
+        diag_lds = diag_s.cyc;
+    }
     const u32 tid = threadIdx.x;
     const u32 lane = lane_id();
     const u32 wave = readfirstlane_u32(tid / WAVE);
-    const unsigned long long t_entry = __builtin_amdgcn_s_memrealtime();
-    DynPre dpre;
-    if (P.dyn_kib && wave == 0) dyn_load(P, lane, dpre);
+    unsigned long long t_entry = 0;
+    if (DYN || DIAG || P.wg_time) t_entry = __builtin_amdgcn_s_memrealtime();
+    typename std::conditional<DYN, DynPre, DynLds<false>>::type dpre;
+    if constexpr (DYN)
+        if (wave == 0) dyn_load(P, lane, dpre);
 
     const u32 mis = (u32)((uintptr_t)P.data & 15);
     const u8 *A = P.data - mis;
@@ -1610,7 +1635,7 @@
     }
     {
         u32 lo = 0, n = 0;
-        if (P.fin_keys) {
+        if constexpr (FUSED) {
             const uint32_t *f = P.fin_wg + 4 * (size_t)blockIdx.x;
             n = f[3];
             if (tid == 0) {
@@ -1644,16 +1669,20 @@
             __hip_atomic_store(&P.wg_time[gridDim.x + blockIdx.x], t_entry, __ATOMIC_RELAXED,
                                __HIP_MEMORY_SCOPE_AGENT);
     }
-    if (tid < 8 * MAX_CONF_WAVES) prof_lds[tid] = 0;
-    if (tid < 3) diag_lds[tid] = 0;
-    if (P.dyn_kib && wave == 0) {
-        DynB d;
-        dyn_bounds(P, lane, dpre, d);
-        if (lane == 0) {
-            dyn_s[0] = d.s_lo;
-            dyn_s[1] = d.s_hi;
-            dyn_s[2] = d.lk;
-            dyn_s[3] = d.hk;
+    if constexpr (DIAG) {
+        if (tid < 8 * MAX_CONF_WAVES) prof_lds[tid] = 0;
+        if (tid < 3) diag_lds[tid] = 0;
+    }
+    if constexpr (DYN) {
+        if (wave == 0) {
+            DynB d;
+            dyn_bounds(P, lane, dpre, d);
+            if (lane == 0) {
+                dyn_s.s[0] = d.s_lo;
+                dyn_s.s[1] = d.s_hi;
+                dyn_s.s[2] = d.lk;
+                dyn_s.s[3] = d.hk;
+            }
         }
     }
     __syncthreads();
@@ -1662,25 +1691,25 @@
         const u32 cw = wave - NS;
         u64 dg[3] = {0, 0, 0};
         if (NC == 1)
-            confirm_wave<MODE, 4, XP>(P, cl, rings, 31 - __clz(P.qcap), q_tails, q_heads, &q_done,
+            confirm_wave<MODE, 4, XP, OPT>(P, cl, rings, 31 - __clz(P.qcap), q_tails, q_heads, &q_done,
                                   mis, slots, pqx, 0, 1, prof_lds, dg);
         else
-            confirm_wave<MODE, 2, XP>(P, cl, rings, 31 - __clz(P.qcap), q_tails, q_heads, &q_done,
+            confirm_wave<MODE, 2, XP, OPT>(P, cl, rings, 31 - __clz(P.qcap), q_tails, q_heads, &q_done,
                                   mis, slots, pqx + (size_t)cw * PQ_ENTRIES(2), cw, NC,
-                                  prof_lds + 8 * cw, dg);
+                                  DIAG ? prof_lds + 8 * cw : nullptr, dg);
         {
             u32 prev = 0;
             if (lane == 0)
                 prev = __hip_atomic_fetch_add(&conf_fin, 1u, __ATOMIC_ACQ_REL,
                                               __HIP_MEMORY_SCOPE_WORKGROUP);
             if (readfirstlane_u32(prev) + 1 == NC) {
-                const u32 lo = cl.lb_lo, n = P.fin_keys ? 0u : cl.lb_n;
+                const u32 lo = cl.lb_lo, n = FUSED ? 0u : cl.lb_n;
                 for (u32 i = lane; i < n; i += WAVE) P.bin_counts[lo + i] = cl.lbins[i];
                 if (lane == 0 && cl.nrec)
                     atomicAdd(&P.counters[0], (unsigned long long)cl.nrec);
             }
         }
-        if ((P.dbg & 8192) && P.wave_log && lane < 8) {
+        if (VSA_DBGO(OPT, P.dbg, 8192) && P.wave_log && lane < 8) {
             const unsigned long long t_end = __builtin_amdgcn_s_memrealtime();
             P.wave_log[((size_t)blockIdx.x * LIT_WAVES + wave) * 8 + lane] =
                 lane == 0 ? t_entry : lane == 1 ? t_end : lane == 2 ? 1ull
@@ -1691,7 +1720,7 @@
     {
 
     u32 bucket_mask = 0;
-    if (!(P.dbg & 2)) {
+    if (!VSA_DBGO(OPT, P.dbg, 2)) {
         u32 present = 0;
         for (int b = 0; b < 16; b++) {
             if (P.conf_off[b]) present |= 1u << b;
@@ -1715,9 +1744,9 @@
     L.dbg = P.dbg;
     L.diag = diag_lds;
 
-    const unsigned long long t_start = __builtin_amdgcn_s_memrealtime();
+    const unsigned long long t_start = DIAG ? __builtin_amdgcn_s_memrealtime() : 0ull;
     u32 n_seg = 0, n_iter = 0;
-    if ((P.dbg & 2048) && lane == 0)
+    if (VSA_DBGO(OPT, P.dbg, 2048) && lane == 0)
         atomicMax(&P.counters[8], ~t_start);
     u32 ncand_total = 0;
     u32 ring_tail_cache = 0, ring_head = 0;
@@ -1731,8 +1760,14 @@
     };
     auto resolve = [&](u32 t0) -> u32 {
         const u32 t = readlane_u32(t0, 0);
-        const u32 wg_lo = readfirstlane_u32(P.dyn_kib ? dyn_s[0] : P.wg_seg[blockIdx.x]);
-        const u32 wg_hi = readfirstlane_u32(P.dyn_kib ? dyn_s[1] : P.wg_seg[blockIdx.x + 1]);
+        u32 wg_lo, wg_hi;
+        if constexpr (DYN) {
+            wg_lo = readfirstlane_u32(dyn_s.s[0]);
+            wg_hi = readfirstlane_u32(dyn_s.s[1]);
+        } else {
+            wg_lo = readfirstlane_u32(P.wg_seg[blockIdx.x]);
+            wg_hi = readfirstlane_u32(P.wg_seg[blockIdx.x + 1]);
+        }
         return wg_lo + t < wg_hi ? wg_lo + t : (u32)P.nsegs;
     };
     const bool steal_on = P.steal != 0;
@@ -1801,9 +1836,9 @@
         const u32 sbv = ((cu32 *)P.seg_desc)[4 * (size_t)segu];
         u32 d_off = ((cu32 *)P.seg_desc)[4 * (size_t)segu + 1];
         u32 d_len = ((cu32 *)P.seg_desc)[4 * (size_t)segu + 2];
-        if (P.dyn_kib) {
+        if constexpr (DYN) {
             const u32 d_pos = ((cu32 *)P.seg_desc)[4 * (size_t)segu + 3];
-            const u32 lk = readfirstlane_u32(dyn_s[2]), hk = readfirstlane_u32(dyn_s[3]);
+            const u32 lk = readfirstlane_u32(dyn_s.s[2]), hk = readfirstlane_u32(dyn_s.s[3]);
             const u32 a = d_pos > lk ? d_pos : lk;
             const u32 e = d_pos + d_len < hk ? d_pos + d_len : hk;
             d_off += a - d_pos;
@@ -1952,7 +1987,7 @@
             const int64_t ib = s_lo + 1024 * (int64_t)it;
             uint4 cur = ring[0];
             if (it > 0) cur = load_chunk(A, ib + 16 * (int64_t)lane, S.bhi);
-            is = scan_iter<MODE, true, XP, SPLIT>(P, cl, L, S, mis, ib, cur, is, bucket_mask);
+            is = scan_iter<MODE, true, XP, SPLIT, OPT>(P, cl, L, S, mis, ib, cur, is, bucket_mask);
             run_adv(ib);
         }
         bool tail_mine = true;
@@ -1982,7 +2017,7 @@
                 for (int k = 0; k < LIT_DEPTH; k++) {
                     const u32 it = g * LIT_DEPTH + k;
                     const int64_t ib = fb + 1024 * (int64_t)it;
-                    is = scan_iter<MODE, false, XP, SPLIT>(P, cl, L, S, mis, ib, ring[k], is, bucket_mask);
+                    is = scan_iter<MODE, false, XP, SPLIT, OPT>(P, cl, L, S, mis, ib, ring[k], is, bucket_mask);
                     run_adv(ib);
                     const u32 itn = (it + LIT_DEPTH < nf) ? it + LIT_DEPTH : it;
                     ring[k] = load_wave_kib(sb, 1024u * itn);
@@ -2004,7 +2039,7 @@
                 if ((u32)k < rem) {
                     const u32 it = ng * LIT_DEPTH + k;
                     const int64_t ib = fb + 1024 * (int64_t)it;
-                    is = scan_iter<MODE, false, XP, SPLIT>(P, cl, L, S, mis, ib, ring[k], is, bucket_mask);
+                    is = scan_iter<MODE, false, XP, SPLIT, OPT>(P, cl, L, S, mis, ib, ring[k], is, bucket_mask);
                     run_adv(ib);
                 }
             }
@@ -2018,10 +2053,10 @@
             const int64_t ib = s_lo + 1024 * (int64_t)it;
             uint4 cur = ring[1];
             if (it > f1 || !tail_pre) cur = load_chunk(A, ib + 16 * (int64_t)lane, S.bhi);
-            is = scan_iter<MODE, true, XP, SPLIT>(P, cl, L, S, mis, ib, cur, is, bucket_mask);
+            is = scan_iter<MODE, true, XP, SPLIT, OPT>(P, cl, L, S, mis, ib, cur, is, bucket_mask);
             run_adv(ib);
         }
-        n_iter += (stolen ? 0u : f0) + swept + (tail_mine ? niters - f1 : 0u);
+        if constexpr (DIAG) n_iter += (stolen ? 0u : f0) + swept + (tail_mine ? niters - f1 : 0u);
         ncand_total = is.ncand;
         ring_tail_cache = is.tail_cache;
         ring_head = is.head;
@@ -2041,7 +2076,7 @@
         fs.xn = xp_n;
         xp_flush(P, cl, L, fs);
     }
-    if ((P.dbg & 4096) && P.wave_log && lane < 8) {
+    if (VSA_DBGO(OPT, P.dbg, 4096) && P.wave_log && lane < 8) {
         u32 xcc, hwid;
         asm volatile("s_getreg_b32 %0, hwreg(HW_REG_XCC_ID)" : "=s"(xcc));
         asm volatile("s_getreg_b32 %0, hwreg(HW_REG_HW_ID)" : "=s"(hwid));
@@ -2053,7 +2088,7 @@
         for (int k = 0; k < 8; k++) x = (u32)k == lane ? v[k] : x;
         P.wave_log[((size_t)blockIdx.x * LIT_WAVES + wave) * 8 + lane] = x;
     }
-    if ((P.dbg & 2048) && lane == 0) {
+    if (VSA_DBGO(OPT, P.dbg, 2048) && lane == 0) {
         const unsigned long long t = __builtin_amdgcn_s_memrealtime();
         atomicMax(&P.counters[9], ~t);
         atomicMax(&P.counters[10], t);
@@ -2061,10 +2096,10 @@
     if (lane == 0) {
         const u32 prev = __hip_atomic_fetch_add(&q_done, 1u, __ATOMIC_RELAXED,
                                                 __HIP_MEMORY_SCOPE_WORKGROUP);
-        if (VSA_DIAG_ON && (P.dbg & 32768) && prev + 1 == NS) {
+        if (VSA_DBGO(OPT, P.dbg, 32768) && prev + 1 == NS) {
             for (int k = 0; k < 3; k++) atomicAdd(&P.counters[13 + k], diag_lds[k]);
         }
-        if ((P.dbg & 2048) && prev + 1 == NS)
+        if (VSA_DBGO(OPT, P.dbg, 2048) && prev + 1 == NS)
             atomicMax(&P.counters[11], ~(unsigned long long)__builtin_amdgcn_s_memrealtime());
         if (P.wg_time && prev + 1 == NS) {
             u32 xcc;
@@ -2077,23 +2112,41 @@
     }
     if (P.counters && lane_id() == 0 && ncand_total) {
         atomicAdd(&P.counters[2], (unsigned long long)ncand_total);
-        if (P.fin_keys)
+        if constexpr (FUSED)
             __hip_atomic_fetch_add(&cl.f_cand, ncand_total, __ATOMIC_RELAXED,
                                    __HIP_MEMORY_SCOPE_WORKGROUP);
     }
     }
 finish:
-    if constexpr (MODE != VSA_MODE_FAT)
-        if (P.fin_keys) fused_finish(P, cl, (u32 *)smem);
-}
-
-template __global__ void vsa_lit_scan<VSA_MODE_FDR4, false, false>(VsaLitParams);
-template __global__ void vsa_lit_scan<VSA_MODE_FDR4, true, false>(VsaLitParams);
-template __global__ void vsa_lit_scan<VSA_MODE_FDR4, false, true>(VsaLitParams);
-template __global__ void vsa_lit_scan<VSA_MODE_FDR4, true, true>(VsaLitParams);
-template __global__ void vsa_lit_scan<VSA_MODE_TEDDY, false, false>(VsaLitParams);
-template __global__ void vsa_lit_scan<VSA_MODE_FAT, false, false>(VsaLitParams);
-template __global__ void vsa_lit_scan<VSA_MODE_NOOD, false, false>(VsaLitParams);
+    if constexpr (FUSED) fused_finish<OPT>(P, cl, (u32 *)smem);
+}
+
+#ifdef VSA_DIAG
+#define VSA_LIT_INST(MODE, XP, SPLIT, OPT)                                          \
+    template __global__ void vsa_lit_scan<MODE, XP, SPLIT, (OPT)>(VsaLitParams);    \
+    template __global__ void vsa_lit_scan<MODE, XP, SPLIT, (OPT) | OPT_DIAG>(VsaLitParams);
+#else
+#define VSA_LIT_INST(MODE, XP, SPLIT, OPT) \
+    template __global__ void vsa_lit_scan<MODE, XP, SPLIT, (OPT)>(VsaLitParams);
+#endif
+#ifndef VSA_KERNELS_OPT_TU
+VSA_LIT_INST(VSA_MODE_FDR4, false, false, 0)
+VSA_LIT_INST(VSA_MODE_FDR4, true, false, 0)
+VSA_LIT_INST(VSA_MODE_FDR4, false, true, 0)
+VSA_LIT_INST(VSA_MODE_FDR4, true, true, 0)
+VSA_LIT_INST(VSA_MODE_TEDDY, false, false, 0)
+VSA_LIT_INST(VSA_MODE_FAT, false, false, 0)
+VSA_LIT_INST(VSA_MODE_NOOD, false, false, 0)
+#else
+VSA_LIT_INST(VSA_MODE_FDR4, false, false, OPT_DYN)
+VSA_LIT_INST(VSA_MODE_FDR4, true, false, OPT_DYN)
+VSA_LIT_INST(VSA_MODE_FDR4, false, true, OPT_DYN)
+VSA_LIT_INST(VSA_MODE_FDR4, true, true, OPT_DYN)
+VSA_LIT_INST(VSA_MODE_FDR4, false, false, OPT_FUSED)
+VSA_LIT_INST(VSA_MODE_FDR4, true, false, OPT_FUSED)
+VSA_LIT_INST(VSA_MODE_TEDDY, false, false, OPT_FUSED)
+VSA_LIT_INST(VSA_MODE_NOOD, false, false, OPT_FUSED)
+#endif
 
 
 
@@ -2159,6 +2212,7 @@
     }
 }
 
+template <u32 OPT>
 __device__ __forceinline__ void publish_fused(const VsaLitParams &P, unsigned long long n,
                                               unsigned long long cand, bool crowded) {
     const u32 l = lane_id();
@@ -2166,7 +2220,7 @@
     if (l == 0) v = n;
     else if (l == 2) v = cand;
     else if (l == VSA_CTR_BIN_OVERFLOW) v = crowded ? 1ULL : 0ULL;
-    else if (P.dbg && l < 16)
+    else if ((OPT & OPT_DIAG) && P.dbg && l < 16)
         v = __hip_atomic_load(&P.counters[l], __ATOMIC_RELAXED, __HIP_MEMORY_SCOPE_AGENT);
     if (P.fin_pk && l == 0)
         P.fin_pk[0] = n | ((n > P.out_cap || crowded) ? (1ULL << 62) : 0ULL);
@@ -2181,6 +2235,7 @@
         __hip_atomic_store(&P.fin_pub[0], P.fin_seq, __ATOMIC_RELEASE, __HIP_MEMORY_SCOPE_SYSTEM);
 }
 
+template <u32 OPT>
 __device__ __forceinline__ void fused_finish(const VsaLitParams &P, const ConfLds &cl, u32 *sc) {
     __syncthreads();
     const u32 tid = threadIdx.x, wave = tid / WAVE, lane = lane_id();
@@ -2304,10 +2359,11 @@
         const bool crowded = misc[2] != 0 || misc[3] != 0;
         const unsigned long long cand =
             (((unsigned long long)misc[5] << 32) | misc[4]) + cl.f_cand;
-        publish_fused(P, n, cand, crowded);
-    }
-}
-
+        publish_fused<OPT>(P, n, cand, crowded);
+    }
+}
+
+#ifndef VSA_KERNELS_OPT_TU
 __global__ void __launch_bounds__(256) vsa_publish(unsigned long long *ctr,
                                                    unsigned long long *h,
                                                    unsigned long long seq, uint32_t nzero,
@@ -2659,3 +2715,4 @@
     }
     if (acc == 0x9e3779b9u) sink[threadIdx.x & 15] = acc;
 }
+#endif
diff --git a/vectorscan_amd/csrc/kernels_opt.hip b/vectorscan_amd/csrc/kernels_opt.hip
--- /dev/null
+++ b/vectorscan_amd/csrc/kernels_opt.hip
@@ -0,0 +1,2 @@
+#define VSA_KERNELS_OPT_TU 1
+#include "kernels.hip"
diff --git a/vectorscan_amd/csrc/runtime.hip b/vectorscan_amd/csrc/runtime.hip
--- a/vectorscan_amd/csrc/runtime.hip
+++ b/vectorscan_amd/csrc/runtime.hip
@@ -101,9 +101,11 @@
     return b;
 }
 
-template <int MODE, bool XP = false, bool SPLIT = false>
-int launch_lit(vsa_ctx *c, const VsaLitParams &P, size_t lds) {
-    auto fn = vsa_lit_scan<MODE, XP, SPLIT>;
+template <int MODE, bool XP, bool SPLIT, uint32_t OPT>
+int launch_lit_as(vsa_ctx *c, const VsaLitParams &P, size_t lds) {
+    auto fn = vsa_lit_scan<MODE, XP, SPLIT, OPT>;
+    c->launch.variant = (uint32_t)MODE | (XP ? VSA_VARIANT_XP : 0u) |
+                        (SPLIT ? VSA_VARIANT_SPLIT : 0u) | (OPT << VSA_VARIANT_OPT_SHIFT);
     static std::atomic<int> lds_set[64];
     std::atomic<int> &ls = lds_set[c->device & 63];
     if (ls.load(std::memory_order_relaxed) < (int)lds) {
@@ -131,6 +133,31 @@
                           P);
     VSA_CHECK(hipGetLastError());
     return VSA_OK;
+}
+
+template <int MODE, bool XP, bool SPLIT, uint32_t DIAG>
+int launch_lit_opt(vsa_ctx *c, const VsaLitParams &P, size_t lds) {
+    const bool dyn = P.dyn_kib != 0, fused = P.fin_keys != nullptr;
+    if (dyn && fused) return VSA_E_INVALID;
+    if (dyn) {
+        if constexpr (MODE == VSA_MODE_FDR4)
+            return launch_lit_as<MODE, XP, SPLIT, OPT_DYN | DIAG>(c, P, lds);
+        return VSA_E_INVALID;
+    }
+    if (fused) {
+        if constexpr (MODE != VSA_MODE_FAT && !SPLIT)
+            return launch_lit_as<MODE, XP, SPLIT, OPT_FUSED | DIAG>(c, P, lds);
+        return VSA_E_INVALID;
+    }
+    return launch_lit_as<MODE, XP, SPLIT, DIAG>(c, P, lds);
+}
+
+template <int MODE, bool XP = false, bool SPLIT = false>
+int launch_lit(vsa_ctx *c, const VsaLitParams &P, size_t lds) {
+#ifdef VSA_DIAG
+    if (P.dbg || P.wave_log) return launch_lit_opt<MODE, XP, SPLIT, OPT_DIAG>(c, P, lds);
+#endif
+    return launch_lit_opt<MODE, XP, SPLIT, 0u>(c, P, lds);
 }
 
 size_t plan_lds(size_t tab, uint32_t slot_words, size_t ent, uint32_t *qcap,
@@ -473,6 +500,12 @@
     {
         const char *e = getenv("VSA_DEBUG_FLAGS");
         P.dbg = e ? (uint32_t)atoi(e) : 0u;
+#ifndef VSA_DIAG
+        static std::atomic<bool> warned{false};
+        if (P.dbg && !warned.exchange(true))
+            fprintf(stderr, "vsa: VSA_DEBUG_FLAGS is ignored by this build (it needs -DVSA_DIAG: "
+                            "tools/build_variant.sh diag -DVSA_DIAG)\n");
+#endif
     }
     if (db->type == HWLM_ENGINE_NOOD) {
         const uint32_t ml = db->nood.msk_len;
@@ -1356,6 +1389,8 @@
 
 uint64_t vsa_scan_candidates(vsa_ctx_t *c) { return c ? c->last_cand : 0; }
 
+uint32_t vsa_ctx_last_variant(vsa_ctx_t *c) { return c ? c->launch.variant : 0; }
+
 int vsa_scan_debug_counters(vsa_ctx_t *c, uint64_t out[16]) {
     if (!c || !out) return VSA_E_INVALID;
     if (int r = finish_pending(c)) return r;
diff --git a/vectorscan_amd/csrc/runtime_internal.h b/vectorscan_amd/csrc/runtime_internal.h
--- a/vectorscan_amd/csrc/runtime_internal.h
+++ b/vectorscan_amd/csrc/runtime_internal.h
@@ -25,7 +25,7 @@
 #include "kernels.h"
 #include "vsa_internal.h"
 
-template <int MODE, bool XP, bool SPLIT>
+template <int MODE, bool XP, bool SPLIT, uint32_t OPT>
 __global__ void vsa_lit_scan(VsaLitParams P);
 __global__ void vsa_class_scan(VsaClassParams P);
 __global__ void vsa_bin_finish(const uint32_t *counts, uint32_t *counts_next,
@@ -153,6 +153,7 @@
         uint32_t dyn_kib = 0, dyn_margin = 0;
         bool dyn = false;
         uint64_t dyn_epoch = 0;
+        uint32_t variant = 0;
         uint64_t bytes = 0;
         const VsaBlock *d_blocks = nullptr;
         const uint32_t *d_segblk = nullptr;
```
